# wangjiarui153/AIGV-Assessor

Hardware: AMD Instinct MI355X
Metric: scored clips/sec (8-frame 448x448, InternVL2-8B stage-2 score eval) (higher is better)
Workload: dtype bf16

## Files before the change

### aigv-assessor_amd/build.py

```python
from __future__ import annotations

import os
import subprocess
import sys
from concurrent.futures import ThreadPoolExecutor

HERE = os.path.dirname(os.path.abspath(__file__))
CSRC = os.path.join(HERE, "csrc")
OBJ = os.path.join(HERE, "build")
SOURCES = ["api.hip", "gemm.hip", "gemm256.hip", "gemmco.hip", "attention.hip", "rowops.hip", "head.hip", "head8.hip", "ingest.hip", "slowfast.hip"]
HEADERS = ["common.h", "kernels.h", "attn_lay.h", os.path.join("..", "..", "include", "aigv_amd.h")]
OUT = os.path.join(HERE, "libaigv_amd.so")
FLAGS = ["--offload-arch=gfx950", "-O3", "-std=c++17", "-fPIC", "-Wno-unused-value"]
EXTRA_FLAGS = {"attention.hip": ["-fno-slp-vectorize"]}
DIAG_DEFINES = os.environ.get("AIGV_HIPCC_DEFINES", "").split()


def _mtime(p: str) -> float:
    return os.path.getmtime(p) if os.path.exists(p) else 0.0


def _obj(src: str) -> str:
    return os.path.join(OBJ, src.replace(".hip", ".o"))


def _stale_objects() -> list:
    newest_header = max(_mtime(os.path.join(CSRC, h)) for h in HEADERS)
    me = _mtime(os.path.abspath(__file__))
    return [s for s in SOURCES if _mtime(_obj(s)) < max(_mtime(os.path.join(CSRC, s)), newest_header, me)]


def _stale() -> bool:
    return bool(_stale_objects()) or _mtime(OUT) < max(_mtime(_obj(s)) for s in SOURCES)


def build(force: bool = False, verbose: bool = False, jobs: int = 4) -> str:
    os.makedirs(OBJ, exist_ok=True)
    todo = list(SOURCES) if force else _stale_objects()
    if not todo and not _stale():
        return OUT
    hipcc = os.environ.get("HIPCC", "/opt/rocm/bin/hipcc")
    if not os.path.exists(hipcc):
        hipcc = "hipcc"

    def compile_one(src: str):
        cmd = [hipcc] + FLAGS + DIAG_DEFINES + EXTRA_FLAGS.get(src, []) + ["-c", os.path.join(CSRC, src), "-o", _obj(src)]
        if verbose:
            print(" ".join(cmd), file=sys.stderr)
        return src, subprocess.run(cmd, capture_output=True, text=True)

    with ThreadPoolExecutor(max_workers=max(1, jobs)) as ex:
        for src, r in ex.map(compile_one, todo):
            if r.returncode != 0:
                raise RuntimeError(f"hipcc failed on {src} ({r.returncode}):\n{r.stderr[-4000:]}")
    cmd = [hipcc, "--offload-arch=gfx950", "-shared", "-fPIC", "-o", OUT] + [_obj(s) for s in SOURCES]
    if verbose:
        print(" ".join(cmd), file=sys.stderr)
    r = subprocess.run(cmd, capture_output=True, text=True)
    if r.returncode != 0:
        raise RuntimeError(f"link failed ({r.returncode}):\n{r.stderr[-4000:]}")
    return OUT


if __name__ == "__main__":
    print(build(force="--force" in sys.argv, verbose=True))
```

### aigv-assessor_amd/csrc/api.hip

```cpp
#include <hip/hip_runtime.h>

#include <algorithm>
#include <cmath>
#include <new>
#include <cstdarg>
#include <cstdio>
#include <cstring>
#include <mutex>
#include <string>
#include <unordered_map>
#include <vector>

#include "../../include/aigv_amd.h"
#include "kernels.h"

namespace {

thread_local std::string g_err;

struct DevBuf {
  void* p = nullptr;
  size_t bytes = 0;
};

struct VitLayer {
  const bf16_t *ls1, *ls2, *qkv_w, *qkv_b, *qn, *kn, *proj_w, *proj_b, *fc1_w, *fc1_b, *fc2_w, *fc2_b, *n1w, *n1b, *n2w, *n2b;
};
struct LlmLayer {
  const bf16_t *wqkv, *wo, *w13, *w2, *an, *fn;
};

struct LlmLayerFp8 {
  uint8_t *wqkv = nullptr, *wo = nullptr, *w13 = nullptr, *w2 = nullptr;
  float *s_wqkv = nullptr, *s_wo = nullptr, *s_w13 = nullptr, *s_w2 = nullptr;
};

struct ProfRec {
  int cls;
  hipEvent_t a, b;
  double flops, bytes;
};

struct RowPlan {
  struct Tiny { int row0, stride_rows, count; };
  std::vector<Tiny> tiny;
  int rows = 0, body_halves = 0, tail_halves = 0, tail_rows = 0;
  int32_t* d_tab = nullptr;
  int cap_halves = 0;
};

}

struct aigv_ctx {
  aigv_config cfg{};
  int device = 0;
  std::string err;
  std::unordered_map<std::string, DevBuf> w;
  std::vector<void*> allocs;
  std::vector<void*> ws_allocs;
  bool ws_phase = false;
  bool finalized = false;
  int np = 0, S = 0, Kp = 0, grid = 0, ntok = 0, proj_in = 0, qkv_out = 0, head_dim = 0, vit_head_dim = 0, g = 0;
  std::vector<VitLayer> vit;
  std::vector<LlmLayer> llm;
  const bf16_t *patch_w = nullptr, *patch_b = nullptr, *pos = nullptr, *cls_pos = nullptr;
  const bf16_t *tok_emb = nullptr, *final_norm = nullptr, *lm_head = nullptr, *rope_cos = nullptr, *rope_sin = nullptr;
  const bf16_t *p_ln_w[2] = {nullptr, nullptr}, *p_ln_b[2] = {nullptr, nullptr}, *p_w1[2] = {nullptr, nullptr},
               *p_b1[2] = {nullptr, nullptr}, *p_w2[2] = {nullptr, nullptr}, *p_b2[2] = {nullptr, nullptr};
  ScoreHeadArgs score{};
  bf16_t *v_col = nullptr, *v_x = nullptr, *v_t = nullptr, *v_qkv = nullptr, *v_ao = nullptr, *v_h = nullptr;
  int32_t* v_cu = nullptr;
  bf16_t *p_t = nullptr, *p_mid = nullptr;
  bf16_t *l_h = nullptr, *l_t = nullptr, *l_qkv = nullptr, *l_ao = nullptr, *l_ffn = nullptr, *l_rows = nullptr;
  int32_t *l_pos = nullptr, *l_seq = nullptr, *l_cu = nullptr, *l_rowidx = nullptr, *l_rowidx2 = nullptr, *l_kvlen = nullptr;
  unsigned long long* l_packed = nullptr;
  int32_t* l_neg1 = nullptr;
  bool fp8_llm = false;
  bool llm_lin_dirty = false;
  std::vector<LlmLayerFp8> llm8;
  uint8_t* q8 = nullptr;
  float* q8_scale = nullptr;
  RowPlan rp_vit, rp_llm;
  const RowPlan* cur_rp = nullptr;
  bool trim_last_layer = true;
  int attn_round_scores = AIGV_ATTENTION_NUMERICS_DEFAULT;
  int gemm_mode = -1;
  int t_order = -1, t_variant = -1, t_attn_waves = -1, t_skinny_p = -1, t_body_tile = -1, t_co_kmax = -1;
  int t_tail_slices = -1, t_lead_key = -1, t_decode_fused = -1, t_decode_fp8 = -1, t_skinny_p8 = -1, t_fuse_tails = -1, t_lone_body = -1;
  size_t splitk_floats = 0;
  float* splitk_ws = nullptr;
  float* splitk_ws_vit = nullptr;
  bool on_vit_front = false;
  bf16_t* l_trim = nullptr;
  bf16_t* l_trim_h = nullptr;
  bf16_t* l_score_ws = nullptr;
  bf16_t *kc = nullptr, *vc = nullptr;
  bf16_t *kc_alt = nullptr, *vc_alt = nullptr;
  int32_t* beam_ints = nullptr;
  float* dec_ws = nullptr;
  int32_t *dec_pos = nullptr, *dec_seq = nullptr, *dec_kvlen = nullptr, *dec_slot = nullptr;
  std::vector<int32_t> h_dec;
  std::vector<int32_t> h_pos, h_seq, h_rowidx, h_kvlen;
  int kv_seqs = 0;
  bool kv_valid = false;
  bool prof = false;
  int gemm_cls = AIGV_PROF_GEMM;
  std::vector<ProfRec> recs;
  std::vector<hipEvent_t> ev_pool;
};

namespace {

int fail(aigv_ctx* c, int code, const char* fmt, ...) {
  char buf[512];
  va_list ap;
  va_start(ap, fmt);
  vsnprintf(buf, sizeof buf, fmt, ap);
  va_end(ap);
  if (c) c->err = buf;
  g_err = buf;
  return code;
}

#define HIPCHK(c, call)                                                                              \
  do {                                                                                               \
    hipError_t e_ = (call);                                                                          \
    if (e_ != hipSuccess) return fail(c, AIGV_ERR_HIP, "%s failed: %s (%s:%d)", #call, hipGetErrorString(e_), __FILE__, __LINE__); \
  } while (0)
#define TRY(x)            \
  do {                    \
    int r_ = (x);         \
    if (r_ != 0) return r_; \
  } while (0)

template <typename T>
int dalloc(aigv_ctx* c, T** out, size_t count) {
  void* p = nullptr;
  const size_t bytes = (count ? count : 1) * sizeof(T);
  hipError_t e = hipMalloc(&p, bytes);
  if (e != hipSuccess) return fail(c, AIGV_ERR_ALLOC, "hipMalloc(%zu bytes) failed: %s", bytes, hipGetErrorString(e));
  e = hipMemset(p, 0, bytes);
  if (e != hipSuccess) return fail(c, AIGV_ERR_HIP, "hipMemset failed: %s", hipGetErrorString(e));
  (c->ws_phase ? c->ws_allocs : c->allocs).push_back(p);
  *out = (T*)p;
  return 0;
}

inline uint16_t f32_to_bf16_host(float f) {
  uint32_t u;
  memcpy(&u, &f, 4);
  if ((u & 0x7fffffffu) > 0x7f800000u) return (uint16_t)((u >> 16) | 0x40);
  u += 0x7fffu + ((u >> 16) & 1u);
  return (uint16_t)(u >> 16);
}
inline float bf16_to_f32_host(uint16_t v) {
  uint32_t u = (uint32_t)v << 16;
  float f;
  memcpy(&f, &u, 4);
  return f;
}

int roundup(int x, int m) { return (x + m - 1) / m * m; }

hipEvent_t get_event(aigv_ctx* c) {
  if (!c->ev_pool.empty()) {
    hipEvent_t e = c->ev_pool.back();
    c->ev_pool.pop_back();
    return e;
  }
  hipEvent_t e;
  if (hipEventCreate(&e) != hipSuccess) return nullptr;
  return e;
}
struct ProfScope {
  aigv_ctx* c;
  hipStream_t s;
  ProfRec r{};
  bool on;
  ProfScope(aigv_ctx* c_, int cls, double flops, double bytes, hipStream_t s_) : c(c_), s(s_), on(c_ && c_->prof) {
    if (!on) return;
    r.cls = cls; r.flops = flops; r.bytes = bytes;
    r.a = get_event(c); r.b = get_event(c);
    if (!r.a || !r.b) { on = false; return; }
    hipEventRecord(r.a, s);
  }
  ~ProfScope() {
    if (!on) return;
    hipEventRecord(r.b, s);
    c->recs.push_back(r);
  }
};

struct RowPlanScope {
  aigv_ctx* c;
  RowPlanScope(aigv_ctx* c_, const RowPlan* rp) : c(c_) { c->cur_rp = rp; }
  ~RowPlanScope() { c->cur_rp = nullptr; }
};

struct SplitkVitScope {
  aigv_ctx* c;
  explicit SplitkVitScope(aigv_ctx* c_) : c(c_) { c->on_vit_front = true; }
  ~SplitkVitScope() { c->on_vit_front = false; }
};

struct GemmClassScope {
  aigv_ctx* c;
  int keep;
  GemmClassScope(aigv_ctx* c_, int cls) : c(c_), keep(c_->gemm_cls) { c->gemm_cls = cls; }
  ~GemmClassScope() { c->gemm_cls = keep; }
};

constexpr int CO_KMAX_DEFAULT = 0;
struct Tune {
  int gemm_mode = 0, order_sel = 0, variant_sel = 0, attn_waves = 0, skinny_p = 0, body_tile = 0, co_kmax = CO_KMAX_DEFAULT;
  int tail_slices = 0, lead_key = 0, decode_fused = 1, decode_fp8 = 1, skinny_p8 = 0;
  int fuse_tails = 0;
  int lone_body = 1;
};
Tune g_tune;
int resolved_gemm_mode(const aigv_ctx* c) { return (c && c->gemm_mode >= 0) ? c->gemm_mode : g_tune.gemm_mode; }
Tune tune_of(const aigv_ctx* c) {
  Tune t = g_tune;
  if (c) {
    if (c->gemm_mode >= 0) t.gemm_mode = c->gemm_mode;
    if (c->t_order >= 0) t.order_sel = c->t_order;
    if (c->t_variant >= 0) t.variant_sel = c->t_variant;
    if (c->t_attn_waves >= 0) t.attn_waves = c->t_attn_waves;
    if (c->t_skinny_p >= 0) t.skinny_p = c->t_skinny_p;
    if (c->t_body_tile >= 0) t.body_tile = c->t_body_tile;
    if (c->t_co_kmax >= 0) t.co_kmax = c->t_co_kmax;
    if (c->t_tail_slices >= 0) t.tail_slices = c->t_tail_slices;
    if (c->t_lead_key >= 0) t.lead_key = c->t_lead_key;
    if (c->t_decode_fused >= 0) t.decode_fused = c->t_decode_fused;
    if (c->t_decode_fp8 >= 0) t.decode_fp8 = c->t_decode_fp8;
    if (c->t_skinny_p8 >= 0) t.skinny_p8 = c->t_skinny_p8;
    if (c->t_fuse_tails >= 0) t.fuse_tails = c->t_fuse_tails;
    if (c->t_lone_body >= 0) t.lone_body = c->t_lone_body;
  }
  return t;
}
GemmArgs tuned(const aigv_ctx* c, const GemmArgs& a) {
  GemmArgs b = a;
  const Tune t = tune_of(c);
  b.order_sel = t.order_sel; b.variant_sel = t.variant_sel;
  return b;
}
double g_rate256 = 1.46;
constexpr double KT128 = 0.95, FIX128 = 6.0, LONE128 = 0.70, FIX256 = 9.0, LAUNCH_GAP = 2.0;
double kt256() { return 2.0 * KT128 / g_rate256; }

double t256(long row_tiles, int N, int nk) {
  if (row_tiles <= 0) return 0;
  const long tiles = row_tiles * (N / 256);
  return (double)((tiles + 255) / 256) * (nk * kt256() + FIX256);
}
double t128_blocks(long blocks, double nk_each) {
  const double rt = nk_each * KT128 + FIX128;
  const long full = blocks / 512, part = blocks % 512;
  return full * rt + (part == 0 ? 0.0 : part <= 256 ? LONE128 * rt : rt);
}
double t128(int rows, int N, int nk) { return rows <= 0 ? 0 : t128_blocks((long)((rows + 127) / 128) * (N / 128), nk); }
double t_finalize(long rows, int N, int S) { return (double)rows * N * (4.0 * S + 4.0) / 3.0e6 + 3.0; }

constexpr size_t SPLITK_MAX_FLOATS = (size_t)64 << 20;
constexpr int MAX_DEVICES = 64;
float* g_op_splitk_ws[MAX_DEVICES] = {};
std::mutex g_op_splitk_lock;

int splitk_scratch(aigv_ctx* c, size_t need_floats, float** out) {
  if (need_floats > SPLITK_MAX_FLOATS) return fail(c, AIGV_ERR_ARG, "split-K scratch: %zu floats exceed the planner's cap", need_floats);
  if (c) {
    if (need_floats > c->splitk_floats) return fail(c, AIGV_ERR_STATE, "split-K scratch: %zu floats exceed the context's %zu", need_floats, c->splitk_floats);
    *out = c->on_vit_front ? c->splitk_ws_vit : c->splitk_ws;
    return 0;
  }
  int dev = 0;
  HIPCHK(c, hipGetDevice(&dev));
  if (dev < 0 || dev >= MAX_DEVICES) return fail(c, AIGV_ERR_ARG, "device %d out of range", dev);
  std::lock_guard<std::mutex> g(g_op_splitk_lock);
  if (!g_op_splitk_ws[dev]) HIPCHK(c, hipMalloc((void**)&g_op_splitk_ws[dev], SPLITK_MAX_FLOATS * sizeof(float)));
  *out = g_op_splitk_ws[dev];
  return 0;
}
constexpr int SPLITS[] = {2, 3, 4, 6, 8};

double best_split128(int rows, int N, int nk, int epi, int* S_out) {
  *S_out = 1;
  double best = t128(rows, N, nk);
  if (epi == EPI_PATCH) return best;
  const long tiles = (long)((rows + 127) / 128) * (N / 128);
  for (int S : SPLITS) {
    if (nk % S || nk / S < 4 || (size_t)S * rows * N > SPLITK_MAX_FLOATS) continue;
    const double t = t128_blocks(tiles * S, (double)nk / S) + t_finalize(rows, N, S) + LAUNCH_GAP;
    if (t < best) { best = t; *S_out = S; }
  }
  return best;
}
double best_split256(long row_tiles, int N, int nk, int* S_out) {
  *S_out = 0;
  double best = 1e30;
  for (int S : SPLITS) {
    if (nk % S || nk / S < 4 || (size_t)S * row_tiles * 256 * N > SPLITK_MAX_FLOATS) continue;
    const long blocks = row_tiles * (N / 256) * S;
    const double t = (double)((blocks + 255) / 256) * ((double)nk / S * kt256() + FIX256) + t_finalize(row_tiles * 256, N, S) + LAUNCH_GAP;
    if (t < best) { best = t; *S_out = S; }
  }
  return best;
}

int skinny_epi(int epi) {
  switch (epi) {
    case EPI_STORE: return 0;
    case EPI_GELU: return 3;
    case EPI_LS_RESID: return 6;
    case EPI_RESID: return 1;
    case EPI_SWIGLU: return 2;
  }
  return -1;
}
double t_skinny(int rows, int N, int K) {
  if (rows <= 0) return 0;
  if (rows > 64 || K % 128) return 1e30;
  return (double)N * K * 2.0 / 4.5e6 + 4.0;
}

#define GEMM_PROF(c, a, s) ProfScope ps(c, (c) ? (c)->gemm_cls : AIGV_PROF_GEMM, 2.0 * (a).M * (double)(a).N * (a).K, \
                                       2.0 * ((double)(a).M * (a).K + (double)(a).N * (a).K + (double)(a).M * (a).N), s)

int launch_one(aigv_ctx* c, const GemmArgs& a, int epi, bool use256, hipStream_t s) {
  GEMM_PROF(c, a, s);
  HIPCHK(c, use256 ? aigv_launch_gemm256(tuned(c, a), epi, s) : aigv_launch_gemm(a, epi, s));
  return 0;
}

int launch_co(aigv_ctx* c, const GemmArgs& a, int epi, hipStream_t s) {
  GEMM_PROF(c, a, s);
  HIPCHK(c, aigv_launch_gemmco(tuned(c, a), epi, s));
  return 0;
}
bool use_co(const aigv_ctx* c, const GemmArgs& a, int mode) {
  if (!aigv_gemmco_supported(a)) return false;
  return mode == 4 || ((mode == 0 || mode == 3) && a.K <= tune_of(c).co_kmax);
}

int launch_splitk(aigv_ctx* c, const GemmArgs& a, int epi, int S, bool tile256, hipStream_t s) {
  float* ws = nullptr;
  TRY(splitk_scratch(c, (size_t)S * a.M * a.N, &ws));
  GEMM_PROF(c, a, s);
  HIPCHK(c, aigv_launch_gemm_splitk(tuned(c, a), epi, S, ws, s, tile256));
  return 0;
}

GemmArgs row_slice(const GemmArgs& a, int row0, int rows) {
  GemmArgs b = a;
  b.M = rows;
  b.A = a.A + (size_t)row0 * a.lda;
  b.C = a.C + (size_t)row0 * a.ldc;
  if (a.resid) b.resid = a.resid + (size_t)row0 * a.ldr;
  return b;
}

struct GemmPlan {
  int top_tiles = 0;
  int mid_tiles = 0;
  int mid_slices = 0;
  int last_rows = 0;
  int last_kind = 0;
  int last_slices = 1;
  double est_us = 0;
};

GemmPlan plan_gemm(int M, int N, int K, int epi, int mode) {
  GemmPlan pl;
  const int nk = K / 64, sk = skinny_epi(epi);
  const bool ok256 = (N % 256 == 0);
  if (mode == 1 || !ok256) { pl.last_rows = M; pl.last_kind = 2; pl.est_us = t128(M, N, nk); return pl; }
  pl.top_tiles = -1;
  pl.est_us = t256((M + 255) / 256, N, nk);
  if (mode == 2) return pl;
  if (epi == EPI_PATCH) {
    if (t128(M, N, nk) < pl.est_us) { pl = GemmPlan(); pl.last_rows = M; pl.last_kind = 2; pl.est_us = t128(M, N, nk); }
    return pl;
  }
  const int full_tiles = M / 256;
  for (int R = 0; R <= full_tiles; ++R) {
    for (int Q = 0; Q <= 8 && R + Q <= full_tiles; ++Q) {
      const int rem = M - (R + Q) * 256;
      int S256 = 0, S128 = 1, last = 0;
      double t = t256(R, N, nk);
      if (Q > 0) {
        const double tm = best_split256(Q, N, nk, &S256);
        if (!S256) continue;
        t += tm;
      }
      if (rem > 0) {
        const double tk = best_split128(rem, N, nk, epi, &S128);
        const double ts = sk >= 0 ? t_skinny(rem, N, K) : 1e30;
        last = ts < tk ? 1 : 2;
        if (last == 1) S128 = 1;
        t += ts < tk ? ts : tk;
      }
      t += LAUNCH_GAP * ((R > 0) + (Q > 0) + (rem > 0) - 1);
      if (t < pl.est_us) {
        pl.est_us = t; pl.top_tiles = R; pl.mid_tiles = Q; pl.mid_slices = S256; pl.last_rows = rem; pl.last_kind = last;
        pl.last_slices = S128;
      }
    }
  }
  return pl;
}

int split_columns(int M, int N, int K, int epi, int mode) {
  if (mode != 0 || N % 256 != 128 || N < 384 || epi == EPI_PATCH || epi == EPI_SWIGLU) return 0;
  const int nk = K / 64;
  const double whole = t128(M, N, nk);
  const double split = plan_gemm(M, N - 128, K, epi, mode).est_us + t128(M, 128, nk) + LAUNCH_GAP;
  return split < whole ? 128 : 0;
}

GemmArgs col_slice(const GemmArgs& a, int n0, int n) {
  GemmArgs b = a;
  b.N = n;
  b.W = a.W + (size_t)n0 * a.ldw;
  b.C = a.C + n0;
  if (a.bias) b.bias = a.bias + n0;
  if (a.ls) b.ls = a.ls + n0;
  if (a.resid) b.resid = a.resid + n0;
  return b;
}

int run_gemm(aigv_ctx* c, const GemmArgs& a, int epi, hipStream_t s) {
  if (const char* m = aigv_gemm_check(a, epi)) return fail(c, AIGV_ERR_ARG, "%s (M=%d N=%d K=%d epi=%d)", m, a.M, a.N, a.K, epi);
  if (use_co(c, a, resolved_gemm_mode(c))) return launch_co(c, a, epi, s);
  const int mode = resolved_gemm_mode(c) == 3 || resolved_gemm_mode(c) == 4 ? 0 : resolved_gemm_mode(c);
  if (const int right = split_columns(a.M, a.N, a.K, epi, mode)) {
    TRY(run_gemm(c, col_slice(a, 0, a.N - right), epi, s));
    return launch_one(c, col_slice(a, a.N - right, right), epi, false, s);
  }
  const GemmPlan pl = plan_gemm(a.M, a.N, a.K, epi, mode);
  if (pl.top_tiles < 0) return launch_one(c, a, epi, true, s);
  int row = 0;
  if (pl.top_tiles > 0) {
    TRY(launch_one(c, row_slice(a, 0, pl.top_tiles * 256), epi, true, s));
    row = pl.top_tiles * 256;
  }
  if (pl.mid_tiles > 0) {
    TRY(launch_splitk(c, row_slice(a, row, pl.mid_tiles * 256), epi, pl.mid_slices, true, s));
    row += pl.mid_tiles * 256;
  }
  if (row < a.M) {
    const GemmArgs bot = row_slice(a, row, a.M - row);
    if (pl.last_kind == 1) {
      const int sk = skinny_epi(epi);
      ProfScope ps(c, c ? c->gemm_cls : AIGV_PROF_GEMM, 2.0 * bot.M * (double)a.N * a.K, 2.0 * (double)a.N * a.K, s);
      hipError_t e = aigv_launch_skinny_gemm(bot.A, bot.lda, bot.M, bot.W, bot.ldw, bot.N, bot.K, bot.bias, bot.resid, bot.ldr,
                                            bot.C, bot.ldc, sk, s, bot.ls);
      if (e != hipSuccess) return fail(c, AIGV_ERR_HIP, "skinny remainder (M=%d N=%d K=%d): %s", bot.M, bot.N, bot.K, hipGetErrorString(e));
      return 0;
    }
    if (pl.last_slices > 1) return launch_splitk(c, bot, epi, pl.last_slices, false, s);
    return launch_one(c, bot, epi, false, s);
  }
  return 0;
}

constexpr int TINY_TAIL = 4;

int build_row_plan(aigv_ctx* c, RowPlan& rp, const int32_t* cu, int n_seq, hipStream_t s) {
  rp.tiny.clear();
  std::vector<int32_t> body, tail;
  bool uniform = true;
  for (int b = 1; b < n_seq; ++b) uniform = uniform && (cu[b + 1] - cu[b] == cu[1] - cu[0]);
  rp.tail_rows = 0;
  for (int b = 0; b < n_seq; ++b) {
    const int L = cu[b + 1] - cu[b], nb = L / 256, rem = L % 256, r0 = cu[b] + nb * 256;
    for (int j = 0; j < 2 * nb; ++j) { body.push_back(cu[b] + j * 128); body.push_back(128); }
    if (rem == 0) continue;
    if (rem <= TINY_TAIL) {
      if (!uniform) rp.tiny.push_back({r0, 1, rem});
      else if (b == 0)
        for (int j = 0; j < rem; ++j) rp.tiny.push_back({r0 + j, L, n_seq});
      continue;
    }
    tail.push_back(r0); tail.push_back(std::min(rem, 128));
    if (rem > 128) { tail.push_back(r0 + 128); tail.push_back(rem - 128); }
    rp.tail_rows += rem;
  }
  rp.body_halves = (int)body.size() / 2;
  rp.tail_halves = (int)tail.size() / 2;
  rp.rows = cu[n_seq];
  if (rp.body_halves + rp.tail_halves > rp.cap_halves)
    return fail(c, AIGV_ERR_STATE, "row plan: %d half tiles exceed the table's %d", rp.body_halves + rp.tail_halves, rp.cap_halves);
  body.insert(body.end(), tail.begin(), tail.end());
  if (!body.empty()) HIPCHK(c, aigv_launch_write_ints(body.data(), (int)body.size(), rp.d_tab, s));
  return 0;
}

int tail_slices(int N, int K, int forced) {
  const int tn = N / 256, nk = K / 64;
  int best = 1;
  for (int S : {2, 4, 8})
    if (nk % S == 0 && nk / S >= 8 && 2 * tn * S <= 256) best = S;
  if (forced == 1 || (forced > 1 && nk % forced == 0 && nk / forced >= 4)) best = forced;
  return best;
}

int launch_tab(aigv_ctx* c, const GemmArgs& a, int epi, const int32_t* tab, int halves, int rows, int S, hipStream_t s) {
  if (halves <= 0) return 0;
  GemmArgs b = tuned(c, a);
  b.row_tab = tab; b.tab_halves = halves;
  GemmArgs pf = a; pf.M = rows;
  GEMM_PROF(c, pf, s);
  if (S <= 1) {
    HIPCHK(c, aigv_launch_gemm256(b, epi, s));
    return 0;
  }
  float* ws = nullptr;
  TRY(splitk_scratch(c, (size_t)S * ((halves + 1) / 2) * 256 * a.N, &ws));
  HIPCHK(c, aigv_launch_gemm_splitk(b, epi, S, ws, s, true));
  return 0;
}

int run_tiny_tails(aigv_ctx* c, const GemmArgs& a, int epi, const RowPlan& rp, hipStream_t s);

int run_gemm_rows(aigv_ctx* c, const GemmArgs& a, int epi, const RowPlan& rp, hipStream_t s) {
  if (const char* m = aigv_gemm_check(a, epi)) return fail(c, AIGV_ERR_ARG, "%s (M=%d N=%d K=%d epi=%d)", m, a.M, a.N, a.K, epi);
  if (a.M != rp.rows) return fail(c, AIGV_ERR_STATE, "row plan covers %d rows, the GEMM has %d", rp.rows, a.M);
  const int mode = resolved_gemm_mode(c);
  if (mode == 3) return run_gemm(c, a, epi, s);
  if (mode == 4) return use_co(c, a, mode) ? launch_co(c, a, epi, s) : launch_one(c, a, epi, false, s);
  if (use_co(c, a, mode)) {
    if (rp.body_halves + rp.tail_halves > 0) {
      GemmArgs b = a;
      b.row_tab = rp.d_tab; b.tab_halves = rp.body_halves + rp.tail_halves;
      GemmArgs pf = a; pf.M = rp.body_halves * 128 + rp.tail_rows;
      GEMM_PROF(c, pf, s);
      HIPCHK(c, aigv_launch_gemmco(tuned(c, b), epi, s));
    }
    return run_tiny_tails(c, a, epi, rp, s);
  }
  if (mode == 1 || a.N < 256) return launch_one(c, a, epi, false, s);
  if (mode == 2 && a.N % 256 == 0) return launch_one(c, a, epi, true, s);
  if (a.N % 256) {
    if (epi == EPI_SWIGLU) return launch_one(c, a, epi, false, s);
    TRY(run_gemm_rows(c, col_slice(a, 0, a.N - 128), epi, rp, s));
    return launch_one(c, col_slice(a, a.N - 128, 128), epi, false, s);
  }
  const int S = tail_slices(a.N, a.K, tune_of(c).tail_slices);
  const bool body128 = rp.body_halves > 0 && tune_of(c).body_tile == 2;
  const bool tails_apart = rp.tail_halves > 0 && S > 1;
  const long body_tiles = (long)(rp.body_halves / 2) * (a.N / 256);
  const int lone_knob = tune_of(c).lone_body;
  const bool lone = !body128 && lone_knob != 1 && rp.body_halves > 0 && a.N % 128 == 0 &&
                    (lone_knob == 2 || (body_tiles <= 128 && (!tails_apart || a.K / 64 >= 128) && (lone_knob != 3 || tails_apart) && (lone_knob != 4 || !tails_apart)));
  if (lone) {
    GemmArgs b = tuned(c, a);
    b.row_tab = rp.d_tab; b.tab_halves = tails_apart ? rp.body_halves : rp.body_halves + rp.tail_halves;
    b.variant_sel = 7;
    GemmArgs pf = a; pf.M = rp.body_halves * 128 + (tails_apart ? 0 : rp.tail_rows);
    GEMM_PROF(c, pf, s);
    HIPCHK(c, aigv_launch_gemmco(b, epi, s));
  } else if (body128) {
    {
      GemmArgs b = a;
      b.row_tab = rp.d_tab; b.tab_halves = rp.body_halves;
      GemmArgs pf = a; pf.M = rp.body_halves * 128;
      GEMM_PROF(c, pf, s);
      HIPCHK(c, aigv_launch_gemm(b, epi, s));
    }
    if (rp.tail_halves > 0 && !tails_apart) TRY(launch_tab(c, a, epi, rp.d_tab + 2 * rp.body_halves, rp.tail_halves, rp.tail_rows, 1, s));
  } else if (!tails_apart) {
    TRY(launch_tab(c, a, epi, rp.d_tab, rp.body_halves + rp.tail_halves, rp.body_halves * 128 + rp.tail_rows, 1, s));
  } else {
    const int tn = a.N / 256;
    const long body_wg = (long)(rp.body_halves / 2) * tn, slice_wg = (long)((rp.tail_halves + 1) / 2) * tn * S;
    const size_t need = (size_t)S * ((rp.tail_halves + 1) / 2) * 256 * a.N;
    const int fuse_knob = tune_of(c).fuse_tails;
    const bool by_fill = body_wg % 256 != 0 && body_wg % 256 + slice_wg <= 320;
    if (!lone && rp.body_halves > 0 && (rp.body_halves & 1) == 0 && need <= (c ? c->splitk_floats : SPLITK_MAX_FLOATS) && fuse_knob != 1 && (by_fill || fuse_knob == 2)) {
      float* ws = nullptr;
      TRY(splitk_scratch(c, need, &ws));
      GemmArgs b = tuned(c, a);
      b.row_tab = rp.d_tab; b.tab_halves = rp.body_halves; b.fuse_tail_halves = rp.tail_halves; b.part = ws; b.k_slices = S;
      GemmArgs pf = a; pf.M = rp.body_halves * 128 + rp.tail_halves * 128;
      GEMM_PROF(c, pf, s);
      HIPCHK(c, aigv_launch_gemm256_fused(b, epi, s));
      GemmArgs f = a;
      f.row_tab = rp.d_tab + 2 * rp.body_halves; f.tab_halves = rp.tail_halves;
      HIPCHK(c, aigv_launch_gemm_finalize(f, epi, S, ws, s));
      return run_tiny_tails(c, a, epi, rp, s);
    }
    if (!lone) TRY(launch_tab(c, a, epi, rp.d_tab, rp.body_halves, rp.body_halves * 128, 1, s));
  }
  if (tails_apart) {
    const size_t per_pair = (size_t)S * 256 * a.N;
    const size_t cap = c ? c->splitk_floats : SPLITK_MAX_FLOATS;
    const int max_halves = (int)std::min<size_t>(cap / per_pair, 4096) * 2;
    if (max_halves < 2) return fail(c, AIGV_ERR_STATE, "split-K scratch too small for one tail tile (N=%d, %d slices)", a.N, S);
    for (int h0 = 0; h0 < rp.tail_halves; h0 += max_halves) {
      const int nh = std::min(max_halves, rp.tail_halves - h0);
      TRY(launch_tab(c, a, epi, rp.d_tab + 2 * (rp.body_halves + h0), nh, nh * 128, S, s));
    }
  }
  return run_tiny_tails(c, a, epi, rp, s);
}

int run_tiny_tails(aigv_ctx* c, const GemmArgs& a, int epi, const RowPlan& rp, hipStream_t s) {
  const int sk = skinny_epi(epi);
  for (const RowPlan::Tiny& t : rp.tiny) {
    if (sk < 0 || a.K % 128) return fail(c, AIGV_ERR_STATE, "no skinny form for epilogue %d / K=%d (tiny sequence tails)", epi, a.K);
    const size_t ldx = (size_t)t.stride_rows * a.lda, ldo = (size_t)t.stride_rows * a.ldc, ldr = (size_t)t.stride_rows * a.ldr;
    if (ldx > 0x7fffffffu || ldo > 0x7fffffffu || ldr > 0x7fffffffu) return fail(c, AIGV_ERR_STATE, "tiny-tail row stride overflows");
    for (int i0 = 0; i0 < t.count; i0 += 64) {
      const int R = std::min(64, t.count - i0);
      const size_t r0 = (size_t)t.row0 + (size_t)i0 * t.stride_rows;
      ProfScope ps(c, c ? c->gemm_cls : AIGV_PROF_GEMM, 2.0 * R * (double)a.N * a.K, 2.0 * (double)a.N * a.K, s);
      hipError_t e = aigv_launch_skinny_gemm(a.A + r0 * a.lda, (int)ldx, R, a.W, a.ldw, a.N, a.K, a.bias, a.resid ? a.resid + r0 * a.ldr : nullptr,
                                            (int)ldr, a.C + r0 * a.ldc, (int)ldo, sk, s, a.ls, 0);
      if (e != hipSuccess) return fail(c, AIGV_ERR_HIP, "skinny tiny tails (R=%d N=%d K=%d): %s", R, a.N, a.K, hipGetErrorString(e));
    }
  }
  return 0;
}

int run_gemm_full(aigv_ctx* c, const GemmArgs& a, int epi, hipStream_t s) {
  if (const char* m = aigv_gemm_check(a, epi)) return fail(c, AIGV_ERR_ARG, "%s (M=%d N=%d K=%d epi=%d)", m, a.M, a.N, a.K, epi);
  const int mode = resolved_gemm_mode(c);
  if (use_co(c, a, mode)) return launch_co(c, a, epi, s);
  if (mode == 1 || a.N < 256 || (a.N % 256 && epi == EPI_SWIGLU)) return launch_one(c, a, epi, false, s);
  if (a.N % 256) {
    TRY(launch_one(c, col_slice(a, 0, a.N - 128), epi, true, s));
    return launch_one(c, col_slice(a, a.N - 128, 128), epi, false, s);
  }
  return launch_one(c, a, epi, true, s);
}

int run_llm_gemm(aigv_ctx* c, const GemmArgs& a, int epi, hipStream_t s) {
  return c->cur_rp ? run_gemm_rows(c, a, epi, *c->cur_rp, s) : run_gemm(c, a, epi, s);
}

GemmArgs gemm_args(const bf16_t* A, int lda, const bf16_t* W, int ldw, bf16_t* C, int ldc, int M, int N, int K) {
  GemmArgs a{};
  a.A = A; a.lda = lda; a.W = W; a.ldw = ldw; a.C = C; a.ldc = ldc; a.M = M; a.N = N; a.K = K;
  return a;
}

int run_gemm_fp8(aigv_ctx* c, const bf16_t* A, int lda, int K, const uint8_t* W8, const float* w_scale, bf16_t* C, int ldc, int T, int N,
                 int epi, const bf16_t* resid, int ldr, hipStream_t s) {
  hipError_t e = hipSuccess;
  if (A) {
    e = aigv_launch_quant_fp8_rows(A, lda, T, K, c->q8, K, c->q8_scale, s);
    if (e != hipSuccess) return fail(c, AIGV_ERR_HIP, "fp8 activation quantisation (T=%d K=%d): %s", T, K, hipGetErrorString(e));
  }
  GemmArgs a = tuned(c, GemmArgs{});
  a.A = (const bf16_t*)c->q8; a.lda = K; a.W = (const bf16_t*)W8; a.ldw = K; a.C = C; a.ldc = ldc; a.M = T; a.N = N; a.K = K;
  a.row_scale = c->q8_scale; a.col_scale = w_scale; a.resid = resid; a.ldr = ldr;
  ProfScope ps(c, AIGV_PROF_GEMM_FP8, 2.0 * T * (double)N * K, (double)T * K + (double)N * K + 2.0 * T * (epi == EPI_SWIGLU ? N / 2 : N), s);
  e = aigv_launch_gemm256_fp8(a, epi, s);
  if (e != hipSuccess) return fail(c, e == hipErrorInvalidValue ? AIGV_ERR_ARG : AIGV_ERR_HIP, "fp8 gemm (M=%d N=%d K=%d epi=%d): %s", T, N, K, epi, hipGetErrorString(e));
  return 0;
}


int run_skinny(aigv_ctx* c, const bf16_t* x, int ldx, int R, const bf16_t* W, int ldw, int N, int K, const bf16_t* bias,
               const bf16_t* resid, int ldr, bf16_t* out, int ldo, int epi, hipStream_t s, int p = 1) {
  ProfScope ps(c, AIGV_PROF_SKINNY, 2.0 * R * (double)N * K, 2.0 * (double)N * K, s);
  hipError_t e = aigv_launch_skinny_gemm(x, ldx, R, W, ldw, N, K, bias, resid, ldr, out, ldo, epi, s, nullptr, p);
  if (e != hipSuccess) return fail(c, e == hipErrorInvalidValue ? AIGV_ERR_ARG : AIGV_ERR_HIP,
                                   "skinny gemm (R=%d N=%d K=%d epi=%d): %s", R, N, K, epi, hipGetErrorString(e));
  return 0;
}

int need(aigv_ctx* c, const std::string& name, size_t elems, const bf16_t** out) {
  auto it = c->w.find(name);
  if (it == c->w.end()) return fail(c, AIGV_ERR_STATE, "weight '%s' was never loaded", name.c_str());
  if (it->second.bytes != elems * 2)
    return fail(c, AIGV_ERR_STATE, "weight '%s' has %zu elements, expected %zu", name.c_str(), it->second.bytes / 2, elems);
  *out = (const bf16_t*)it->second.p;
  return 0;
}

}


void aigv_set_error(const char* msg) { g_err = msg ? msg : ""; }

extern "C" {

int aigv_abi_version(void) { return AIGV_ABI_VERSION; }
int aigv_sizeof_config(void) { return (int)sizeof(aigv_config); }

const char* aigv_last_error(const aigv_ctx* ctx) { return ctx ? ctx->err.c_str() : g_err.c_str(); }

void aigv_clear_hip_error(void) { (void)hipGetLastError(); }

static int alloc_workspaces(aigv_ctx* c) {
  const aigv_config& k = c->cfg;
  hipError_t e = hipSuccess;
  int rc = 0;
  c->ws_phase = true;
  c->kc = c->vc = nullptr;
  c->kc_alt = c->vc_alt = nullptr; c->beam_ints = nullptr;
  c->dec_ws = nullptr; c->dec_pos = c->dec_seq = c->dec_kvlen = c->dec_slot = nullptr;
  const size_t vr = (size_t)k.vit_chunk * c->S;
  const size_t pr = (size_t)k.vit_chunk * c->ntok;
  const size_t T = (size_t)k.max_tokens;
  do {
    if ((rc = dalloc(c, &c->v_col, (size_t)k.vit_chunk * c->np * c->Kp))) break;
    if ((rc = dalloc(c, &c->v_x, vr * k.vit_hidden))) break;
    if ((rc = dalloc(c, &c->v_t, vr * k.vit_hidden))) break;
    if ((rc = dalloc(c, &c->v_qkv, vr * 3 * k.vit_hidden))) break;
    if ((rc = dalloc(c, &c->v_ao, vr * k.vit_hidden))) break;
    if ((rc = dalloc(c, &c->v_h, vr * k.vit_inter))) break;
    if ((rc = dalloc(c, &c->v_cu, (size_t)k.vit_chunk + 1))) break;
    if ((rc = dalloc(c, &c->p_t, pr * c->proj_in))) break;
    if ((rc = dalloc(c, &c->p_mid, pr * k.llm_hidden))) break;
    if ((rc = dalloc(c, &c->l_h, T * k.llm_hidden))) break;
    if ((rc = dalloc(c, &c->l_t, T * k.llm_hidden))) break;
    if ((rc = dalloc(c, &c->l_qkv, T * c->qkv_out))) break;
    if ((rc = dalloc(c, &c->l_ao, T * k.llm_hidden))) break;
    if ((rc = dalloc(c, &c->l_ffn, T * k.llm_inter))) break;
    if ((rc = dalloc(c, &c->l_rows, (size_t)(k.max_out_rows + k.max_seqs + 64) * k.llm_hidden))) break;
    if ((rc = dalloc(c, &c->l_pos, T))) break;
    if ((rc = dalloc(c, &c->l_seq, T))) break;
    if ((rc = dalloc(c, &c->l_cu, (size_t)k.max_seqs + 1))) break;
// ... 739 lines not shown
}

int aigv_kv_fork(aigv_ctx* c, int copies, void* stream) {
  if (!c) return fail(c, AIGV_ERR_ARG, "aigv_kv_fork: null context");
  if (!c->kv_valid) return fail(c, AIGV_ERR_STATE, "aigv_kv_fork: no KV state (run aigv_llm_prefill with keep_kv)");
  const aigv_config& k = c->cfg;
  const int B = c->kv_seqs;
  if (copies < 1 || (long)B * copies > k.max_seqs) return fail(c, AIGV_ERR_ARG, "aigv_kv_fork: %d x %d sequences exceed max_seqs %d", B, copies, k.max_seqs);
  if (copies == 1) return 0;
  HIPCHK(c, hipSetDevice(c->device));
  hipStream_t s = (hipStream_t)stream;
  const size_t slot = (size_t)k.llm_kv_heads * k.kv_capacity * c->head_dim;
  const size_t kv_layer = (size_t)k.max_seqs * slot;
  for (int li = 0; li < k.llm_layers; ++li)
    for (int cpy = 1; cpy < copies; ++cpy) {
      HIPCHK(c, hipMemcpyAsync(c->kc + li * kv_layer + (size_t)cpy * B * slot, c->kc + li * kv_layer, (size_t)B * slot * sizeof(bf16_t), hipMemcpyDeviceToDevice, s));
      HIPCHK(c, hipMemcpyAsync(c->vc + li * kv_layer + (size_t)cpy * B * slot, c->vc + li * kv_layer, (size_t)B * slot * sizeof(bf16_t), hipMemcpyDeviceToDevice, s));
    }
  const int N = B * copies;
  c->h_kvlen.resize(N);
  c->h_dec.resize((size_t)4 * N);
  for (int i = 0; i < N; ++i) {
    const int len = c->h_kvlen[i % B];
    c->h_kvlen[i] = len;
    c->h_dec[i] = len; c->h_dec[N + i] = i; c->h_dec[2 * N + i] = len + 1; c->h_dec[3 * N + i] = -1;
  }
  HIPCHK(c, aigv_launch_write_ints(c->h_dec.data(), N, c->dec_pos, s));
  HIPCHK(c, aigv_launch_write_ints(c->h_dec.data() + N, N, c->dec_seq, s));
  HIPCHK(c, aigv_launch_write_ints(c->h_dec.data() + 2 * N, N, c->dec_kvlen, s));
  HIPCHK(c, aigv_launch_write_ints(c->h_dec.data() + 3 * N, N, c->dec_slot, s));
  c->kv_seqs = N;
  return 0;
}

int aigv_kv_reorder(aigv_ctx* c, const int32_t* parent, const int32_t* len, int n, void* stream) {
  if (!c || !parent || !len) return fail(c, AIGV_ERR_ARG, "aigv_kv_reorder: null argument");
  if (!c->kv_valid) return fail(c, AIGV_ERR_STATE, "aigv_kv_reorder: no KV state (run aigv_llm_prefill with keep_kv)");
  const aigv_config& k = c->cfg;
  if (n != c->kv_seqs) return fail(c, AIGV_ERR_ARG, "aigv_kv_reorder: %d sequences, the cache holds %d", n, c->kv_seqs);
  int max_len = 0;
  for (int i = 0; i < n; ++i) {
    if (parent[i] < 0 || parent[i] >= n) return fail(c, AIGV_ERR_ARG, "aigv_kv_reorder: parent[%d] = %d outside 0..%d", i, parent[i], n - 1);
    if (len[i] <= 0 || len[i] > k.kv_capacity) return fail(c, AIGV_ERR_ARG, "aigv_kv_reorder: len[%d] = %d outside 1..%d", i, len[i], k.kv_capacity);
    max_len = std::max(max_len, len[i]);
  }
  HIPCHK(c, hipSetDevice(c->device));
  hipStream_t s = (hipStream_t)stream;
  if (!c->kc_alt || !c->vc_alt || !c->beam_ints) {
    const size_t per = (size_t)k.llm_layers * k.max_seqs * k.llm_kv_heads * k.kv_capacity * c->head_dim;
    void *a = nullptr, *b = nullptr, *i = nullptr;
    const hipError_t e1 = hipMalloc(&a, per * sizeof(bf16_t));
    const hipError_t e2 = e1 == hipSuccess ? hipMalloc(&b, per * sizeof(bf16_t)) : e1;
    const hipError_t e3 = e2 == hipSuccess ? hipMalloc(&i, (size_t)2 * k.max_seqs * sizeof(int32_t)) : e2;
    if (e3 != hipSuccess) {
      if (a) hipFree(a);
      if (b) hipFree(b);
      if (i) hipFree(i);
      c->kc_alt = c->vc_alt = nullptr; c->beam_ints = nullptr;
      return fail(c, AIGV_ERR_ALLOC, "aigv_kv_reorder: second KV cache (2 x %zu bytes): %s", per * sizeof(bf16_t), hipGetErrorString(e3));
    }
    c->kc_alt = (bf16_t*)a; c->vc_alt = (bf16_t*)b; c->beam_ints = (int32_t*)i;
    c->ws_allocs.push_back(a); c->ws_allocs.push_back(b); c->ws_allocs.push_back(i);
  }
  HIPCHK(c, aigv_launch_write_ints(parent, n, c->beam_ints, s));
  HIPCHK(c, aigv_launch_write_ints(len, n, c->beam_ints + k.max_seqs, s));
  const size_t kv_layer = (size_t)k.max_seqs * k.llm_kv_heads * k.kv_capacity * c->head_dim;
  hipError_t e = aigv_launch_kv_reorder(c->kc, c->vc, c->kc_alt, c->vc_alt, c->beam_ints, c->beam_ints + k.max_seqs, n, k.llm_layers, k.llm_kv_heads,
                                        k.kv_capacity, c->head_dim, kv_layer, max_len, s);
  if (e != hipSuccess) return fail(c, AIGV_ERR_HIP, "aigv_kv_reorder (n=%d): %s", n, hipGetErrorString(e));
  std::swap(c->kc, c->kc_alt);
  std::swap(c->vc, c->vc_alt);
  return 0;
}

int aigv_set_precision(aigv_ctx* c, int mode) {
  if (!c) return fail(c, AIGV_ERR_ARG, "aigv_set_precision: null context");
  if (mode != AIGV_PRECISION_BF16 && mode != AIGV_PRECISION_FP8_LLM) return fail(c, AIGV_ERR_ARG, "aigv_set_precision: unknown mode %d", mode);
  if (mode == AIGV_PRECISION_BF16) { c->fp8_llm = false; return 0; }
  if (c->llm.empty()) return fail(c, AIGV_ERR_STATE, "aigv_set_precision: call aigv_finalize_weights first");
  const aigv_config& k = c->cfg;
  const int H = k.llm_hidden, I = k.llm_inter, Q = c->qkv_out;
  if (H % 256 || Q % 256 || (2 * I) % 256 || H % 128 || I % 128)
    return fail(c, AIGV_ERR_ARG, "aigv_set_precision: the fp8 kernel needs output widths in multiples of 256 and depths in multiples of 128 (H=%d I=%d qkv=%d)", H, I, Q);
  HIPCHK(c, hipSetDevice(c->device));
  if (c->llm8.empty()) {
    std::vector<LlmLayerFp8> q(k.llm_layers);
    TRY(dalloc(c, &c->q8, (size_t)k.max_tokens * (size_t)std::max(H, I)));
    TRY(dalloc(c, &c->q8_scale, (size_t)k.max_tokens));
    for (int li = 0; li < k.llm_layers; ++li) {
      const LlmLayer& L = c->llm[li];
      struct { const bf16_t* w; int n, kk; uint8_t** q; float** sc; } items[4] = {
          {L.wqkv, Q, H, &q[li].wqkv, &q[li].s_wqkv}, {L.wo, H, H, &q[li].wo, &q[li].s_wo},
          {L.w13, 2 * I, H, &q[li].w13, &q[li].s_w13}, {L.w2, H, I, &q[li].w2, &q[li].s_w2}};
      for (auto& it : items) {
        TRY(dalloc(c, it.q, (size_t)it.n * it.kk));
        TRY(dalloc(c, it.sc, (size_t)it.n));
        hipError_t e = aigv_launch_quant_fp8_rows(it.w, it.kk, it.n, it.kk, *it.q, it.kk, *it.sc, nullptr);
        if (e != hipSuccess) return fail(c, AIGV_ERR_HIP, "weight quantisation failed: %s", hipGetErrorString(e));
      }
    }
    HIPCHK(c, hipDeviceSynchronize());
    c->llm8 = std::move(q);
  }
  c->fp8_llm = true;
  return 0;
}

int aigv_set_row_trimming(aigv_ctx* c, int on) {
  if (!c) return fail(c, AIGV_ERR_ARG, "aigv_set_row_trimming: null context");
  c->trim_last_layer = on != 0;
  return 0;
}

int aigv_ctx_tune(aigv_ctx* c, int knob, int value) {
  if (!c) return fail(c, AIGV_ERR_ARG, "aigv_ctx_tune: null context");
  switch (knob) {
    case AIGV_TUNE_GEMM_MODE: return aigv_set_gemm_mode(c, value);
    case AIGV_TUNE_GEMM256_ORDER:
      if (value < -1 || value > 15) break;
      c->t_order = value; return 0;
    case AIGV_TUNE_GEMM256_VARIANT:
      if (value < -1 || value > 7) break;
      c->t_variant = value; return 0;
    case AIGV_TUNE_ATTN_WAVES:
      if (value != -1 && value != 0 && value != 4 && value != 8) break;
      c->t_attn_waves = value; return 0;
    case AIGV_TUNE_SKINNY_P:
      if (value != -1 && value != 0 && value != 1 && value != 2 && value != 4 && !(value >= 1000 && value < 1000 + 4096)) break;
      c->t_skinny_p = value; return 0;
    case AIGV_TUNE_BODY_TILE:
      if (value < -1 || value > 2) break;
      c->t_body_tile = value; return 0;
    case AIGV_TUNE_CO_KMAX:
      if (value < -1 || value > 65536 || (value > 0 && value % 64)) break;
      c->t_co_kmax = value; return 0;
    case AIGV_TUNE_TAIL_SLICES:
      if (value < -1 || value > 16) break;
      c->t_tail_slices = value; return 0;
    case AIGV_TUNE_ATTN_LEAD_KEY:
      if (value < -1 || value > 1) break;
      c->t_lead_key = value; return 0;
    case AIGV_TUNE_DECODE_FUSED:
      if (value < -1 || value > 1) break;
      c->t_decode_fused = value; return 0;
    case AIGV_TUNE_DECODE_FP8:
      if (value < -1 || value > 1) break;
      c->t_decode_fp8 = value; return 0;
    case AIGV_TUNE_FUSE_TAILS:
      if (value < -1 || value > 2) break;
      c->t_fuse_tails = value; return 0;
    case AIGV_TUNE_LONE_BODY:
      if (value < -1 || value > 4) break;
      c->t_lone_body = value; return 0;
    case AIGV_TUNE_SKINNY_P8:
      if (value != -1 && value != 0 && value != 1 && value != 2 && value != 4) break;
      c->t_skinny_p8 = value; return 0;
    default: return fail(c, AIGV_ERR_ARG, "aigv_ctx_tune: unknown knob %d", knob);
  }
  return fail(c, AIGV_ERR_ARG, "aigv_ctx_tune: value %d out of range for knob %d", value, knob);
}

int aigv_get_attention_numerics(const aigv_ctx* c) { return c ? c->attn_round_scores : AIGV_ATTENTION_NUMERICS_DEFAULT; }

int aigv_set_attention_numerics(aigv_ctx* c, int mode) {
  if (!c) return fail(c, AIGV_ERR_ARG, "aigv_set_attention_numerics: null context");
  if (mode != 0 && mode != 1) return fail(c, AIGV_ERR_ARG, "aigv_set_attention_numerics: 0 (fp32 scores) or 1 (the reference's bf16 score matrix)");
  c->attn_round_scores = mode;
  return 0;
}

int aigv_set_gemm_mode(aigv_ctx* c, int mode) {
  if (!c) return fail(c, AIGV_ERR_ARG, "aigv_set_gemm_mode: null context");
  if (mode < -1 || mode > 4) return fail(c, AIGV_ERR_ARG, "aigv_set_gemm_mode: mode must be -1 (process default), 0 (row plans), 1 (128 tile), 2 (256 tile), 3 (batch-level dispatch) or 4 (co-resident 256x128 tile)");
  c->gemm_mode = mode;
  return 0;
}

static int pick_form(int max_p, int K) {
  int best = 1;
  for (int p = 2; p <= max_p; p *= 2) {
    if (K % (128 * p) || K / (4 * p) < 256 || (K > 8192 && p > 2)) break;
    best = p;
  }
  return best;
}

static void decode_forms(aigv_ctx* c, int B, int* pq, int* po, int* p13, int* p2) {
  const aigv_config& k = c->cfg;
  const int max_p = B <= 4 ? 4 : B <= 8 ? 2 : 1;
  if (resolved_gemm_mode(c) == 1) {
    *pq = *po = *p13 = *p2 = 1;
    return;
  }
  *pq = *po = *p13 = pick_form(max_p, k.llm_hidden);
  *p2 = pick_form(max_p, k.llm_inter);
  if (const int sp = tune_of(c).skinny_p) {
    if (sp < 1000) *pq = *po = *p13 = *p2 = std::min(sp, max_p);
    else {
      int* out[4] = {pq, po, p13, p2};
      for (int i = 0; i < 4; ++i) {
        const int v = ((sp - 1000) >> (3 * i)) & 7;
        if ((v == 1 || v == 2 || v == 4) && v <= max_p) *out[i] = v;
      }
    }
  }
}

int aigv_decode_step(aigv_ctx* c, const int64_t* ids, int64_t* next, void* stream) {
  if (!c || !ids || !next) return fail(c, AIGV_ERR_ARG, "aigv_decode_step: null argument");
  if (!c->kv_valid) return fail(c, AIGV_ERR_STATE, "aigv_decode_step: no KV state (run aigv_llm_prefill with keep_kv)");
  const aigv_config& k = c->cfg;
  const int B = c->kv_seqs, H = k.llm_hidden, I = k.llm_inter, D = c->head_dim, g = c->g, nkv = k.llm_kv_heads;
  if (B > 64) return fail(c, AIGV_ERR_ARG, "decode supports at most 64 clips per step");
  for (int b = 0; b < B; ++b)
    if (c->h_kvlen[b] + 1 > k.kv_capacity || c->h_kvlen[b] + 1 > k.max_positions)
      return fail(c, AIGV_ERR_STATE, "clip %d: KV cache / RoPE table exhausted at %d tokens", b, c->h_kvlen[b]);
  HIPCHK(c, hipSetDevice(c->device));
  hipStream_t s = (hipStream_t)stream;
  int max_vis = 0;
  for (int b = 0; b < B; ++b) max_vis = std::max(max_vis, c->h_kvlen[b] + 1);
  HIPCHK(c, aigv_launch_embed(ids, c->dec_slot, c->tok_emb, nullptr, nullptr, 0, c->l_h, B, H, s));
  const size_t kv_layer = (size_t)k.max_seqs * nkv * k.kv_capacity * D;
  const Tune tn_ = tune_of(c);
  const bool fused = tn_.decode_fused != 0 && B <= 4 && aigv_skinny_norm_fusable(H);
  int pq, po, p13, p2;
  decode_forms(c, B, &pq, &po, &p13, &p2);
  const bool f8 = tn_.decode_fp8 != 0 && c->fp8_llm && B <= 4 && aigv_skinny_fp8_supported(H, true) && aigv_skinny_fp8_supported(I, false) && D == 128;
  int q8[4] = {4, 2, 4, 2};
  {
    if (const int v = tn_.skinny_p8)
      for (int i = 0; i < 4; ++i) q8[i] = v;
    if (I / (4 * q8[3]) < 256 || I % (512 * q8[3])) q8[3] = 1;
  }
  for (int li = 0; li < k.llm_layers; ++li) {
    const LlmLayer& L = c->llm[li];
    if (f8) {
      const LlmLayerFp8& Q = c->llm8[li];
      const bool post8 = li != k.llm_layers - 1;
      const AigvRopeKv rk{c->dec_pos, c->dec_seq, c->rope_cos, c->rope_sin, c->kc + li * kv_layer, c->vc + li * kv_layer, g, nkv, k.kv_capacity};
      {
        ProfScope ps(c, AIGV_PROF_SKINNY, 2.0 * B * (double)c->qkv_out * H, (double)c->qkv_out * H, s);
        HIPCHK(c, aigv_launch_skinny_fp8(c->l_h, H, B, Q.wqkv, H, Q.s_wqkv, c->qkv_out, H, nullptr, 0, c->l_qkv, c->qkv_out, 7, &rk, L.an, k.rms_eps, q8[0], s));
      }
      HIPCHK(c, aigv_launch_attention_decode(c->l_qkv, c->qkv_out, (g + 2) * D, c->kc + li * kv_layer, c->vc + li * kv_layer,
                                             c->dec_kvlen, k.kv_capacity, c->l_ao, H, B, nkv, g, D, sqrtf((float)D), max_vis,
                                             c->dec_ws, s));
      if (post8) {
        ProfScope ps(c, AIGV_PROF_SKINNY, 2.0 * B * ((double)H * H + 3.0 * H * I), (double)H * H + 3.0 * H * I, s);
        HIPCHK(c, aigv_launch_skinny_fp8(c->l_ao, H, B, Q.wo, H, Q.s_wo, H, H, c->l_h, H, c->l_h, H, 1, nullptr, nullptr, 0.f, q8[1], s));
        HIPCHK(c, aigv_launch_skinny_fp8(c->l_h, H, B, Q.w13, H, Q.s_w13, 2 * I, H, nullptr, 0, c->l_ffn, I, 2, nullptr, L.fn, k.rms_eps, q8[2], s));
        HIPCHK(c, aigv_launch_skinny_fp8(c->l_ffn, I, B, Q.w2, I, Q.s_w2, H, I, c->l_h, H, c->l_h, H, 1, nullptr, nullptr, 0.f, q8[3], s));
      } else {
        TRY(run_skinny(c, c->l_ao, H, B, L.wo, H, H, H, nullptr, c->l_h, H, c->l_h, H, 1, s, po));
        if (fused) {
          ProfScope ps(c, AIGV_PROF_SKINNY, 2.0 * B * 2.0 * I * H, 2.0 * 2.0 * I * H, s);
          HIPCHK(c, aigv_launch_skinny_swiglu_normed(c->l_h, H, B, L.w13, H, 2 * I, H, c->l_ffn, I, L.fn, k.rms_eps, s, p13));
        } else {
          HIPCHK(c, aigv_launch_rmsnorm(c->l_h, H, L.fn, c->l_t, H, B, H, k.rms_eps, nullptr, s));
          TRY(run_skinny(c, c->l_t, H, B, L.w13, H, 2 * I, H, nullptr, nullptr, 0, c->l_ffn, I, 2, s, p13));
        }
        TRY(run_skinny(c, c->l_ffn, I, B, L.w2, I, H, I, nullptr, c->l_h, H, c->l_h, H, 1, s, p2));
      }
      continue;
    }
    if (!fused) HIPCHK(c, aigv_launch_rmsnorm(c->l_h, H, L.an, c->l_t, H, B, H, k.rms_eps, nullptr, s));
    {
      ProfScope ps(c, AIGV_PROF_SKINNY, 2.0 * B * (double)c->qkv_out * H, 2.0 * (double)c->qkv_out * H, s);
      HIPCHK(c, aigv_launch_skinny_rope_kv(fused ? c->l_h : c->l_t, H, B, L.wqkv, H, c->qkv_out, H, c->l_qkv, c->qkv_out, c->dec_pos, c->dec_seq, c->rope_cos,
                                           c->rope_sin, c->kc + li * kv_layer, c->vc + li * kv_layer, g, nkv, k.kv_capacity, D, s,
                                           fused ? L.an : nullptr, k.rms_eps, pq));
    }
    HIPCHK(c, aigv_launch_attention_decode(c->l_qkv, c->qkv_out, (g + 2) * D, c->kc + li * kv_layer, c->vc + li * kv_layer,
                                           c->dec_kvlen, k.kv_capacity, c->l_ao, H, B, nkv, g, D, sqrtf((float)D), max_vis,
                                           c->dec_ws, s));
    TRY(run_skinny(c, c->l_ao, H, B, L.wo, H, H, H, nullptr, c->l_h, H, c->l_h, H, 1, s, po));
    if (fused) {
      ProfScope ps(c, AIGV_PROF_SKINNY, 2.0 * B * 2.0 * I * H, 2.0 * 2.0 * I * H, s);
      HIPCHK(c, aigv_launch_skinny_swiglu_normed(c->l_h, H, B, L.w13, H, 2 * I, H, c->l_ffn, I, L.fn, k.rms_eps, s, p13));
    } else {
      HIPCHK(c, aigv_launch_rmsnorm(c->l_h, H, L.fn, c->l_t, H, B, H, k.rms_eps, nullptr, s));
      TRY(run_skinny(c, c->l_t, H, B, L.w13, H, 2 * I, H, nullptr, nullptr, 0, c->l_ffn, I, 2, s, p13));
    }
    TRY(run_skinny(c, c->l_ffn, I, B, L.w2, I, H, I, nullptr, c->l_h, H, c->l_h, H, 1, s, p2));
  }
  HIPCHK(c, aigv_launch_rmsnorm(c->l_h, H, c->final_norm, c->l_rows, H, B, H, k.rms_eps, nullptr, s));
  HIPCHK(c, aigv_launch_lm_head_argmax(c->l_rows, B, H, c->lm_head, k.vocab, c->l_packed, next, nullptr, s));
  HIPCHK(c, aigv_launch_advance(c->dec_pos, c->dec_kvlen, B, s));
  for (int b = 0; b < B; ++b) c->h_kvlen[b] += 1;
  return 0;
}

int aigv_out_row_logits(aigv_ctx* c, int first_row, int n_rows, void* logits_bf16, int ldo, void* stream) {
  if (!c || !logits_bf16) return fail(c, AIGV_ERR_ARG, "aigv_out_row_logits: null argument");
  if (!c->finalized) return fail(c, AIGV_ERR_STATE, "aigv_out_row_logits: call aigv_finalize_weights first");
  const aigv_config& k = c->cfg;
  const int cap = k.max_out_rows + k.max_seqs + 64;
  if (first_row < 0 || n_rows <= 0 || first_row + n_rows > cap) return fail(c, AIGV_ERR_ARG, "aigv_out_row_logits: rows %d..%d outside 0..%d", first_row, first_row + n_rows - 1, cap - 1);
  HIPCHK(c, hipSetDevice(c->device));
  hipStream_t s = (hipStream_t)stream;
  for (int r0 = 0; r0 < n_rows; r0 += 64) {
    const int rr = std::min(64, n_rows - r0);
    ProfScope ps(c, AIGV_PROF_SKINNY, 2.0 * rr * (double)k.vocab * k.llm_hidden, 2.0 * (double)k.vocab * k.llm_hidden, s);
    hipError_t e = aigv_launch_lm_head_logits(c->l_rows + (size_t)(first_row + r0) * k.llm_hidden, rr, k.llm_hidden, c->lm_head, k.vocab,
                                              (bf16_t*)logits_bf16 + (size_t)r0 * ldo, ldo, s);
    if (e != hipSuccess) return fail(c, e == hipErrorInvalidValue ? AIGV_ERR_ARG : AIGV_ERR_HIP, "lm-head logits (rows=%d ldo=%d): %s", rr, ldo, hipGetErrorString(e));
  }
// ... 97 lines not shown

int aigv_op_skinny_gemm(const void* x, int ldx, int R, const void* W_, int ldw, int N, int K, const void* bias,
                        const void* resid, int ldr, void* out, int ldo, int epi, void* stream) {
  return run_skinny(nullptr, (const bf16_t*)x, ldx, R, (const bf16_t*)W_, ldw, N, K, (const bf16_t*)bias,
                    (const bf16_t*)resid, ldr, (bf16_t*)out, ldo, epi, (hipStream_t)stream, g_tune.skinny_p ? g_tune.skinny_p : 1);
}

int aigv_op_skinny_gemm_fp8(const void* x, int ldx, int R, const void* W_e4m3, int ldw, const float* w_scale, int N, int K, const void* resid,
                            int ldr, void* out, int ldo, int epi, const void* norm_w, float eps, int p, void* stream) {
  if (epi != 1 && epi != 2) return fail(nullptr, AIGV_ERR_ARG, "aigv_op_skinny_gemm_fp8: epi must be 1 (residual) or 2 (swiglu)");
  hipError_t e = aigv_launch_skinny_fp8((const bf16_t*)x, ldx, R, (const uint8_t*)W_e4m3, ldw, w_scale, N, K, (const bf16_t*)resid, ldr, (bf16_t*)out, ldo,
                                        epi, nullptr, (const bf16_t*)norm_w, eps, p, (hipStream_t)stream);
  if (e != hipSuccess)
    return fail(nullptr, e == hipErrorInvalidValue ? AIGV_ERR_ARG : AIGV_ERR_HIP, "fp8 skinny gemm (R=%d N=%d K=%d epi=%d p=%d): %s", R, N, K, epi, p, hipGetErrorString(e));
  return 0;
}

int aigv_op_layernorm(const void* x, int ldx, const void* w, const void* b, void* y, int ldy, int rows, int H, float eps,
                      void* stream) {
  HIPCHK(nullptr, aigv_launch_layernorm((const bf16_t*)x, ldx, (const bf16_t*)w, (const bf16_t*)b, (bf16_t*)y, ldy, rows, H,
                                        eps, (hipStream_t)stream));
  return 0;
}

int aigv_op_rmsnorm(const void* x, int ldx, const void* w, void* y, int ldy, int rows, int H, float eps,
                    const int32_t* row_idx, void* stream) {
  HIPCHK(nullptr, aigv_launch_rmsnorm((const bf16_t*)x, ldx, (const bf16_t*)w, (bf16_t*)y, ldy, rows, H, eps, row_idx,
                                      (hipStream_t)stream));
  return 0;
}

int aigv_op_rope(void* qkv, int ld, const int32_t* pos, const void* cos, const void* sin, int tokens, int n_rot, int slots,
                 int n_groups, int head_dim, void* stream) {
  HIPCHK(nullptr, aigv_launch_rope((bf16_t*)qkv, ld, pos, (const bf16_t*)cos, (const bf16_t*)sin, tokens, n_rot, slots,
                                   n_groups, head_dim, (hipStream_t)stream));
  return 0;
}

int aigv_op_attention(const void* q, int ldq, const void* k, int ldk, const void* v, int ldv, void* o, int ldo,
                      const int32_t* cu, int n_seq, int max_len, int n_heads, int n_kv_heads, int q_group_stride,
                      int kv_head_stride, int head_dim, int causal, float post_div, float q_prescale, void* stream) {
  AttnArgs a{};
  a.q = (const bf16_t*)q; a.ldq = ldq; a.k = (const bf16_t*)k; a.ldk = ldk; a.v = (const bf16_t*)v; a.ldv = ldv;
  a.o = (bf16_t*)o; a.ldo = ldo; a.cu = cu; a.n_seq = n_seq; a.max_len = max_len; a.n_heads = n_heads;
  a.n_kv_heads = n_kv_heads; a.q_group_stride = q_group_stride; a.kv_head_stride = kv_head_stride;
  a.causal = causal & 1; a.uniform_len = (causal >> 1) & 1; a.post_div = post_div; a.q_prescale = q_prescale;
  a.round_scores = (causal >> 2) & 1; a.lead_key = (causal >> 3) & 1; a.waves = g_tune.attn_waves;
  if (const char* m = aigv_attn_check(a, head_dim)) return fail(nullptr, AIGV_ERR_ARG, "%s", m);
  HIPCHK(nullptr, aigv_launch_attention(a, head_dim, (hipStream_t)stream));
  return 0;
}

int aigv_op_attention_rope(const void* q, int ldq, const void* k, int ldk, const void* v, int ldv, void* o, int ldo,
                           const int32_t* cu, int n_seq, int max_len, int n_heads, int n_kv_heads, int q_group_stride,
                           int kv_head_stride, int head_dim, int causal, float post_div, float q_prescale, const int32_t* pos,
                           const void* cos, const void* sin, void* stream) {
  AttnArgs a{};
  a.q = (const bf16_t*)q; a.ldq = ldq; a.k = (const bf16_t*)k; a.ldk = ldk; a.v = (const bf16_t*)v; a.ldv = ldv;
  a.o = (bf16_t*)o; a.ldo = ldo; a.cu = cu; a.n_seq = n_seq; a.max_len = max_len; a.n_heads = n_heads;
  a.n_kv_heads = n_kv_heads; a.q_group_stride = q_group_stride; a.kv_head_stride = kv_head_stride;
  a.causal = causal & 1; a.uniform_len = (causal >> 1) & 1; a.post_div = post_div; a.q_prescale = q_prescale;
  a.round_scores = (causal >> 2) & 1; a.lead_key = (causal >> 3) & 1; a.waves = g_tune.attn_waves;
  a.rope_pos = pos; a.rope_cos = (const bf16_t*)cos; a.rope_sin = (const bf16_t*)sin;
  if (const char* m = aigv_attn_check(a, head_dim)) return fail(nullptr, AIGV_ERR_ARG, "%s", m);
  HIPCHK(nullptr, aigv_launch_attention(a, head_dim, (hipStream_t)stream));
  return 0;
}

int aigv_op_pixel_shuffle(const void* vit_out, int grid, int vit_hidden, void* out, int n_frames, void* stream) {
  HIPCHK(nullptr, aigv_launch_pixel_shuffle((const bf16_t*)vit_out, grid, vit_hidden, (bf16_t*)out, n_frames, (hipStream_t)stream));
  return 0;
}

int aigv_op_im2col(const void* frames, int n_frames, int channels, int image_size, int patch, int kp, void* out,
                   void* stream) {
  HIPCHK(nullptr, aigv_launch_im2col((const bf16_t*)frames, n_frames, channels, image_size, patch, kp, (bf16_t*)out,
                                     (hipStream_t)stream));
  return 0;
}

int aigv_op_lm_head_argmax(const void* h, int rows, int hidden, const void* W_, int vocab, void* scratch_u64, int64_t* idx,
                           float* val, void* stream) {
  HIPCHK(nullptr, aigv_launch_lm_head_argmax((const bf16_t*)h, rows, hidden, (const bf16_t*)W_, vocab,
                                             (unsigned long long*)scratch_u64, idx, val, (hipStream_t)stream));
  return 0;
}

int aigv_op_frame_ingest(const void* hwc_u8, int n_frames, int height, int width, const float* mean, const float* stdv,
                         void* out_nchw, void* stream) {
  HIPCHK(nullptr, aigv_launch_frame_ingest((const uint8_t*)hwc_u8, n_frames, height, width, mean, stdv, (bf16_t*)out_nchw,
                                           (hipStream_t)stream));
  return 0;
}

int aigv_op_frame_resize_ingest(const void* hwc_u8, int n_frames, int in_h, int in_w, int out_h, int out_w, const float* mean,
                                const float* stdv, void* tmp_u8, void* out_u8_hwc, void* out_nchw, void* stream) {
  if (!hwc_u8 || !tmp_u8 || (!out_u8_hwc && !out_nchw) || n_frames < 0 || in_h <= 0 || in_w <= 0 || out_h <= 0 || out_w <= 0 ||
      (out_nchw && (!mean || !stdv)))
    return fail(nullptr, AIGV_ERR_ARG, "aigv_op_frame_resize_ingest: bad argument (frames %d, %dx%d -> %dx%d)", n_frames, in_h, in_w, out_h, out_w);
  if (in_h > 16384 || in_w > 16384 || out_h > 16384 || out_w > 16384)
    return fail(nullptr, AIGV_ERR_ARG, "aigv_op_frame_resize_ingest: sizes above 16384 are not supported");
  if (in_w != out_w && in_h != out_h && in_h > out_h && (long)in_h > 100L * in_w)
    return fail(nullptr, AIGV_ERR_ARG, "aigv_op_frame_resize_ingest: %dx%d frames (more than 100 times taller than wide) are not supported: Pillow orders its passes differently there", in_h, in_w);
  HIPCHK(nullptr, aigv_launch_frame_resize_ingest((const uint8_t*)hwc_u8, n_frames, in_h, in_w, out_h, out_w, mean, stdv,
                                                  (uint8_t*)tmp_u8, (uint8_t*)out_u8_hwc, (bf16_t*)out_nchw, (hipStream_t)stream));
  return 0;
}

int aigv_plan_gemm(int M, int N, int K, int epi, int* plan, double* est_us) {
  if (!plan || M <= 0 || N <= 0 || K <= 0 || N % 128 || K % 64 || epi < 0 || epi >= EPI_COUNT)
    return fail(nullptr, AIGV_ERR_ARG, "aigv_plan_gemm: bad problem M=%d N=%d K=%d epi=%d", M, N, K, epi);
  const int pmode = g_tune.gemm_mode == 3 ? 0 : g_tune.gemm_mode;
  const int right = split_columns(M, N, K, epi, pmode);
  const GemmPlan pl = plan_gemm(M, N - right, K, epi, pmode);
  plan[6] = right;
  plan[0] = pl.top_tiles; plan[1] = pl.mid_tiles; plan[2] = pl.mid_slices; plan[3] = pl.last_rows; plan[4] = pl.last_kind;
  plan[5] = pl.last_slices;
  if (est_us) *est_us = pl.est_us + (right ? t128(M, right, K / 64) + LAUNCH_GAP : 0.0);
  return 0;
}

int aigv_tune_skinny(int p) {
  if (p != 0 && p != 1 && p != 2 && p != 4) return fail(nullptr, AIGV_ERR_ARG, "aigv_tune_skinny: 0 (default), 1, 2 or 4, got %d", p);
  g_tune.skinny_p = p;
  return 0;
}

int aigv_tune_attention(int waves) {
  if (waves != 0 && waves != 4 && waves != 8)
    return fail(nullptr, AIGV_ERR_ARG, "aigv_tune_attention: 0 (default), 4 or 8 waves per workgroup, got %d", waves);
  g_tune.attn_waves = waves;
  return 0;
}

int aigv_tune_gemm(int mode, double rate256) {
  g_tune.body_tile = (mode >> 14) & 3;
  g_tune.order_sel = (mode >> 10) & 15;
  mode &= 1023;
  const int vsel = mode >> 4;
  mode &= 15;
  if (mode < 0 || mode > 4 || vsel < 0 || vsel > 7)
    return fail(nullptr, AIGV_ERR_ARG, "aigv_tune_gemm: mode must be 0 (auto), 1 (128 tile), 2 (256 tile), 3 (batch-level dispatch in the scoring pass) or 4 (co-resident 256x128 tile)");
  if (vsel > 0) g_tune.variant_sel = vsel;
  g_tune.gemm_mode = mode;
  if (rate256 > 0) g_rate256 = rate256;
  return 0;
}

int aigv_tune_default(int knob, int value) {
  switch (knob) {
    case AIGV_TUNE_TAIL_SLICES: if (value < 0 || value > 16) break; g_tune.tail_slices = value; return 0;
    case AIGV_TUNE_FUSE_TAILS: if (value < 0 || value > 2) break; g_tune.fuse_tails = value; return 0;
    case AIGV_TUNE_LONE_BODY: if (value < 0 || value > 4) break; g_tune.lone_body = value; return 0;
    case AIGV_TUNE_ATTN_LEAD_KEY: if (value < 0 || value > 1) break; g_tune.lead_key = value; return 0;
    case AIGV_TUNE_CO_KMAX: return aigv_tune_co_gemm(value);
    default: return fail(nullptr, AIGV_ERR_ARG, "aigv_tune_default: knob %d has no process default here (aigv_tune_gemm / _attention / _skinny set the others)", knob);
  }
  return fail(nullptr, AIGV_ERR_ARG, "aigv_tune_default: value %d out of range for knob %d", value, knob);
}

int aigv_tune_co_gemm(int kmax) {
  if (kmax < 0 || kmax > 65536 || kmax % 64) return fail(nullptr, AIGV_ERR_ARG, "aigv_tune_co_gemm: K threshold must be 0 (off) or a multiple of 64");
  g_tune.co_kmax = kmax;
  return 0;
}

int aigv_prof_enable(aigv_ctx* c, int on) {
  if (!c) return fail(c, AIGV_ERR_ARG, "null ctx");
  c->prof = on != 0;
  return 0;
}

int aigv_prof_read(aigv_ctx* c, int cls, int64_t* launches, double* total_ms, double* flops, double* bytes) {
  if (!c || cls < 0 || cls >= AIGV_PROF_COUNT) return fail(c, AIGV_ERR_ARG, "aigv_prof_read: bad argument");
  HIPCHK(c, hipSetDevice(c->device));
  int64_t n = 0;
  double ms = 0, fl = 0, by = 0;
  std::vector<ProfRec> keep;
  for (auto& r : c->recs) {
    if (r.cls != cls) { keep.push_back(r); continue; }
    HIPCHK(c, hipEventSynchronize(r.b));
    float t = 0;
    HIPCHK(c, hipEventElapsedTime(&t, r.a, r.b));
    ms += t; fl += r.flops; by += r.bytes; ++n;
    c->ev_pool.push_back(r.a);
    c->ev_pool.push_back(r.b);
  }
  c->recs.swap(keep);
  if (launches) *launches = n;
  if (total_ms) *total_ms = ms;
  if (flops) *flops = fl;
  if (bytes) *bytes = by;
  return 0;
}

}
```

### aigv-assessor_amd/csrc/gemm256.hip

```cpp
#include <cstdlib>
#include <type_traits>

#include "common.h"
#include "kernels.h"

namespace {

constexpr int TM = 256, TN = 256, TK = 64;
constexpr int UNIT = 128 * 128;
constexpr int BUF = 4 * UNIT;
constexpr int STAGE_ROWP = 144;
constexpr int STAGE_BYTES = 16 * STAGE_ROWP;
constexpr int LDS_BYTES = 2 * BUF + 8 * STAGE_BYTES;
constexpr int GROUP_M256 = 4;
inline int row_tiles(const GemmArgs& a) { return a.row_tab ? (a.tab_halves + 1) / 2 : (a.M + TM - 1) / TM; }
}
static inline int tile_order(const GemmArgs& a, bool big_w, int nbm) { return a.order_sel > 0 ? a.order_sel - 1 : (big_w && nbm >= 32 ? 4 : 0); }
namespace {

#define RAW_BARRIER() asm volatile("s_barrier" ::: "memory")

#ifdef AIGV_GEMM_STAMP
constexpr int GSTAMP_REPL = 1024;
__device__ unsigned long long g_gemm_stamp[8][2][GSTAMP_REPL][8];
#define GSTAMP(var) const unsigned long long var = __builtin_readcyclecounter()
#else
#define GSTAMP(var)
#endif

__device__ __forceinline__ void wait_vm(int n) {
  if (n >= 8) asm volatile("s_waitcnt vmcnt(8)" ::: "memory");
  else if (n == 6) asm volatile("s_waitcnt vmcnt(6)" ::: "memory");
  else if (n == 4) asm volatile("s_waitcnt vmcnt(4)" ::: "memory");
  else if (n == 2) asm volatile("s_waitcnt vmcnt(2)" ::: "memory");
  else asm volatile("s_waitcnt vmcnt(0)" ::: "memory");
}

__device__ __forceinline__ void store_row_segment(bf16_t* dst, const u16x8& val, int policy) {
#ifdef AIGV_STORE_POLICY_AB
  if (policy == 5) { asm volatile("global_store_dwordx4 %0, %1, off nt" : : "v"(dst), "v"(val) : "memory"); return; }
  if (policy == 6) { asm volatile("global_store_dwordx4 %0, %1, off sc1" : : "v"(dst), "v"(val) : "memory"); return; }
  if (policy == 7) { asm volatile("global_store_dwordx4 %0, %1, off sc1 nt" : : "v"(dst), "v"(val) : "memory"); return; }
#endif
  (void)policy;
  *(u16x8*)dst = val;
}

template <int EPI, int VAR, bool FP8 = false, bool FUSE = false>
__global__ __launch_bounds__(512, 2) void gemm256_kernel(const GemmArgs p) {
  static_assert(!FP8 || ((VAR & 4) != 0 && EPI != EPI_PATCH), "the fp8 form uses the LDS-staged epilogue (or writes split-K slabs)");
  static_assert(!FUSE || (!FP8 && EPI != EPI_PARTIAL && EPI != EPI_PATCH), "the fused form: bf16, a body epilogue");
  extern __shared__ __attribute__((aligned(16))) char smem[];
  const int tid = threadIdx.x, lane = tid & 63;
  const int wave = __builtin_amdgcn_readfirstlane(tid >> 6);
  const int g = wave >> 2, wc = wave & 3;
  GSTAMP(gs_begin);

  const int nbm = p.row_tab ? (p.tab_halves + 1) / 2 : (p.M + TM - 1) / TM, nbn = p.N / TN;
  const int n_body = nbm * nbn;
  const bool is_slice = FUSE && (int)blockIdx.x >= n_body;
  const int nwg = is_slice ? ((p.fuse_tail_halves + 1) / 2) * nbn * p.k_slices : n_body;
  int wg;
  {
    const int bid = is_slice ? (int)blockIdx.x - n_body : (int)blockIdx.x, xcd = bid & 7, q = nwg >> 3, r = nwg & 7;
    wg = (xcd < r ? xcd * (q + 1) : r * (q + 1) + (xcd - r) * q) + (bid >> 3);
  }
  const bool partial = (EPI == EPI_PARTIAL) || is_slice;
  int slice_idx = (EPI == EPI_PARTIAL) ? (int)blockIdx.y : 0;
  int tm, tn;
  if (is_slice) {
    slice_idx = wg % p.k_slices;
    const int tile = wg / p.k_slices;
    tn = tile % nbn; tm = tile / nbn;
  } else if (p.order == 0) {
    const int per_group = GROUP_M256 * nbn;
    const int grp = wg / per_group, first_m = grp * GROUP_M256;
    const int gsz = min(nbm - first_m, GROUP_M256);
    const int in_g = wg - grp * per_group;
    tm = first_m + in_g % gsz; tn = in_g / gsz;
  } else {
    const int gn = p.order;
    const int per_group = gn * nbm;
    const int grp = wg / per_group, first_n = grp * gn;
    const int gsz = min(nbn - first_n, gn);
    const int in_g = wg - grp * per_group;
    tn = first_n + in_g % gsz; tm = in_g / gsz;
  }
  const int n0 = tn * TN;
  int hb, hv;
  if (p.row_tab) {
    const int h = 2 * tm + g;
    hb = 0; hv = 0;
    if (is_slice) {
      if (h < p.fuse_tail_halves) { hb = p.row_tab[2 * (p.tab_halves + h)]; hv = p.row_tab[2 * (p.tab_halves + h) + 1]; }
    } else if (h < p.tab_halves) { hb = p.row_tab[2 * h]; hv = p.row_tab[2 * h + 1]; }
  } else {
    hb = tm * TM + g * 128; hv = min(p.M - hb, 128);
    if (hv <= 0) { hb = p.M - 1; hv = 0; }
  }
  hb = __builtin_amdgcn_readfirstlane(hb);
  hv = __builtin_amdgcn_readfirstlane(hv);
  const int hend = hb + hv;
  auto relc = [&](int r) { return max(min(r, hv - 1), 0); };

  const int lr = lane >> 3, lc = (lane & 7) ^ lr;
  const int nk = partial ? p.K / TK / p.k_slices : p.K / TK;
  const size_t kbase = partial ? (size_t)slice_idx * nk * TK : 0;
  const char* tileA = (const char*)(p.A + (size_t)hb * p.lda + kbase);
  const char* tileW = (const char*)(p.W + (size_t)n0 * p.ldw + kbase);
  unsigned off[4][2];
#pragma unroll
  for (int i = 0; i < 2; ++i) {
    const int r = wave * 16 + i * 8 + lr;
    const int ra0 = r & 63, rb0 = (r >> 5) * 64 + (r & 31);
    off[0][i] = (unsigned)relc(ra0) * (unsigned)p.lda * 2u + lc * 16;
    off[1][i] = (unsigned)relc(ra0 + 64) * (unsigned)p.lda * 2u + lc * 16;
    off[2][i] = (unsigned)rb0 * (unsigned)p.ldw * 2u + lc * 16;
    off[3][i] = (unsigned)(rb0 + 32) * (unsigned)p.ldw * 2u + lc * 16;
  }
  const int n_units = 4 * nk;
  const unsigned lds0 = (unsigned)(size_t)(LDS_AS char*)smem + wave * 2048;
  auto dma = [&](int tile, int unit) {
    const char* base = (unit < 2 ? tileA : tileW) + (size_t)tile * (TK * 2);
    const unsigned dst = lds0 + (tile & 1) * BUF + unit * UNIT;
    glds16_saddr(base, off[unit][0], dst);
    glds16_saddr(base, off[unit][1], dst + 1024);
  };
  auto issue = [&](int tile, int o) {
    if (tile >= nk) return;
    dma(tile, (o == 0) ? 0 : (o == 1) ? 2 : (o == 2) ? 3 : 1);
  };

  constexpr bool RESID_PF = ((VAR & 4) != 0) && (EPI == EPI_RESID || EPI == EPI_LS_RESID) && !FP8;
  const char* rtile = RESID_PF ? (const char*)(p.resid + (size_t)hb * p.ldr + n0 + wc * 64) : nullptr;
  auto resid_dma = [&](int mh, int i0, int cnt) {
    const int buf = (mh == 0) ? ((nk - 1) & 1) ^ 1 : ((nk - 1) & 1);
    const unsigned dst = (unsigned)(size_t)(LDS_AS char*)smem + buf * BUF + wave * 8192;
#pragma unroll
    for (int i = i0; i < i0 + cnt; ++i) {
      const int r = i * 8 + lr;
      const int row = relc(mh * 64 + r);
      glds16_saddr(rtile, (unsigned)row * (unsigned)p.ldr * 2u + (unsigned)(((lane & 7) ^ (r & 7)) * 16), dst + i * 1024);
    }
  };

  const int fr = lane & 15, fq = lane >> 4, sw = fr & 7;
  int offA[2], offB[2];
#pragma unroll
  for (int kh = 0; kh < 2; ++kh) {
    const int phys = (FP8 ? (2 * fq + kh) : (kh * 4 + fq)) ^ sw;
    offA[kh] = (g * 64 + fr) * 128 + phys * 16;
    offB[kh] = (wc * 32 + fr) * 128 + phys * 16;
  }

  f32x4 acc[2][4][2][2];
#pragma unroll
  for (int a = 0; a < 2; ++a)
#pragma unroll
    for (int b = 0; b < 4; ++b)
#pragma unroll
      for (int c = 0; c < 2; ++c)
#pragma unroll
        for (int d = 0; d < 2; ++d) acc[a][b][c][d] = f32x4{0.f, 0.f, 0.f, 0.f};
  bf16x8 fa[4][2], fb0[2][2][2], fb1[2][2];
  constexpr bool BAL = (VAR & 1) != 0;
  constexpr bool PRIO = (VAR & 2) == 0;

  auto read_b0 = [&](const char* sb, auto SET) {
#pragma unroll
    for (int nt = 0; nt < 2; ++nt)
#pragma unroll
      for (int kh = 0; kh < 2; ++kh) fb0[decltype(SET)::value][nt][kh] = *(const bf16x8*)(sb + 2 * UNIT + offB[kh] + nt * 2048);
  };
  auto read_b1 = [&](const char* sb) {
#pragma unroll
    for (int nt = 0; nt < 2; ++nt)
#pragma unroll
      for (int kh = 0; kh < 2; ++kh) fb1[nt][kh] = *(const bf16x8*)(sb + 3 * UNIT + offB[kh] + nt * 2048);
  };
  auto read_a = [&](const char* sb, int unit) {
#pragma unroll
    for (int mt = 0; mt < 4; ++mt)
#pragma unroll
      for (int kh = 0; kh < 2; ++kh) fa[mt][kh] = *(const bf16x8*)(sb + unit * UNIT + offA[kh] + mt * 2048);
  };
  typedef int v8i_t __attribute__((ext_vector_type(8)));
  typedef int v4i_t __attribute__((ext_vector_type(4)));
  auto cat = [](bf16x8 lo, bf16x8 hi) {
    const v4i_t l = __builtin_bit_cast(v4i_t, lo), h = __builtin_bit_cast(v4i_t, hi);
    return v8i_t{l[0], l[1], l[2], l[3], h[0], h[1], h[2], h[3]};
  };
  auto mfma16 = [&](auto J, auto SET) {
    constexpr int j = decltype(J)::value, st = decltype(SET)::value;
    if constexpr (FP8) {
#pragma unroll
      for (int mt = 0; mt < 4; ++mt)
#pragma unroll
        for (int nt = 0; nt < 2; ++nt) {
          const v8i_t fav = cat(fa[mt][0], fa[mt][1]);
          if constexpr (j == 0) acc[0][mt][0][nt] = __builtin_amdgcn_mfma_scale_f32_16x16x128_f8f6f4(cat(fb0[st][nt][0], fb0[st][nt][1]), fav, acc[0][mt][0][nt], 0, 0, 0, 127, 0, 127);
          if constexpr (j == 1) acc[0][mt][1][nt] = __builtin_amdgcn_mfma_scale_f32_16x16x128_f8f6f4(cat(fb1[nt][0], fb1[nt][1]), fav, acc[0][mt][1][nt], 0, 0, 0, 127, 0, 127);
          if constexpr (j == 2) acc[1][mt][1][nt] = __builtin_amdgcn_mfma_scale_f32_16x16x128_f8f6f4(cat(fb1[nt][0], fb1[nt][1]), fav, acc[1][mt][1][nt], 0, 0, 0, 127, 0, 127);
          if constexpr (j == 3) acc[1][mt][0][nt] = __builtin_amdgcn_mfma_scale_f32_16x16x128_f8f6f4(cat(fb0[st][nt][0], fb0[st][nt][1]), fav, acc[1][mt][0][nt], 0, 0, 0, 127, 0, 127);
        }
      return;
// ... 342 lines not shown
            if constexpr (EPI == EPI_LS_RESID) {
              const u16x4 s = *(const u16x4*)(p.ls + n);
#pragma unroll
              for (int e = 0; e < 4; ++e) v[e] = rbf(v[e] * bf2f(s[e]));
            }
            if constexpr (EPI == EPI_LS_RESID || EPI == EPI_RESID) {
              const u16x4 r = *(const u16x4*)(p.resid + (size_t)m * p.ldr + n);
#pragma unroll
              for (int e = 0; e < 4; ++e) v[e] = rbf(bf2f(r[e]) + v[e]);
            }
            if constexpr (EPI == EPI_PATCH) {
              const u16x4 ps = *(const u16x4*)(posrow + n);
#pragma unroll
              for (int e = 0; e < 4; ++e) v[e] = rbf(v[e] + bf2f(ps[e]));
            }
            u16x4 o;
#pragma unroll
            for (int e = 0; e < 4; ++e) o[e] = f2bf(v[e]);
            *(u16x4*)(p.C + orow * p.ldc + n) = o;
          }
      }
    }
  GSTAMP_FINISH();
}

template <int EPI, int VAR>
hipError_t launch256(const GemmArgs& a, hipStream_t s) {
  static LdsAttrOnce lds_attr;
  if (hipError_t e = lds_attr.ensure((const void*)gemm256_kernel<EPI, VAR>, LDS_BYTES); e != hipSuccess) return e;
  const int nbm = row_tiles(a), nbn = a.N / TN;
  GemmArgs b = a;
  b.order = tile_order(a, (size_t)a.N * (size_t)a.K >= ((size_t)32 << 20), nbm);
  hipLaunchKernelGGL((gemm256_kernel<EPI, VAR>), dim3(nbm * nbn), dim3(512), LDS_BYTES, s, b);
  return hipGetLastError();
}

template <int VAR>
hipError_t launch256v(const GemmArgs& a, int epi, hipStream_t s) {
  switch (epi) {
    case EPI_STORE: return launch256<EPI_STORE, VAR>(a, s);
    case EPI_GELU: return launch256<EPI_GELU, VAR>(a, s);
    case EPI_LS_RESID: return launch256<EPI_LS_RESID, VAR>(a, s);
    case EPI_RESID: return launch256<EPI_RESID, VAR>(a, s);
    case EPI_SWIGLU: return launch256<EPI_SWIGLU, VAR>(a, s);
    case EPI_PATCH: return launch256<EPI_PATCH, VAR>(a, s);
  }
  return hipErrorInvalidValue;
}

}

#ifdef AIGV_GEMM_STAMP
extern "C" int aigv_debug_gemm_stamps(unsigned long long* out , int reset) {
  static unsigned long long host[8][2][GSTAMP_REPL][8];
  if (hipDeviceSynchronize() != hipSuccess) return -2;
  if (out) {
    if (hipMemcpyFromSymbol(host, HIP_SYMBOL(g_gemm_stamp), sizeof host) != hipSuccess) return -2;
    for (int e = 0; e < 8; ++e)
      for (int c = 0; c < 2; ++c)
        for (int i = 0; i < 8; ++i) {
          unsigned long long t = 0;
          for (int r = 0; r < GSTAMP_REPL; ++r) t += host[e][c][r][i];
          out[(e * 2 + c) * 8 + i] = t;
        }
  }
  if (reset) {
    for (auto& a : host) for (auto& b : a) for (auto& c : b) for (auto& d : c) d = 0;
    if (hipMemcpyToSymbol(HIP_SYMBOL(g_gemm_stamp), host, sizeof host) != hipSuccess) return -2;
  }
  return 0;
}
#endif


bool aigv_gemm256_supported(const GemmArgs& a) { return a.N % TN == 0 && a.K % TK == 0 && a.M >= 1 && (!a.row_tab || a.tab_halves >= 1); }

template <int EPI>
hipError_t launch256_fp8(const GemmArgs& b, hipStream_t s) {
  static LdsAttrOnce lds_attr;
  if (hipError_t e = lds_attr.ensure((const void*)gemm256_kernel<EPI, 7, true>, LDS_BYTES); e != hipSuccess) return e;
  const int nbm = row_tiles(b), nbn = b.N / TN;
  GemmArgs c = b;
  c.order = tile_order(b, (size_t)b.N * (size_t)b.K * 2 >= ((size_t)64 << 20), nbm);
  hipLaunchKernelGGL((gemm256_kernel<EPI, 7, true>), dim3(nbm * nbn), dim3(512), LDS_BYTES, s, c);
  return hipGetLastError();
}

hipError_t aigv_launch_gemm256_fp8(const GemmArgs& a, int epi, hipStream_t s) {
  if (a.M < 1 || a.N % TN || a.K % 128 || (a.lda % 16) || (a.ldw % 16) || !a.row_scale || !a.col_scale || !a.A || !a.W || !a.C)
    return hipErrorInvalidValue;
  if ((epi == EPI_RESID || epi == EPI_LS_RESID) && (!a.resid || a.ldr % 8)) return hipErrorInvalidValue;
  if (epi == EPI_LS_RESID && !a.ls) return hipErrorInvalidValue;
  if (epi == EPI_SWIGLU && a.bias) return hipErrorInvalidValue;
  GemmArgs b = a;
  b.K = a.K / 2; b.lda = a.lda / 2; b.ldw = a.ldw / 2;
  switch (epi) {
    case EPI_STORE: return launch256_fp8<EPI_STORE>(b, s);
    case EPI_GELU: return launch256_fp8<EPI_GELU>(b, s);
    case EPI_LS_RESID: return launch256_fp8<EPI_LS_RESID>(b, s);
    case EPI_RESID: return launch256_fp8<EPI_RESID>(b, s);
    case EPI_SWIGLU: return launch256_fp8<EPI_SWIGLU>(b, s);
    default: return hipErrorInvalidValue;
  }
}

hipError_t aigv_launch_gemm256_fp8_partial(const GemmArgs& a, hipStream_t s) {
  if (a.M < 1 || a.N % TN || a.K % 128 || (a.lda % 16) || (a.ldw % 16) || !a.row_scale || !a.col_scale || !a.A || !a.W || !a.part || a.k_slices < 1 ||
      (a.K / 128) % a.k_slices)
    return hipErrorInvalidValue;
  static LdsAttrOnce lds_attr;
  if (hipError_t e = lds_attr.ensure((const void*)gemm256_kernel<EPI_PARTIAL, 7, true>, LDS_BYTES); e != hipSuccess) return e;
  GemmArgs b = a;
  b.K = a.K / 2; b.lda = a.lda / 2; b.ldw = a.ldw / 2;
  const int nbm = row_tiles(a), nbn = a.N / TN;
  hipLaunchKernelGGL((gemm256_kernel<EPI_PARTIAL, 7, true>), dim3(nbm * nbn, a.k_slices), dim3(512), LDS_BYTES, s, b);
  return hipGetLastError();
}

hipError_t aigv_launch_gemm256_partial(const GemmArgs& a, hipStream_t s) {
  if (!aigv_gemm256_supported(a) || a.k_slices < 1 || (a.K / TK) % a.k_slices || !a.part) return hipErrorInvalidValue;
  static LdsAttrOnce lds_attr;
  if (hipError_t e = lds_attr.ensure((const void*)gemm256_kernel<EPI_PARTIAL, 7>, LDS_BYTES); e != hipSuccess) return e;
  const int nbm = row_tiles(a), nbn = a.N / TN;
  hipLaunchKernelGGL((gemm256_kernel<EPI_PARTIAL, 7>), dim3(nbm * nbn, a.k_slices), dim3(512), LDS_BYTES, s, a);
  return hipGetLastError();
}

template <int EPI>
static hipError_t launch256_fused(const GemmArgs& a, hipStream_t s) {
  static LdsAttrOnce lds_attr;
  if (hipError_t e = lds_attr.ensure((const void*)gemm256_kernel<EPI, 7, false, true>, LDS_BYTES); e != hipSuccess) return e;
  const int nbm = (a.tab_halves + 1) / 2, nbn = a.N / TN;
  GemmArgs b = a;
  b.order = tile_order(a, (size_t)a.N * (size_t)a.K >= ((size_t)32 << 20), nbm);
  b.fuse_body_wg = nbm * nbn;
  const int grid = nbm * nbn + ((a.fuse_tail_halves + 1) / 2) * nbn * a.k_slices;
  hipLaunchKernelGGL((gemm256_kernel<EPI, 7, false, true>), dim3(grid), dim3(512), LDS_BYTES, s, b);
  return hipGetLastError();
}

hipError_t aigv_launch_gemm256_fused(const GemmArgs& a, int epi, hipStream_t s) {
  if (!aigv_gemm256_supported(a) || !a.row_tab || (a.tab_halves & 1) || a.fuse_tail_halves < 1 || a.k_slices < 2 || (a.K / TK) % a.k_slices || !a.part)
    return hipErrorInvalidValue;
  switch (epi) {
    case EPI_STORE: return launch256_fused<EPI_STORE>(a, s);
    case EPI_GELU: return launch256_fused<EPI_GELU>(a, s);
    case EPI_LS_RESID: return launch256_fused<EPI_LS_RESID>(a, s);
    case EPI_RESID: return launch256_fused<EPI_RESID>(a, s);
    case EPI_SWIGLU: return launch256_fused<EPI_SWIGLU>(a, s);
  }
  return hipErrorInvalidValue;
}

hipError_t aigv_launch_gemm256(const GemmArgs& a, int epi, hipStream_t s) {
  switch (a.variant_sel > 0 ? a.variant_sel - 1 : 1) {
    case 0: return launch256v<0>(a, epi, s);
    case 3: return launch256v<3>(a, epi, s);
    default: return launch256v<7>(a, epi, s);
  }
}
```

### aigv-assessor_amd/csrc/head.hip

```cpp
#include <cstdlib>
#include <type_traits>

#include "common.h"
#include "kernels.h"

namespace {

#ifndef SKINNY_DEPTH2
#define SKINNY_DEPTH2 8
#endif
enum { SK_STORE = 0, SK_RESID = 1, SK_SWIGLU = 2, SK_GELU = 3, SK_ARGMAX = 4, SK_RELU = 5, SK_LS_RESID = 6, SK_ROPE_KV = 7 };

struct RopeKvArgs {
  const int32_t* pos; const int32_t* seq;
  const bf16_t* cos; const bf16_t* sin;
  bf16_t* kc; bf16_t* vc;
  int g, n_kv, cap;
};

struct NormArgs { const bf16_t* w; float eps; };

__device__ __forceinline__ unsigned int ord_f32(float f) {
  const unsigned int u = __float_as_uint(f);
  return (u & 0x80000000u) ? ~u : (u | 0x80000000u);
}

template <bool NT>
__device__ __forceinline__ bf16x8 wload(const bf16_t* p) {
  if constexpr (NT) return __builtin_nontemporal_load((const bf16x8*)p);
  else return *(const bf16x8*)p;
}

template <int RT, int EPI, int NWV = 4, bool NT = false, int NC = 0, int P = 1>
__global__ __launch_bounds__(NWV * 64) void skinny_kernel(const bf16_t* __restrict__ x, int ldx, int R,
                                                     const bf16_t* __restrict__ W, int ldw, int N, int K,
                                                     const bf16_t* __restrict__ bias, const bf16_t* __restrict__ resid,
                                                     int ldr, bf16_t* __restrict__ out, int ldo,
                                                     unsigned long long* __restrict__ packed,
                                                     const bf16_t* __restrict__ ls, const RopeKvArgs rk = RopeKvArgs{},
                                                     const NormArgs na = NormArgs{}) {
  constexpr bool NORM = NC > 0;
  static_assert(!NORM || (RT == 1 && NWV == 4), "the fused norm is the decode form: one row tile, 256 threads (rmsnorm_kernel's reduction)");
  extern __shared__ __attribute__((aligned(16))) bf16_t xs[];
  constexpr int NS = (EPI == SK_SWIGLU || EPI == SK_ROPE_KV) ? 2 : (EPI == SK_ARGMAX && RT >= 2) ? 4 : 1;
  static_assert(P == 1 || ((P == 2 || P == 4) && RT == 1 && EPI != SK_ARGMAX), "sub-slab forms: one row tile, 8 or 4 rows per slab");
  constexpr int RS = 16 / P;
  __shared__ float part[NWV - 1][NS][RT][4][64];
  const int lane = threadIdx.x & 63, wave = threadIdx.x >> 6;
  const int fr = lane & 15, fq = lane >> 4;
  const int sr = fr % RS, sp = fr / RS;
  const int n0 = EPI == SK_ROPE_KV ? (int)(blockIdx.x / (64 / RS)) * 128 + (int)(blockIdx.x % (64 / RS)) * RS
                 : EPI == SK_SWIGLU ? (int)(blockIdx.x / P) * 32 + (int)(blockIdx.x % P) * RS
                                    : blockIdx.x * RS * NS;
  constexpr int SLAB_STEP = EPI == SK_ROPE_KV ? 64 : 16;
  const int kper = K / (NWV * P), kbeg = (wave * P + sp) * kper;

  const bf16_t* wrow[NS];
#pragma unroll
  for (int s = 0; s < NS; ++s) wrow[s] = W + (size_t)min(n0 + s * SLAB_STEP + sr, N - 1) * ldw + kbeg + fq * 8;
  const bf16_t* xrow[RT];
#pragma unroll
  for (int t = 0; t < RT; ++t) xrow[t] = x + (size_t)min(t * 16 + sr, R - 1) * ldx + kbeg + fq * 8;

  f32x4 acc[NS][RT];
#pragma unroll
  for (int s = 0; s < NS; ++s)
#pragma unroll
    for (int t = 0; t < RT; ++t) acc[s][t] = f32x4{0.f, 0.f, 0.f, 0.f};

  constexpr int DEPTH = RT == 1 ? (NS == 1 ? 16 : SKINNY_DEPTH2) : (RT == 2 && NS == 1) ? 8 : 4;
  int k = 0;
  const int xs_off = min(sr, R - 1) * K + kbeg + fq * 8;
  if constexpr (NORM) {
    u16x8 xr[4][NC], gw[NC];
#pragma unroll
    for (int r = 0; r < 4; ++r)
#pragma unroll
      for (int c = 0; c < NC; ++c) xr[r][c] = *(const u16x8*)(x + (size_t)min(r, R - 1) * ldx + ((threadIdx.x + c * 256) << 3));
#pragma unroll
    for (int c = 0; c < NC; ++c) gw[c] = *(const u16x8*)(na.w + ((threadIdx.x + c * 256) << 3));
    bf16x8 wf[DEPTH][NS];
#pragma unroll
    for (int u = 0; u < DEPTH; ++u)
#pragma unroll
      for (int s = 0; s < NS; ++s) wf[u][s] = wload<NT>(wrow[s] + 32 * u);
    {
      __shared__ float red[4];
#pragma unroll
      for (int r = 0; r < 4; ++r) {
        if (r == 0 || r < R) {
          float sq = 0.f;
#pragma unroll
          for (int c = 0; c < NC; ++c)
#pragma unroll
            for (int e = 0; e < 8; ++e) { const float v = bf2f(xr[r][c][e]); sq += v * v; }
          const float rstd = rsqrtf(block_sum_256(sq, red) / (float)K + na.eps);
#pragma unroll
          for (int c = 0; c < NC; ++c) {
            u16x8 o;
#pragma unroll
            for (int e = 0; e < 8; ++e) o[e] = f2bf(bf2f(gw[c][e]) * rbf(bf2f(xr[r][c][e]) * rstd));
            *(u16x8*)(xs + (size_t)r * K + ((threadIdx.x + c * 256) << 3)) = o;
          }
        }
      }
      __syncthreads();
    }
#pragma unroll
    for (int u = 0; u < DEPTH; ++u) {
      const bf16x8 xf = *(const bf16x8*)(xs + xs_off + 32 * u);
#pragma unroll
      for (int s = 0; s < NS; ++s) acc[s][0] = __builtin_amdgcn_mfma_f32_16x16x32_bf16(wf[u][s], xf, acc[s][0], 0, 0, 0);
    }
    k = 32 * DEPTH;
  }
  auto run = [&](auto dtag) {
    constexpr int DD = decltype(dtag)::value;
    for (; k + 32 * DD <= kper; k += 32 * DD) {
      bf16x8 wf[DD][NS], xf[DD][RT];
#pragma unroll
      for (int u = 0; u < DD; ++u) {
#pragma unroll
        for (int s = 0; s < NS; ++s) wf[u][s] = wload<NT>(wrow[s] + k + 32 * u);
#pragma unroll
        for (int t = 0; t < RT; ++t) {
          if constexpr (NORM) xf[u][t] = *(const bf16x8*)(xs + xs_off + k + 32 * u);
          else xf[u][t] = *(const bf16x8*)(xrow[t] + k + 32 * u);
        }
      }
#pragma unroll
      for (int u = 0; u < DD; ++u)
#pragma unroll
        for (int s = 0; s < NS; ++s)
#pragma unroll
          for (int t = 0; t < RT; ++t)
            acc[s][t] = __builtin_amdgcn_mfma_f32_16x16x32_bf16(wf[u][s], xf[u][t], acc[s][t], 0, 0, 0);
    }
  };
  run(std::integral_constant<int, DEPTH>{});
  if constexpr (DEPTH > 8) run(std::integral_constant<int, 8>{});
  if constexpr (DEPTH > 4) run(std::integral_constant<int, 4>{});
  run(std::integral_constant<int, 1>{});

  if (wave > 0) {
#pragma unroll
    for (int s = 0; s < NS; ++s)
#pragma unroll
      for (int t = 0; t < RT; ++t)
#pragma unroll
        for (int e = 0; e < 4; ++e) part[wave - 1][s][t][e][lane] = acc[s][t][e];
  }
  __syncthreads();
  if (wave != 0) return;
#pragma unroll
  for (int s = 0; s < NS; ++s)
#pragma unroll
    for (int t = 0; t < RT; ++t)
#pragma unroll
      for (int e = 0; e < 4; ++e) {
        if constexpr (NWV == 4) {
          acc[s][t][e] += (part[0][s][t][e][lane] + part[1][s][t][e][lane]) + part[2][s][t][e][lane];
        } else {
          float sum = 0.f;
#pragma unroll
          for (int w = 0; w < NWV - 1; ++w) sum += part[w][s][t][e][lane];
          acc[s][t][e] += sum;
        }
      }

  if constexpr (P == 2) {
#pragma unroll
    for (int s = 0; s < NS; ++s)
#pragma unroll
      for (int e = 0; e < 4; ++e) acc[s][0][e] += __shfl(acc[s][0][e], (lane + 40) & 63, 64);
  } else if constexpr (P == 4) {
#pragma unroll
    for (int s = 0; s < NS; ++s)
#pragma unroll
      for (int e = 0; e < 4; ++e) {
        const float v = acc[s][0][e];
        acc[s][0][e] = ((v + __shfl(v, (lane + 20) & 63, 64)) + __shfl(v, (lane + 40) & 63, 64)) + __shfl(v, (lane + 60) & 63, 64);
      }
  }
  const bool own = P == 1 || (fr < RS && fq < RS / 4);

#pragma unroll
  for (int t = 0; t < RT; ++t) {
    const int r = own ? t * 16 + fr : R;
    if constexpr (EPI == SK_ARGMAX) {
      unsigned long long best = 0ull;
#pragma unroll
      for (int sl = 0; sl < NS; ++sl)
#pragma unroll
        for (int e = 0; e < 4; ++e) {
          const int n = n0 + sl * 16 + 4 * fq + e;
          if (n < N) {
            const unsigned long long key = ((unsigned long long)ord_f32(rbf(acc[sl][t][e])) << 32) | (0xFFFFFFFFu - (unsigned)n);
            best = key > best ? key : best;
          }
        }
      unsigned long long o = __shfl_xor(best, 16, 64); best = o > best ? o : best;
      o = __shfl_xor(best, 32, 64); best = o > best ? o : best;
      if (fq == 0 && r < R) atomicMax(packed + r, best);
    } else if constexpr (EPI == SK_ROPE_KV) {
      if (r < R) {
        const int hs = blockIdx.x / (64 / RS), d = (int)(blockIdx.x % (64 / RS)) * RS + 4 * fq;
        const int slot = hs % (rk.g + 2), gi = hs / (rk.g + 2);
        const int p = rk.pos[r];
        u16x4 olo, ohi;
        if (slot <= rk.g) {
          const u16x4 co = *(const u16x4*)(rk.cos + (size_t)p * 64 + d), si = *(const u16x4*)(rk.sin + (size_t)p * 64 + d);
#pragma unroll
          for (int e = 0; e < 4; ++e) {
            const float x1 = rbf(acc[0][t][e]), x2 = rbf(acc[1][t][e]), cc = bf2f(co[e]), ss = bf2f(si[e]);
            olo[e] = f2bf(rbf(x1 * cc) + rbf(-x2 * ss));
            ohi[e] = f2bf(rbf(x2 * cc) + rbf(x1 * ss));
          }
        } else {
#pragma unroll
          for (int e = 0; e < 4; ++e) { olo[e] = f2bf(acc[0][t][e]); ohi[e] = f2bf(acc[1][t][e]); }
        }
        bf16_t* dst = slot < rk.g ? out + (size_t)r * ldo + (size_t)hs * 128 + d
                                  : (slot == rk.g ? rk.kc : rk.vc) + (((size_t)rk.seq[r] * rk.n_kv + gi) * rk.cap + p) * 128 + d;
        *(u16x4*)dst = olo;
        *(u16x4*)(dst + 64) = ohi;
      }
    } else if constexpr (EPI == SK_SWIGLU) {
      if (r < R) {
        const int n = (int)(blockIdx.x / P) * 16 + (int)(blockIdx.x % P) * RS + 4 * fq;
        u16x4 o;
#pragma unroll
        for (int e = 0; e < 4; ++e) {
          const float g = rbf(acc[0][t][e]), u = rbf(acc[1][t][e]);
          o[e] = f2bf(rbf(silu_f(g)) * u);
        }
        *(u16x4*)(out + (size_t)r * ldo + n) = o;
      }
    } else {
      const int n = n0 + 4 * fq;
      if (r < R && n < N) {
        float v[4];
#pragma unroll
        for (int e = 0; e < 4; ++e) v[e] = acc[0][t][e] + (bias ? bf2f(bias[n + e]) : 0.f);
#pragma unroll
        for (int e = 0; e < 4; ++e) v[e] = rbf(v[e]);
        if constexpr (EPI == SK_GELU) {
#pragma unroll
          for (int e = 0; e < 4; ++e) v[e] = rbf(gelu_fast(v[e]));
        }
        if constexpr (EPI == SK_RELU) {
#pragma unroll
          for (int e = 0; e < 4; ++e) v[e] = fmaxf(v[e], 0.f);
        }
        if constexpr (EPI == SK_LS_RESID) {
#pragma unroll
          for (int e = 0; e < 4; ++e) v[e] = rbf(v[e] * bf2f(ls[n + e]));
        }
        if constexpr (EPI == SK_RESID || EPI == SK_LS_RESID) {
          const u16x4 rr = *(const u16x4*)(resid + (size_t)r * ldr + n);
#pragma unroll
          for (int e = 0; e < 4; ++e) v[e] = rbf(bf2f(rr[e]) + v[e]);
        }
        u16x4 o;
#pragma unroll
        for (int e = 0; e < 4; ++e) o[e] = f2bf(v[e]);
        *(u16x4*)(out + (size_t)r * ldo + n) = o;
      }
    }
  }
}

__global__ void unpack_argmax_kernel(const unsigned long long* __restrict__ packed, int64_t* __restrict__ idx,
                                     float* __restrict__ val, int R) {
  const int r = blockIdx.x * blockDim.x + threadIdx.x;
  if (r >= R) return;
  const unsigned long long p = packed[r];
  idx[r] = (int64_t)(0xFFFFFFFFu - (unsigned)(p & 0xFFFFFFFFull));
  if (val) {
    unsigned int u = (unsigned)(p >> 32);
    u = (u & 0x80000000u) ? (u & 0x7FFFFFFFu) : ~u;
    val[r] = __uint_as_float(u);
  }
}

__global__ __launch_bounds__(256) void score_guard_kernel(const bf16_t* __restrict__ x, int ldx, int B, int H,
                                                          bf16_t* __restrict__ out) {
  __shared__ int any_nan;
  if (threadIdx.x == 0) any_nan = 0;
  __syncthreads();
  int nan_here = 0;
  for (int i = threadIdx.x; i < B * H; i += 256) {
    const float v = bf2f(x[(size_t)(i / H) * ldx + (i % H)]);
    nan_here |= (v != v);
  }
  if (nan_here) atomicOr(&any_nan, 1);
  __syncthreads();
  const bool fix = any_nan != 0;
  for (int i = threadIdx.x; i < B * H; i += 256) {
    float v = bf2f(x[(size_t)(i / H) * ldx + (i % H)]);
    if (fix) {
      if (v != v) v = 0.f;
      else if (isinf(v)) v = v > 0 ? 1e9f : -1e9f;
    }
    out[i] = f2bf(v);
  }
}

__global__ __launch_bounds__(256) void score_tail_kernel(const ScoreHeadArgs a, int first_layer) {
  __shared__ float buf[2][1024];
  const int b = blockIdx.x, lane = threadIdx.x & 63, wave = threadIdx.x >> 6;
  const int d0 = a.dims[first_layer];
  for (int i = threadIdx.x; i < d0; i += 256) buf[0][i] = bf2f(a.x[(size_t)b * a.ldx + i]);
  __syncthreads();
  int cur = 0;
  for (int L = first_layer; L < a.n_layers; ++L) {
    const int din = a.dims[L], dout = a.dims[L + 1];
    const bf16_t* w = a.w[L];
    const bf16_t* bb = a.b[L];
    for (int o = wave; o < dout; o += 4) {
      float s = 0.f;
      for (int i = lane; i < din; i += 64) s += bf2f(w[(size_t)o * din + i]) * buf[cur][i];
      s = wave_sum(s);
      if (lane == 0) buf[cur ^ 1][o] = fmaxf(rbf(s + bf2f(bb[o])), 0.f);
    }
    __syncthreads();
    cur ^= 1;
  }
  if (threadIdx.x == 0) a.score[b] = buf[cur][0];
}

template <int EPI>
hipError_t launch_skinny(const bf16_t* x, int ldx, int R, const bf16_t* W, int ldw, int N, int K, const bf16_t* bias,
                         const bf16_t* resid, int ldr, bf16_t* out, int ldo, unsigned long long* packed,
                         hipStream_t s, const bf16_t* ls = nullptr, int p = 1) {
  const int rt = (R + 15) / 16;
  if (p > 1) {
    const int rs = 16 / p;
    if ((p != 2 && p != 4) || R > rs || K % (128 * p) || N % (EPI == SK_SWIGLU ? 32 : rs)) return hipErrorInvalidValue;
    if constexpr (EPI == SK_STORE || EPI == SK_RESID || EPI == SK_SWIGLU) {
      const int blocks = EPI == SK_SWIGLU ? N / 32 * p : N / rs;
      if (p == 2) hipLaunchKernelGGL((skinny_kernel<1, EPI, 4, false, 0, 2>), dim3(blocks), dim3(256), 0, s, x, ldx, R, W, ldw, N, K, bias, resid, ldr, out, ldo, packed, ls);
      else hipLaunchKernelGGL((skinny_kernel<1, EPI, 4, false, 0, 4>), dim3(blocks), dim3(256), 0, s, x, ldx, R, W, ldw, N, K, bias, resid, ldr, out, ldo, packed, ls);
      return hipGetLastError();
    } else {
      return hipErrorInvalidValue;
    }
  }
  const int ns = (EPI == SK_SWIGLU) ? 2 : (EPI == SK_ARGMAX && rt >= 2) ? 4 : 1;
  const int blocks = (N + 16 * ns - 1) / (16 * ns);
#define GO(RT) hipLaunchKernelGGL((skinny_kernel<RT, EPI>), dim3(blocks), dim3(256), 0, s, x, ldx, R, W, ldw, N, K, bias, resid, ldr, out, ldo, packed, ls)
  if constexpr (EPI == SK_STORE || EPI == SK_RESID) {
    constexpr int max8 = 256;
    if (rt == 1 && K % 256 == 0 && blocks <= max8 && p != 0) {
      hipLaunchKernelGGL((skinny_kernel<1, EPI, 8>), dim3(blocks), dim3(512), 0, s, x, ldx, R, W, ldw, N, K, bias, resid, ldr, out, ldo, packed, ls);
      return hipGetLastError();
    }
  }
  switch (rt) {
    case 1: GO(1); break;
    case 2: GO(2); break;
    case 3: GO(3); break;
    case 4: GO(4); break;
    default: return hipErrorInvalidValue;
  }
#undef GO
  return hipGetLastError();
}

}

bool aigv_skinny_norm_fusable(int K) { return K == 4096 || K == 6144; }

hipError_t aigv_launch_skinny_rope_kv(const bf16_t* x, int ldx, int R, const bf16_t* W, int ldw, int N, int K, bf16_t* qkv, int ldo,
                                      const int32_t* pos, const int32_t* seq, const bf16_t* cos, const bf16_t* sin, bf16_t* kc, bf16_t* vc,
                                      int g, int n_kv, int cap, int head_dim, hipStream_t s, const bf16_t* norm_w, float norm_eps, int p) {
  if (R <= 0) return hipSuccess;
  if (R > 64 || K % 128 || (ldx % 8) || (ldw % 8) || (ldo % 4) || head_dim != 128 || N != n_kv * (g + 2) * 128 || !pos || !seq || !cos ||
      !sin || !kc || !vc)
    return hipErrorInvalidValue;
  RopeKvArgs rk{pos, seq, cos, sin, kc, vc, g, n_kv, cap};
  const int rt = (R + 15) / 16, blocks = N / 32 * p;
  if ((p != 1 && p != 2 && p != 4) || R > (p == 1 ? 64 : 16 / p) || K % (128 * p)) return hipErrorInvalidValue;
  if (norm_w) {
    if (R > 4 || !aigv_skinny_norm_fusable(K)) return hipErrorInvalidValue;
#define GO(NC, PP) hipLaunchKernelGGL((skinny_kernel<1, SK_ROPE_KV, 4, false, NC, PP>), dim3(blocks), dim3(256), (size_t)R * K * sizeof(bf16_t), s, x, ldx, R, W, ldw, N, K, \
                                      nullptr, nullptr, 0, qkv, ldo, nullptr, nullptr, rk, NormArgs{norm_w, norm_eps})
    if (K == 4096) { if (p == 1) GO(2, 1); else if (p == 2) GO(2, 2); else GO(2, 4); }
    else { if (p == 1) GO(3, 1); else if (p == 2) GO(3, 2); else GO(3, 4); }
#undef GO
    return hipGetLastError();
  }
  if (p != 1) {
    if (p == 2) hipLaunchKernelGGL((skinny_kernel<1, SK_ROPE_KV, 4, false, 0, 2>), dim3(blocks), dim3(256), 0, s, x, ldx, R, W, ldw, N, K, nullptr, nullptr, 0, qkv, ldo, nullptr, nullptr, rk);
    else hipLaunchKernelGGL((skinny_kernel<1, SK_ROPE_KV, 4, false, 0, 4>), dim3(blocks), dim3(256), 0, s, x, ldx, R, W, ldw, N, K, nullptr, nullptr, 0, qkv, ldo, nullptr, nullptr, rk);
    return hipGetLastError();
  }
#define GO(RT) hipLaunchKernelGGL((skinny_kernel<RT, SK_ROPE_KV, 4, false>), dim3(blocks), dim3(256), 0, s, x, ldx, R, W, ldw, N, K, nullptr, nullptr, 0, qkv, ldo, nullptr, nullptr, rk)
  switch (rt) {
    case 1: GO(1); break;
    case 2: GO(2); break;
    case 3: GO(3); break;
    case 4: GO(4); break;
    default: return hipErrorInvalidValue;
  }
#undef GO
  return hipGetLastError();
}

hipError_t aigv_launch_skinny_swiglu_normed(const bf16_t* x, int ldx, int R, const bf16_t* W, int ldw, int N, int K, bf16_t* out, int ldo,
                                            const bf16_t* norm_w, float norm_eps, hipStream_t s, int p) {
  if (R <= 0) return hipSuccess;
  if (R > 4 || !aigv_skinny_norm_fusable(K) || (ldx % 8) || (ldw % 8) || (ldo % 4) || (N % 32) || !norm_w || (p != 1 && p != 2 && p != 4)) return hipErrorInvalidValue;
#define GO(NC, PP) hipLaunchKernelGGL((skinny_kernel<1, SK_SWIGLU, 4, false, NC, PP>), dim3(N / 32 * p), dim3(256), (size_t)R * K * sizeof(bf16_t), s, x, ldx, R, W, ldw, N, K, \
                                      nullptr, nullptr, 0, out, ldo, nullptr, nullptr, RopeKvArgs{}, NormArgs{norm_w, norm_eps})
  if (K == 4096) { if (p == 1) GO(2, 1); else if (p == 2) GO(2, 2); else GO(2, 4); }
  else { if (p == 1) GO(3, 1); else if (p == 2) GO(3, 2); else GO(3, 4); }
#undef GO
  return hipGetLastError();
}

hipError_t aigv_launch_skinny_gemm(const bf16_t* x, int ldx, int R, const bf16_t* W, int ldw, int N, int K,
                                   const bf16_t* bias, const bf16_t* resid, int ldr, bf16_t* out, int ldo, int epi,
// ... 72 lines not shown
```

### aigv-assessor_amd/csrc/kernels.h

```cpp
#pragma once
#include <hip/hip_runtime.h>
#include <stdint.h>

typedef uint16_t bf16_t;

enum GemmEpilogue {
  EPI_STORE = 0,
  EPI_GELU = 1,
  EPI_LS_RESID = 2,
  EPI_RESID = 3,
  EPI_SWIGLU = 4,
  EPI_PATCH = 5,
  EPI_COUNT = 6,
  EPI_PARTIAL = 6
};

struct GemmArgs {
  const bf16_t* A; int lda;
  const bf16_t* W; int ldw;
  bf16_t* C; int ldc;
  const bf16_t* bias;
  const bf16_t* ls;
  const bf16_t* resid; int ldr;
  const bf16_t* pos;
  int M, N, K;
  int np;
  float* part;
  int k_slices;
  const float* row_scale;
  const float* col_scale;
  const int32_t* row_tab; int tab_halves;
  int fuse_tail_halves, fuse_body_wg;
  int order_sel, variant_sel;
  int order;
};

const char* aigv_gemm_check(const GemmArgs& a, int epi);
hipError_t aigv_launch_gemm(const GemmArgs& a, int epi, hipStream_t s);
hipError_t aigv_launch_gemm_splitk(const GemmArgs& a, int epi, int k_slices, float* ws, hipStream_t s, bool tile256 = false);
hipError_t aigv_launch_gemm256_partial(const GemmArgs& a, hipStream_t s);
hipError_t aigv_launch_gemm256_fp8(const GemmArgs& a, int epi, hipStream_t s);
hipError_t aigv_launch_gemm256_fp8_partial(const GemmArgs& a, hipStream_t s);
hipError_t aigv_launch_gemm_splitk_fp8(const GemmArgs& a, int epi, int k_slices, float* ws, hipStream_t s);
hipError_t aigv_launch_rmsnorm_quant_fp8(const bf16_t* x, int ldx, const bf16_t* w, uint8_t* q, int ldq, float* scale, int rows, int H, float eps,
                                         hipStream_t s);
hipError_t aigv_launch_quant_fp8_rows(const bf16_t* x, int ldx, int rows, int K, uint8_t* q, int ldq, float* scale, hipStream_t s);
bool aigv_gemm256_supported(const GemmArgs& a);
hipError_t aigv_launch_gemm256_fused(const GemmArgs& a, int epi, hipStream_t s);
hipError_t aigv_launch_gemm_finalize(const GemmArgs& a, int epi, int k_slices, const float* ws, hipStream_t s);
hipError_t aigv_launch_gemm256(const GemmArgs& a, int epi, hipStream_t s);
bool aigv_gemmco_supported(const GemmArgs& a);
hipError_t aigv_launch_gemmco(const GemmArgs& a, int epi, hipStream_t s);

struct AttnArgs {
  const bf16_t* q; int ldq;
  const bf16_t* k; int ldk;
  const bf16_t* v; int ldv;
  bf16_t* o; int ldo;
  const int32_t* cu;
  int n_seq, max_len;
  int n_heads, n_kv_heads;
  int q_group_stride, kv_head_stride;
  int kv_len_offset;
  const int32_t* kv_off;
  size_t kv_seq_stride;
  int causal;
  float post_div;
  int round_scores;
  float q_prescale;
  const int32_t* rope_pos; const bf16_t* rope_cos; const bf16_t* rope_sin;
  int rope_pos_is_row;
  int q_tail;
  int uniform_len;
  int waves;
  int lead_key;
  int q_begin;
};
const char* aigv_attn_check(const AttnArgs& a, int head_dim);
hipError_t aigv_launch_attention(const AttnArgs& a, int head_dim, hipStream_t s);
size_t aigv_attention_decode_ws_floats(int n_seq, int n_kv, int g, int cap);
hipError_t aigv_launch_attention_decode(const bf16_t* q, int ldq, int q_group_stride, const bf16_t* kc,
                                        const bf16_t* vc, const int32_t* kv_lens, int cap, bf16_t* o, int ldo,
                                        int n_seq, int n_kv, int g, int head_dim, float post_div, int max_kv_len,
                                        float* ws, hipStream_t s);

hipError_t aigv_launch_layernorm(const bf16_t* x, int ldx, const bf16_t* w, const bf16_t* b, bf16_t* y, int ldy,
                                 int rows, int H, float eps, hipStream_t s);
hipError_t aigv_launch_rmsnorm(const bf16_t* x, int ldx, const bf16_t* w, bf16_t* y, int ldy, int rows, int H,
                               float eps, const int32_t* row_idx, hipStream_t s);
hipError_t aigv_launch_pixel_shuffle(const bf16_t* vit, int grid, int Hv, bf16_t* out, int frames, hipStream_t s);
hipError_t aigv_launch_im2col(const bf16_t* frames, int F, int C, int S, int P, int Kp, bf16_t* out, hipStream_t s);
hipError_t aigv_launch_gather_rows(const bf16_t* src, int ld, const int32_t* idx, int n, bf16_t* dst, int H, hipStream_t s);
hipError_t aigv_launch_scatter_rows(const bf16_t* src, const int32_t* idx, int n, bf16_t* dst, int ld, int H, hipStream_t s);
hipError_t aigv_launch_cls_rows(const bf16_t* cls_pos, bf16_t* x, int F, int tokens_per_frame, int H, hipStream_t s);
hipError_t aigv_launch_rope(bf16_t* qkv, int ld, const int32_t* pos, const bf16_t* cos, const bf16_t* sin,
                            int tokens, int n_rot, int slots, int n_groups, int D, hipStream_t s, int first_rot = 0);
hipError_t aigv_launch_embed(const int64_t* ids, const int32_t* slot, const bf16_t* emb, const bf16_t* vis,
                             const bf16_t* motion, int n_vis, bf16_t* out, int tokens, int H, hipStream_t s);
hipError_t aigv_launch_skinny_gemm(const bf16_t* x, int ldx, int R, const bf16_t* W, int ldw, int N, int K,
                                   const bf16_t* bias, const bf16_t* resid, int ldr, bf16_t* out, int ldo, int epi,
                                   hipStream_t s, const bf16_t* ls = nullptr, int p = 1);
struct AigvRopeKv {
  const int32_t* pos; const int32_t* seq;
  const bf16_t* cos; const bf16_t* sin;
  bf16_t* kc; bf16_t* vc;
  int g, n_kv, cap;
};
bool aigv_skinny_fp8_supported(int K, bool with_norm);
hipError_t aigv_launch_skinny_fp8(const bf16_t* x, int ldx, int R, const uint8_t* W8, int ldw, const float* w_scale, int N, int K, const bf16_t* resid,
                                  int ldr, bf16_t* out, int ldo, int epi, const AigvRopeKv* rk, const bf16_t* norm_w, float eps, int p, hipStream_t s);
bool aigv_skinny_norm_fusable(int K);
hipError_t aigv_launch_skinny_swiglu_normed(const bf16_t* x, int ldx, int R, const bf16_t* W, int ldw, int N, int K, bf16_t* out, int ldo,
                                            const bf16_t* norm_w, float norm_eps, hipStream_t s, int p = 1);
hipError_t aigv_launch_skinny_rope_kv(const bf16_t* x, int ldx, int R, const bf16_t* W, int ldw, int N, int K, bf16_t* qkv, int ldo,
                                      const int32_t* pos, const int32_t* seq, const bf16_t* cos, const bf16_t* sin, bf16_t* kc, bf16_t* vc,
                                      int g, int n_kv, int cap, int head_dim, hipStream_t s, const bf16_t* norm_w = nullptr, float norm_eps = 0.f, int p = 1);
hipError_t aigv_launch_lm_head_argmax(const bf16_t* h, int R, int H, const bf16_t* W, int V,
                                      unsigned long long* packed, int64_t* out_idx, float* out_val, hipStream_t s);
hipError_t aigv_launch_lm_head_logits(const bf16_t* h, int R, int H, const bf16_t* W, int V, bf16_t* out, int ldo, hipStream_t s);
struct ScoreHeadArgs {
  const bf16_t* x; int ldx; int B;
  int n_layers; int dims[9];
  const bf16_t* w[8]; const bf16_t* b[8];
  float* score;
};
hipError_t aigv_launch_score_head(const ScoreHeadArgs& a, bf16_t* scratch, hipStream_t s);
hipError_t aigv_launch_rope_kv_store(bf16_t* qkv, int ld, const int32_t* seq_of_tok, const int32_t* pos, const bf16_t* cos,
                                     const bf16_t* sin, bf16_t* kc, bf16_t* vc, int tokens, int n_groups, int g, int D, int cap,
                                     hipStream_t s);
hipError_t aigv_launch_kv_store(const bf16_t* qkv, int ld, const int32_t* seq_of_tok, const int32_t* pos,
                                bf16_t* kc, bf16_t* vc, int tokens, int n_groups, int g, int D, int cap,
                                hipStream_t s);
hipError_t aigv_launch_frame_ingest(const uint8_t* hwc, int n_frames, int H, int W, const float* mean, const float* stdv,
                                    bf16_t* out, hipStream_t s);
hipError_t aigv_launch_frame_resize_ingest(const uint8_t* hwc, int n_frames, int in_h, int in_w, int out_h, int out_w,
                                           const float* mean, const float* stdv, uint8_t* tmp_u8, uint8_t* out_u8, bf16_t* out_nchw,
                                           hipStream_t s);
void aigv_set_error(const char* msg);
hipError_t aigv_launch_advance(int32_t* a, int32_t* b, int n, hipStream_t s);
hipError_t aigv_launch_decode_eos(int64_t* tok, int32_t* state, int n, const int64_t* eos_host, int n_eos, int64_t pad, hipStream_t s);
#define AIGV_SMALL_INTS 256
struct SmallInts { int32_t v[AIGV_SMALL_INTS]; };
hipError_t aigv_launch_seqpos(const int32_t* cu_host, int n_seq, int32_t* pos, int32_t* seq, int32_t* cu_dev, int tokens,
                              hipStream_t s, const int32_t* pos_offset_host = nullptr);
hipError_t aigv_launch_write_ints(const int32_t* host, int n, int32_t* dst, hipStream_t s);
hipError_t aigv_launch_kv_reorder(const bf16_t* sk, const bf16_t* sv, bf16_t* dk, bf16_t* dv, const int32_t* parent, const int32_t* lens, int n,
                                  int layers, int nkv, int cap, int D, size_t kv_layer, int max_len, hipStream_t s);
```

### aigv-assessor_amd/modeling.py

```python
from __future__ import annotations

import ctypes as C
import os
from typing import Dict, List, Optional

import torch
import torch.nn as nn
import torch.nn.functional as F

from . import native, synth
from .config import InternVLChatConfig
from .conversation import get_conv_template


def rope_tables(head_dim: int, theta: float, n_pos: int, max_pos: int = 32768, scaling: Optional[dict] = None,
                seq_len: Optional[int] = None):
    base = float(theta)
    if scaling is not None and scaling.get("type") == "dynamic" and seq_len is not None and seq_len > max_pos:
        f = float(scaling["factor"])
        base = base * ((f * seq_len / max_pos) - (f - 1)) ** (head_dim / (head_dim - 2))
    inv_freq = 1.0 / (base ** (torch.arange(0, head_dim, 2).float() / head_dim))
    t = torch.arange(n_pos).to(inv_freq.dtype)
    if scaling is not None and scaling.get("type") == "linear":
        t = t / float(scaling["factor"])
# ... 1105 lines not shown
        return x

    @torch.no_grad()
    def generate(self, pixel_values: Optional[torch.Tensor] = None, input_ids: Optional[torch.Tensor] = None,
                 attention_mask: Optional[torch.Tensor] = None, visual_features: Optional[torch.Tensor] = None,
                 generation_config=None, output_hidden_states=None, return_dict=None, **generate_kwargs) -> torch.Tensor:
        assert self.img_context_token_id is not None
        max_new, eos, pad, sampler, procs, beams = self._gen_args(generation_config, generate_kwargs)
        pad = self.config.llm_config.pad_token_id if pad is None else pad
        dev = self.device
        input_ids = input_ids.to(dev)
        ids_packed, cu, _ = self._pack(input_ids, attention_mask.to(dev) if attention_mask is not None else None)
        slot = torch.full_like(ids_packed, -1, dtype=torch.int32)
        vis, n_vis = None, 0
        if pixel_values is not None or visual_features is not None:
            vit = visual_features if visual_features is not None else self.extract_feature(pixel_values)
            vis = vit.reshape(-1, vit.shape[-1]).to(dev).contiguous()
            n_vis = vis.shape[0]
            sel = ids_packed == self.img_context_token_id
            assert int(sel.sum()) != 0
            if int(sel.sum()) != n_vis:
                raise ValueError(f"visual token count mismatch: {int(sel.sum())} slots vs {n_vis} tokens")
            slot[sel] = torch.arange(n_vis, device=dev, dtype=torch.int32)
        return self._greedy(ids_packed, slot, cu, vis, n_vis, max_new, eos, pad, sampler=sampler, processors=procs, beams=beams)

    @torch.no_grad()
    def generate2(self, input_embeds: torch.Tensor, attention_mask: Optional[torch.Tensor] = None, visual_features=None,
                  generation_config=None, output_hidden_states=None, return_dict=None, **generate_kwargs) -> torch.Tensor:
        max_new, eos, pad, sampler, procs, beams = self._gen_args(generation_config, generate_kwargs)
        pad = self.config.llm_config.pad_token_id if pad is None else pad
        dev = self.device
        b, n, _ = input_embeds.shape
        mask = torch.ones((b, n), dtype=torch.bool, device=dev) if attention_mask is None else attention_mask.to(dev).bool()
        emb = input_embeds.to(dev)[mask].to(torch.bfloat16).contiguous()
        lens = mask.sum(1).tolist()
        cu = [0]
        for x in lens:
            cu.append(cu[-1] + int(x))
        T = emb.shape[0]
        ids = torch.zeros(T, dtype=torch.long, device=dev)
        slot = torch.arange(T, dtype=torch.int32, device=dev)
        return self._greedy(ids, slot, cu, emb, T, max_new, eos, pad, sampler=sampler, processors=procs, beams=beams)

    @torch.no_grad()
    def generate_stage2(self, pixel_values, input_ids, attention_mask=None, image_flags=None, motion_feature=None,
                        generation_config=None, **generate_kwargs) -> torch.LongTensor:
        if self.img_context_token_id is None:
            raise AssertionError("img_context_token_id must be set (stage2_eval.py:810)")
        max_new, eos, pad, sampler, procs, beams = self._gen_args(generation_config, generate_kwargs)
        pad = self.config.llm_config.pad_token_id if pad is None else pad
        B = input_ids.shape[0]
        plan = self._plan(input_ids, attention_mask, None, image_flags, pixel_values.shape[0], drop_dead_tail=False)
        motion_feature = self._motion_feature(pixel_values, B, motion_feature)
        self._native(n_frames=pixel_values.shape[0], n_tokens=plan["cu"][-1], n_clips=B)
        vit_embeds, motion = self._visual_inputs(pixel_values, None, motion_feature, plan)
        return self._greedy(plan["ids_packed"], plan["slot"], plan["cu"], vit_embeds, plan["n_vis"], max_new, eos, pad, motion=motion, sampler=sampler, processors=procs, beams=beams)

    def chat2(self, tokenizer, pixel_values, input_ids, generation_config, attention_mask, history=None,
              return_history=False, image_flags=None, IMG_START_TOKEN="<img>", IMG_END_TOKEN="</img>",
              IMG_CONTEXT_TOKEN="<IMG_CONTEXT>", verbose=False, motion_feature=None):
        self.img_context_token_id = tokenizer.convert_tokens_to_ids(IMG_CONTEXT_TOKEN)
        template = get_conv_template(self.template)
        generation_config["eos_token_id"] = tokenizer.convert_tokens_to_ids(template.sep)
        out = self.generate_stage2(pixel_values, input_ids, attention_mask, image_flags, motion_feature, **generation_config)
        response = tokenizer.batch_decode(out, skip_special_tokens=True)[0].split(template.sep)[0].strip()
        return (response, history) if return_history else response

    def chat(self, tokenizer, pixel_values, question, generation_config, history=None, return_history=False,
             num_patches_list=None, IMG_START_TOKEN="<img>", IMG_END_TOKEN="</img>", IMG_CONTEXT_TOKEN="<IMG_CONTEXT>",
             verbose=False):
        if history is None and pixel_values is not None and "<image>" not in question:
            question = "<image>\n" + question
        if num_patches_list is None:
            num_patches_list = [pixel_values.shape[0]] if pixel_values is not None else []
        assert pixel_values is None or len(pixel_values) == sum(num_patches_list)
        self.img_context_token_id = tokenizer.convert_tokens_to_ids(IMG_CONTEXT_TOKEN)
        template = get_conv_template(self.template)
        template.system_message = self.system_message
        eos_token_id = tokenizer.convert_tokens_to_ids(template.sep)
        history = [] if history is None else history
        for old_q, old_a in history:
            template.append_message(template.roles[0], old_q)
            template.append_message(template.roles[1], old_a)
        template.append_message(template.roles[0], question)
        template.append_message(template.roles[1], None)
        query = template.get_prompt()
        for num_patches in num_patches_list:
            image_tokens = IMG_START_TOKEN + IMG_CONTEXT_TOKEN * self.num_image_token * num_patches + IMG_END_TOKEN
            query = query.replace("<image>", image_tokens, 1)
        model_inputs = tokenizer(query, return_tensors="pt")
        generation_config["eos_token_id"] = eos_token_id
        out = self.generate(pixel_values=pixel_values, input_ids=model_inputs["input_ids"],
                            attention_mask=model_inputs["attention_mask"], **generation_config)
        response = tokenizer.batch_decode(out, skip_special_tokens=True)[0].split(template.sep)[0].strip()
        history.append((question, response))
        if return_history:
            return response, history
        if verbose:
            print(query.replace(IMG_CONTEXT_TOKEN, "").replace(f"{IMG_START_TOKEN}{IMG_END_TOKEN}", "<image>"), response)
        return response

    def batch_chat(self, tokenizer, pixel_values, questions, generation_config, num_patches_list=None, history=None,
                   return_history=False, IMG_START_TOKEN="<img>", IMG_END_TOKEN="</img>",
                   IMG_CONTEXT_TOKEN="<IMG_CONTEXT>", verbose=False, image_counts=None):
        if history is not None or return_history:
            raise NotImplementedError("Now multi-turn chat is not supported in batch_chat.")
        if image_counts is not None:
            num_patches_list = image_counts
        self.img_context_token_id = tokenizer.convert_tokens_to_ids(IMG_CONTEXT_TOKEN)
        queries = []
        template = None
        for idx, num_patches in enumerate(num_patches_list):
            question = questions[idx]
            if pixel_values is not None and "<image>" not in question:
                question = "<image>\n" + question
            template = get_conv_template(self.template)
            template.system_message = self.system_message
            template.append_message(template.roles[0], question)
            template.append_message(template.roles[1], None)
            query = template.get_prompt()
            image_tokens = IMG_START_TOKEN + IMG_CONTEXT_TOKEN * self.num_image_token * num_patches + IMG_END_TOKEN
            queries.append(query.replace("<image>", image_tokens, 1))
        tokenizer.padding_side = "left"
        model_inputs = tokenizer(queries, return_tensors="pt", padding=True)
        generation_config["eos_token_id"] = tokenizer.convert_tokens_to_ids(template.sep)
        out = self.generate(pixel_values=pixel_values, input_ids=model_inputs["input_ids"],
                            attention_mask=model_inputs["attention_mask"], **generation_config)
        responses = tokenizer.batch_decode(out, skip_special_tokens=True)
        return [r.split(template.sep)[0].strip() for r in responses]

    def set_precision(self, mode: str = "bf16"):
        self._drop_graphs()
        if mode not in ("bf16", "fp8"):
            raise ValueError("precision must be 'bf16' or 'fp8'")
        self._precision = mode
        if self._ctx is not None and not self._dirty:
            native.check(native.load().aigv_set_precision(self._ctx, 1 if mode == "fp8" else 0), self._ctx)

    def set_attention_numerics(self, mode: str = "fp32"):
        self._drop_graphs()
        if mode not in ("reference", "fp32"):
            raise ValueError("attention numerics must be 'reference' or 'fp32'")
        self._attn_numerics = 1 if mode == "reference" else 0
        lib, ctx = self._native()
        native.check(lib.aigv_set_attention_numerics(ctx, self._attn_numerics), ctx)

    def set_gemm_mode(self, mode: int = -1):
        self._drop_graphs()
        self._gemm_mode = int(mode)
        lib, ctx = self._native()
        native.check(lib.aigv_set_gemm_mode(ctx, int(mode)), ctx)

    TUNE_KNOBS = {"gemm_mode": 0, "gemm256_order": 1, "gemm256_variant": 2, "attn_waves": 3, "skinny_p": 4, "body_tile": 5, "co_kmax": 6,
                  "tail_slices": 7, "attn_lead_key": 8, "decode_fused": 9, "decode_fp8": 10, "skinny_p8": 11, "fuse_tails": 12, "lone_body": 13}

    def tune(self, knob: str, value: int = -1):
        self._drop_graphs()
        lib, ctx = self._native()
        native.check(lib.aigv_ctx_tune(ctx, self.TUNE_KNOBS[knob], int(value)), ctx)

    def capture_forward(self, **forward_kwargs):
        pv = forward_kwargs.get("pixel_values")
        if torch.is_tensor(pv) and forward_kwargs.get("motion_feature") is None and forward_kwargs.get("input_ids") is not None:
            self._prepare_motion_branch(pv, int(forward_kwargs["input_ids"].shape[0]))
        torch.cuda.synchronize(self.device)
        graph = torch.cuda.CUDAGraph()
        self._capture_keep = []
        try:
            with native.capturing(), torch.cuda.graph(graph, capture_error_mode="relaxed"):
                outputs = self.forward(**forward_kwargs)
            keep = self._capture_keep
        finally:
            self._capture_keep = None

        def replay(_graph=graph, _keep=keep):
            _graph.replay()
            return outputs
        return replay, outputs

    def set_row_trimming(self, on: bool = True):
        self._drop_graphs()
        self._row_trim = bool(on)
        lib, ctx = self._native()
        native.check(lib.aigv_set_row_trimming(ctx, int(on)), ctx)
        self.drop_dead_tail = bool(on)

    def prof_enable(self, on: bool = True):
        self._drop_graphs()
        self._prof_on = bool(on)
        lib, ctx = self._native()
        native.check(lib.aigv_prof_enable(ctx, int(on)), ctx)

    def prof_read(self) -> Dict[str, Dict[str, float]]:
        lib, ctx = self._native()
        out = {}
        for cls, name in enumerate(("gemm_llm", "attn_vit", "attn_llm", "skinny", "gemm_fp8", "gemm_vit")):
            n, ms, fl, by = C.c_int64(), C.c_double(), C.c_double(), C.c_double()
            native.check(lib.aigv_prof_read(ctx, cls, C.byref(n), C.byref(ms), C.byref(fl), C.byref(by)), ctx)
            out[name] = dict(launches=n.value, ms=ms.value, flops=fl.value, bytes=by.value)
        out["gemm"] = {k: out["gemm_llm"][k] + out["gemm_vit"][k] for k in out["gemm_llm"]}
        return out
```

### include/aigv_amd.h

```cpp
#ifndef AIGV_AMD_H
#define AIGV_AMD_H

#include <stdint.h>

#ifdef __cplusplus
extern "C" {
#endif

#define AIGV_ABI_VERSION 1

typedef struct aigv_ctx aigv_ctx;

enum aigv_status {
  AIGV_OK = 0,
  AIGV_ERR_ARG = -1,
  AIGV_ERR_HIP = -2,
  AIGV_ERR_STATE = -3,
  AIGV_ERR_ALLOC = -4
};

enum aigv_dtype { AIGV_BF16 = 0, AIGV_F32 = 1 };

typedef struct aigv_config {
  int32_t vit_hidden, vit_inter, vit_heads, vit_layers;
  int32_t image_size, patch_size, num_channels;
  int32_t vit_norm_rms;
  int32_t vit_qk_norm;
  int32_t vit_qkv_bias;
  float vit_eps;
  int32_t select_layer;
  int32_t shuffle;
  int32_t llm_hidden, llm_inter, llm_heads, llm_kv_heads, llm_layers, vocab;
  float rms_eps;
  int32_t max_positions;
  int32_t motion_dim;
  int32_t n_score_layers;
  int32_t score_dims[8];
  int32_t max_frames;
  int32_t vit_chunk;
  int32_t max_tokens;
  int32_t max_seqs;
  int32_t max_out_rows;
  int32_t kv_capacity;
} aigv_config;

int aigv_abi_version(void);
int aigv_sizeof_config(void);
int aigv_ctx_create(int device, const aigv_config* cfg, aigv_ctx** out);
void aigv_ctx_destroy(aigv_ctx* ctx);
int aigv_ctx_resize(aigv_ctx* ctx, const aigv_config* cfg);
const char* aigv_last_error(const aigv_ctx* ctx);
void aigv_clear_hip_error(void);

int aigv_load_weight(aigv_ctx* ctx, const char* name, const void* data, const int64_t* shape, int ndim,
                     int dtype, int on_device);
int aigv_finalize_weights(aigv_ctx* ctx);

int aigv_vit_forward(aigv_ctx* ctx, const void* frames, int n_frames, void* out_tokens, void* stream);
int aigv_project(aigv_ctx* ctx, const void* tokens, int rows, void* out, void* stream);
int aigv_motion_project(aigv_ctx* ctx, const void* motion_feature, int n_clips, void* out, void* stream);

int aigv_llm_prefill(aigv_ctx* ctx, const int64_t* ids, const int32_t* slot, const int32_t* cu_seqlens, int n_clips,
                     const void* vis, int n_vis, const void* motion, const int32_t* score_rows, float* score,
                     const int32_t* logit_rows, int n_logit_rows, int64_t* argmax, int keep_kv, void* stream);
int aigv_llm_extend(aigv_ctx* ctx, const int64_t* ids, const int32_t* cu, int n_clips, const int32_t* score_rows, float* score,
                    const int32_t* logit_rows, int n_logit_rows, int64_t* argmax, int commit, void* stream);

int aigv_kv_fork(aigv_ctx* ctx, int copies, void* stream);
int aigv_kv_reorder(aigv_ctx* ctx, const int32_t* parent, const int32_t* len, int n, void* stream);

enum aigv_precision { AIGV_PRECISION_BF16 = 0, AIGV_PRECISION_FP8_LLM = 1 };
int aigv_set_precision(aigv_ctx* ctx, int mode);
int aigv_set_row_trimming(aigv_ctx* ctx, int on);
#define AIGV_ATTENTION_NUMERICS_DEFAULT 0
int aigv_set_attention_numerics(aigv_ctx* ctx, int mode);
int aigv_get_attention_numerics(const aigv_ctx* ctx);
int aigv_set_gemm_mode(aigv_ctx* ctx, int mode);

int aigv_decode_step(aigv_ctx* ctx, const int64_t* ids, int64_t* next, void* stream);
int aigv_out_row_logits(aigv_ctx* ctx, int first_row, int n_rows, void* logits_bf16, int ldo, void* stream);
int aigv_out_row_hidden(aigv_ctx* ctx, int first_row, int n_rows, void* hidden_bf16, int ldo, void* stream);
int aigv_decode_eos(aigv_ctx* ctx, int64_t* tokens, int32_t* state, const int64_t* eos_ids, int n_eos, int64_t pad_id, void* stream);

int aigv_op_gemm(const void* A, int lda, const void* W, int ldw, void* C, int ldc, const void* bias, const void* ls,
                 const void* resid, int ldr, const void* pos, int np, int M, int N, int K, int epi, void* stream);
int aigv_op_gemm_rows(const void* A, int lda, const void* W, int ldw, void* C, int ldc, const void* bias, const void* ls,
                      const void* resid, int ldr, const int32_t* cu_host, int n_seq, int N, int K, int epi, void* stream);
int aigv_op_gemm_splitk(const void* A, int lda, const void* W, int ldw, void* C, int ldc, const void* bias, const void* ls,
                        const void* resid, int ldr, int M, int N, int K, int epi, int k_slices, void* ws_f32, void* stream);
int aigv_op_gemm_splitk256(const void* A, int lda, const void* W, int ldw, void* C, int ldc, const void* bias, const void* ls,
                           const void* resid, int ldr, int M, int N, int K, int epi, int k_slices, void* ws_f32, void* stream);
int aigv_op_quant_fp8_rows(const void* x_bf16, int ldx, int rows, int K, void* q_e4m3, int ldq, float* row_scale, void* stream);
int aigv_op_gemm_fp8(const void* A_e4m3, int lda, const void* W_e4m3, int ldw, void* C, int ldc, const float* row_scale,
                     const float* col_scale, const void* bias, const void* ls, const void* resid, int ldr, int M, int N, int K, int epi,
                     int k_slices, void* ws_f32, void* stream);
int aigv_op_skinny_gemm(const void* x, int ldx, int R, const void* W, int ldw, int N, int K, const void* bias,
                        const void* resid, int ldr, void* out, int ldo, int epi, void* stream);
int aigv_op_skinny_gemm_fp8(const void* x, int ldx, int R, const void* W_e4m3, int ldw, const float* w_scale, int N, int K, const void* resid,
                            int ldr, void* out, int ldo, int epi, const void* norm_w, float eps, int p, void* stream);
int aigv_op_layernorm(const void* x, int ldx, const void* w, const void* b, void* y, int ldy, int rows, int H,
                      float eps, void* stream);
int aigv_op_rmsnorm(const void* x, int ldx, const void* w, void* y, int ldy, int rows, int H, float eps,
                    const int32_t* row_idx, void* stream);
int aigv_op_rope(void* qkv, int ld, const int32_t* pos, const void* cos, const void* sin, int tokens, int n_rot,
                 int slots, int n_groups, int head_dim, void* stream);
int aigv_op_attention(const void* q, int ldq, const void* k, int ldk, const void* v, int ldv, void* o, int ldo,
                      const int32_t* cu, int n_seq, int max_len, int n_heads, int n_kv_heads, int q_group_stride,
                      int kv_head_stride, int head_dim, int causal, float post_div, float q_prescale, void* stream);
int aigv_op_attention_rope(const void* q, int ldq, const void* k, int ldk, const void* v, int ldv, void* o, int ldo,
                           const int32_t* cu, int n_seq, int max_len, int n_heads, int n_kv_heads, int q_group_stride,
                           int kv_head_stride, int head_dim, int causal, float post_div, float q_prescale, const int32_t* pos,
                           const void* cos, const void* sin, void* stream);
int aigv_op_pixel_shuffle(const void* vit_out, int grid, int vit_hidden, void* out, int n_frames, void* stream);
int aigv_op_im2col(const void* frames, int n_frames, int channels, int image_size, int patch, int kp, void* out,
                   void* stream);
int aigv_op_lm_head_argmax(const void* h, int rows, int hidden, const void* W, int vocab, void* scratch_u64,
                           int64_t* idx, float* val, void* stream);

int aigv_op_frame_ingest(const void* hwc_u8, int n_frames, int height, int width, const float* mean, const float* stdv,
                         void* out_nchw, void* stream);

int aigv_op_frame_resize_ingest(const void* hwc_u8, int n_frames, int in_h, int in_w, int out_h, int out_w, const float* mean,
                                const float* stdv, void* tmp_u8, void* out_u8_hwc, void* out_nchw, void* stream);

enum aigv_tune_knob {
  AIGV_TUNE_GEMM_MODE = 0,
  AIGV_TUNE_GEMM256_ORDER = 1,
  AIGV_TUNE_GEMM256_VARIANT = 2,
  AIGV_TUNE_ATTN_WAVES = 3,
  AIGV_TUNE_SKINNY_P = 4,
  AIGV_TUNE_BODY_TILE = 5,
  AIGV_TUNE_CO_KMAX = 6,
  AIGV_TUNE_TAIL_SLICES = 7,
  AIGV_TUNE_ATTN_LEAD_KEY = 8,
  AIGV_TUNE_DECODE_FUSED = 9,
  AIGV_TUNE_DECODE_FP8 = 10,
  AIGV_TUNE_SKINNY_P8 = 11,
  AIGV_TUNE_FUSE_TAILS = 12,
  AIGV_TUNE_LONE_BODY = 13
};
int aigv_ctx_tune(aigv_ctx* ctx, int knob, int value);
int aigv_tune_gemm(int mode, double rate256);
int aigv_tune_co_gemm(int kmax);
int aigv_tune_default(int knob, int value);
int aigv_plan_gemm(int M, int N, int K, int epi, int* plan, double* est_us);
int aigv_tune_attention(int waves);
int aigv_tune_skinny(int p);

enum aigv_prof_class { AIGV_PROF_GEMM = 0, AIGV_PROF_ATTN_VIT = 1, AIGV_PROF_ATTN_LLM = 2, AIGV_PROF_SKINNY = 3,
                       AIGV_PROF_GEMM_FP8 = 4, AIGV_PROF_GEMM_VIT = 5, AIGV_PROF_COUNT = 6 };
int aigv_prof_enable(aigv_ctx* ctx, int on);
int aigv_prof_read(aigv_ctx* ctx, int cls, int64_t* launches, double* total_ms, double* flops, double* bytes);

typedef struct aigv_slowfast aigv_slowfast;
int aigv_slowfast_create(int device, int max_clips, int frames_per_clip, int height, int width, aigv_slowfast** out);
void aigv_slowfast_destroy(aigv_slowfast* sf);
int aigv_slowfast_load_weight(aigv_slowfast* sf, const char* name, const void* host_data, const int64_t* shape, int ndim, int dtype);
int aigv_slowfast_finalize(aigv_slowfast* sf);
int aigv_slowfast_forward(aigv_slowfast* sf, const void* frames_nchw_bf16, int clips, void* feature_bf16, void* stream);
double aigv_slowfast_flops_per_clip(const aigv_slowfast* sf);
int aigv_op_conv3d(const void* x, int ld_in, int Cin, int B, const int* dims, const void* w_packed, int Kp, const float* bias, int Cout,
                   const void* res, int ld_res, void* out, int ld_out, int c_off, int relu, void* stream);

#ifdef __cplusplus
}
#endif
#endif
```

Baseline: 34.18.

## Fold tiny-tail skinny GEMM rows into the gemm256 launch as extra blocks

```diff
diff --git a/aigv-assessor_amd/build.py b/aigv-assessor_amd/build.py
--- a/aigv-assessor_amd/build.py
+++ b/aigv-assessor_amd/build.py
@@ -9,7 +9,7 @@
 CSRC = os.path.join(HERE, "csrc")
 OBJ = os.path.join(HERE, "build")
 SOURCES = ["api.hip", "gemm.hip", "gemm256.hip", "gemmco.hip", "attention.hip", "rowops.hip", "head.hip", "head8.hip", "ingest.hip", "slowfast.hip"]
-HEADERS = ["common.h", "kernels.h", "attn_lay.h", os.path.join("..", "..", "include", "aigv_amd.h")]
+HEADERS = ["common.h", "kernels.h", "attn_lay.h", "skinny.h", os.path.join("..", "..", "include", "aigv_amd.h")]
 OUT = os.path.join(HERE, "libaigv_amd.so")
 FLAGS = ["--offload-arch=gfx950", "-O3", "-std=c++17", "-fPIC", "-Wno-unused-value"]
 EXTRA_FLAGS = {"attention.hip": ["-fno-slp-vectorize"]}
diff --git a/aigv-assessor_amd/csrc/api.hip b/aigv-assessor_amd/csrc/api.hip
--- a/aigv-assessor_amd/csrc/api.hip
+++ b/aigv-assessor_amd/csrc/api.hip
@@ -86,7 +86,7 @@
   int attn_round_scores = AIGV_ATTENTION_NUMERICS_DEFAULT;
   int gemm_mode = -1;
   int t_order = -1, t_variant = -1, t_attn_waves = -1, t_skinny_p = -1, t_body_tile = -1, t_co_kmax = -1;
-  int t_tail_slices = -1, t_lead_key = -1, t_decode_fused = -1, t_decode_fp8 = -1, t_skinny_p8 = -1, t_fuse_tails = -1, t_lone_body = -1;
+  int t_tail_slices = -1, t_lead_key = -1, t_decode_fused = -1, t_decode_fp8 = -1, t_skinny_p8 = -1, t_fuse_tails = -1, t_lone_body = -1, t_fuse_tiny = -1;
   size_t splitk_floats = 0;
   float* splitk_ws = nullptr;
   float* splitk_ws_vit = nullptr;
@@ -215,6 +215,7 @@
   int gemm_mode = 0, order_sel = 0, variant_sel = 0, attn_waves = 0, skinny_p = 0, body_tile = 0, co_kmax = CO_KMAX_DEFAULT;
   int tail_slices = 0, lead_key = 0, decode_fused = 1, decode_fp8 = 1, skinny_p8 = 0;
   int fuse_tails = 0;
+  int fuse_tiny = 0;
   int lone_body = 1;
 };
 Tune g_tune;
@@ -236,6 +237,7 @@
     if (c->t_skinny_p8 >= 0) t.skinny_p8 = c->t_skinny_p8;
     if (c->t_fuse_tails >= 0) t.fuse_tails = c->t_fuse_tails;
     if (c->t_lone_body >= 0) t.lone_body = c->t_lone_body;
+    if (c->t_fuse_tiny >= 0) t.fuse_tiny = c->t_fuse_tiny;
   }
   return t;
 }
@@ -523,6 +525,24 @@
 
 int run_tiny_tails(aigv_ctx* c, const GemmArgs& a, int epi, const RowPlan& rp, hipStream_t s);
 
+bool tiny_jobs(const RowPlan& rp, GemmArgs& b) {
+  b.tiny_jobs = 0;
+  for (const RowPlan::Tiny& t : rp.tiny)
+    for (int i0 = 0; i0 < t.count; i0 += 64) {
+      if (b.tiny_jobs == AIGV_TINY_JOBS) { b.tiny_jobs = 0; return false; }
+      const long long r0 = (long long)t.row0 + (long long)i0 * t.stride_rows;
+      if (r0 > 0x7fffffffLL) { b.tiny_jobs = 0; return false; }
+      b.tiny_row0[b.tiny_jobs] = (int)r0; b.tiny_stride[b.tiny_jobs] = t.stride_rows; b.tiny_rows[b.tiny_jobs] = std::min(64, t.count - i0);
+      ++b.tiny_jobs;
+    }
+  return b.tiny_jobs > 0;
+}
+int tiny_row_count(const RowPlan& rp) {
+  int n = 0;
+  for (const RowPlan::Tiny& t : rp.tiny) n += t.count;
+  return n;
+}
+
 int run_gemm_rows(aigv_ctx* c, const GemmArgs& a, int epi, const RowPlan& rp, hipStream_t s) {
   if (const char* m = aigv_gemm_check(a, epi)) return fail(c, AIGV_ERR_ARG, "%s (M=%d N=%d K=%d epi=%d)", m, a.M, a.N, a.K, epi);
   if (a.M != rp.rows) return fail(c, AIGV_ERR_STATE, "row plan covers %d rows, the GEMM has %d", rp.rows, a.M);
@@ -570,7 +590,16 @@
     }
     if (rp.tail_halves > 0 && !tails_apart) TRY(launch_tab(c, a, epi, rp.d_tab + 2 * rp.body_halves, rp.tail_halves, rp.tail_rows, 1, s));
   } else if (!tails_apart) {
-    TRY(launch_tab(c, a, epi, rp.d_tab, rp.body_halves + rp.tail_halves, rp.body_halves * 128 + rp.tail_rows, 1, s));
+    const int halves = rp.body_halves + rp.tail_halves;
+    GemmArgs b = tuned(c, a);
+    b.row_tab = rp.d_tab; b.tab_halves = halves;
+    if (halves > 0 && tune_of(c).fuse_tiny == 0 && tiny_jobs(rp, b) && aigv_gemm256_tiny_supported(b, epi)) {
+      GemmArgs pf = a; pf.M = rp.body_halves * 128 + rp.tail_rows + tiny_row_count(rp);
+      GEMM_PROF(c, pf, s);
+      HIPCHK(c, aigv_launch_gemm256(b, epi, s));
+      return 0;
+    }
+    TRY(launch_tab(c, a, epi, rp.d_tab, halves, rp.body_halves * 128 + rp.tail_rows, 1, s));
   } else {
     const int tn = a.N / 256;
     const long body_wg = (long)(rp.body_halves / 2) * tn, slice_wg = (long)((rp.tail_halves + 1) / 2) * tn * S;
@@ -1616,6 +1645,9 @@
     case AIGV_TUNE_LONE_BODY:
       if (value < -1 || value > 4) break;
       c->t_lone_body = value; return 0;
+    case AIGV_TUNE_FUSE_TINY:
+      if (value < -1 || value > 1) break;
+      c->t_fuse_tiny = value; return 0;
     case AIGV_TUNE_SKINNY_P8:
       if (value != -1 && value != 0 && value != 1 && value != 2 && value != 4) break;
       c->t_skinny_p8 = value; return 0;
@@ -2019,6 +2051,7 @@
     case AIGV_TUNE_TAIL_SLICES: if (value < 0 || value > 16) break; g_tune.tail_slices = value; return 0;
     case AIGV_TUNE_FUSE_TAILS: if (value < 0 || value > 2) break; g_tune.fuse_tails = value; return 0;
     case AIGV_TUNE_LONE_BODY: if (value < 0 || value > 4) break; g_tune.lone_body = value; return 0;
+    case AIGV_TUNE_FUSE_TINY: if (value < 0 || value > 1) break; g_tune.fuse_tiny = value; return 0;
     case AIGV_TUNE_ATTN_LEAD_KEY: if (value < 0 || value > 1) break; g_tune.lead_key = value; return 0;
     case AIGV_TUNE_CO_KMAX: return aigv_tune_co_gemm(value);
     default: return fail(nullptr, AIGV_ERR_ARG, "aigv_tune_default: knob %d has no process default here (aigv_tune_gemm / _attention / _skinny set the others)", knob);
diff --git a/aigv-assessor_amd/csrc/gemm256.hip b/aigv-assessor_amd/csrc/gemm256.hip
--- a/aigv-assessor_amd/csrc/gemm256.hip
+++ b/aigv-assessor_amd/csrc/gemm256.hip
@@ -3,6 +3,7 @@
 
 #include "common.h"
 #include "kernels.h"
+#include "skinny.h"
 
 namespace {
 
@@ -46,11 +47,52 @@
   *(u16x8*)dst = val;
 }
 
-template <int EPI, int VAR, bool FP8 = false, bool FUSE = false>
+template <int EPI>
+__device__ __forceinline__ void tiny_tail_block(const GemmArgs& p, int b, char* smem) {
+  constexpr int SK = EPI == EPI_STORE ? SK_STORE : EPI == EPI_GELU ? SK_GELU : EPI == EPI_LS_RESID ? SK_LS_RESID : SK_RESID;
+  if (threadIdx.x >= 256) {
+    __syncthreads();
+    return;
+  }
+  const int per_job = (p.N + 15) / 16;
+  int j = 0;
+#pragma unroll
+  for (int i = 1; i < AIGV_TINY_JOBS; ++i) j += (i < p.tiny_jobs && b >= i * per_job) ? 1 : 0;
+  int row0 = p.tiny_row0[0], st = p.tiny_stride[0], R = p.tiny_rows[0];
+#pragma unroll
+  for (int i = 1; i < AIGV_TINY_JOBS; ++i)
+    if (j == i) { row0 = p.tiny_row0[i]; st = p.tiny_stride[i]; R = p.tiny_rows[i]; }
+  const int blk = b - j * per_job, tid = threadIdx.x;
+  float* part = (float*)smem;
+  const size_t r0 = (size_t)row0;
+  const bf16_t* x = p.A + r0 * p.lda;
+  const bf16_t* resid = p.resid ? p.resid + r0 * p.ldr : nullptr;
+  bf16_t* out = p.C + r0 * p.ldc;
+  const int ldx = st * p.lda, ldr = st * p.ldr, ldo = st * p.ldc;
+#define TINY_GO(RT) skinny_body<RT, SK>(blk, tid, part, nullptr, x, ldx, R, p.W, p.ldw, p.N, p.K, p.bias, resid, ldr, out, ldo, nullptr, p.ls, RopeKvArgs{}, NormArgs{})
+  switch ((R + 15) >> 4) {
+    case 1: TINY_GO(1); break;
+    case 2: TINY_GO(2); break;
+    case 3: TINY_GO(3); break;
+    default: TINY_GO(4); break;
+  }
+#undef TINY_GO
+}
+
+template <int EPI, int VAR, bool FP8 = false, bool FUSE = false, bool TINY = false>
 __global__ __launch_bounds__(512, 2) void gemm256_kernel(const GemmArgs p) {
   static_assert(!FP8 || ((VAR & 4) != 0 && EPI != EPI_PATCH), "the fp8 form uses the LDS-staged epilogue (or writes split-K slabs)");
   static_assert(!FUSE || (!FP8 && EPI != EPI_PARTIAL && EPI != EPI_PATCH), "the fused form: bf16, a body epilogue");
+  static_assert(!TINY || (!FP8 && !FUSE && (EPI == EPI_STORE || EPI == EPI_GELU || EPI == EPI_LS_RESID || EPI == EPI_RESID)),
+                "tiny tails: bf16, an epilogue the skinny kernel has");
   extern __shared__ __attribute__((aligned(16))) char smem[];
+  if constexpr (TINY) {
+    const int n_tiles = (p.row_tab ? (p.tab_halves + 1) / 2 : (p.M + TM - 1) / TM) * (p.N / TN);
+    if ((int)blockIdx.x >= n_tiles) {
+      tiny_tail_block<EPI>(p, (int)blockIdx.x - n_tiles, smem);
+      return;
+    }
+  }
   const int tid = threadIdx.x, lane = tid & 63;
   const int wave = __builtin_amdgcn_readfirstlane(tid >> 6);
   const int g = wave >> 2, wc = wave & 3;
@@ -699,7 +741,45 @@
   return hipErrorInvalidValue;
 }
 
+template <int EPI>
+static hipError_t launch256_tiny(const GemmArgs& a, hipStream_t s) {
+  static LdsAttrOnce lds_attr;
+  if (hipError_t e = lds_attr.ensure((const void*)gemm256_kernel<EPI, 7, false, false, true>, LDS_BYTES); e != hipSuccess) return e;
+  const int nbm = row_tiles(a), nbn = a.N / TN;
+  GemmArgs b = a;
+  b.order = tile_order(a, (size_t)a.N * (size_t)a.K >= ((size_t)32 << 20), nbm);
+  const int grid = nbm * nbn + a.tiny_jobs * ((a.N + 15) / 16);
+  hipLaunchKernelGGL((gemm256_kernel<EPI, 7, false, false, true>), dim3(grid), dim3(512), LDS_BYTES, s, b);
+  return hipGetLastError();
+}
+
+bool aigv_gemm256_tiny_supported(const GemmArgs& a, int epi) {
+  if (epi != EPI_STORE && epi != EPI_GELU && epi != EPI_LS_RESID && epi != EPI_RESID) return false;
+  const int v = a.variant_sel > 0 ? a.variant_sel - 1 : 1;
+  if (v == 0 || v == 3) return false;
+  if (!aigv_gemm256_supported(a) || a.K % 128 || a.lda % 8 || a.ldw % 8 || a.ldc % 4) return false;
+  if ((epi == EPI_LS_RESID || epi == EPI_RESID) && !a.resid) return false;
+  if (epi == EPI_LS_RESID && !a.ls) return false;
+  if (a.tiny_jobs < 1 || a.tiny_jobs > AIGV_TINY_JOBS) return false;
+  for (int j = 0; j < a.tiny_jobs; ++j) {
+    const long long st = a.tiny_stride[j];
+    if (a.tiny_rows[j] < 1 || a.tiny_rows[j] > 64 || a.tiny_row0[j] < 0 || st < 1) return false;
+    if (st * a.lda > 0x7fffffffLL || st * a.ldc > 0x7fffffffLL || st * a.ldr > 0x7fffffffLL) return false;
+  }
+  return true;
+}
+
 hipError_t aigv_launch_gemm256(const GemmArgs& a, int epi, hipStream_t s) {
+  if (a.tiny_jobs > 0) {
+    if (!aigv_gemm256_tiny_supported(a, epi)) return hipErrorInvalidValue;
+    switch (epi) {
+      case EPI_STORE: return launch256_tiny<EPI_STORE>(a, s);
+      case EPI_GELU: return launch256_tiny<EPI_GELU>(a, s);
+      case EPI_LS_RESID: return launch256_tiny<EPI_LS_RESID>(a, s);
+      case EPI_RESID: return launch256_tiny<EPI_RESID>(a, s);
+    }
+    return hipErrorInvalidValue;
+  }
   switch (a.variant_sel > 0 ? a.variant_sel - 1 : 1) {
     case 0: return launch256v<0>(a, epi, s);
     case 3: return launch256v<3>(a, epi, s);
diff --git a/aigv-assessor_amd/csrc/head.hip b/aigv-assessor_amd/csrc/head.hip
--- a/aigv-assessor_amd/csrc/head.hip
+++ b/aigv-assessor_amd/csrc/head.hip
@@ -4,32 +4,9 @@
 #include "common.h"
 #include "kernels.h"
 
+#include "skinny.h"
+
 namespace {
-
-#ifndef SKINNY_DEPTH2
-#define SKINNY_DEPTH2 8
-#endif
-enum { SK_STORE = 0, SK_RESID = 1, SK_SWIGLU = 2, SK_GELU = 3, SK_ARGMAX = 4, SK_RELU = 5, SK_LS_RESID = 6, SK_ROPE_KV = 7 };
-
-struct RopeKvArgs {
-  const int32_t* pos; const int32_t* seq;
-  const bf16_t* cos; const bf16_t* sin;
-  bf16_t* kc; bf16_t* vc;
-  int g, n_kv, cap;
-};
-
-struct NormArgs { const bf16_t* w; float eps; };
-
-__device__ __forceinline__ unsigned int ord_f32(float f) {
-  const unsigned int u = __float_as_uint(f);
-  return (u & 0x80000000u) ? ~u : (u | 0x80000000u);
-}
-
-template <bool NT>
-__device__ __forceinline__ bf16x8 wload(const bf16_t* p) {
-  if constexpr (NT) return __builtin_nontemporal_load((const bf16x8*)p);
-  else return *(const bf16x8*)p;
-}
 
 template <int RT, int EPI, int NWV = 4, bool NT = false, int NC = 0, int P = 1>
 __global__ __launch_bounds__(NWV * 64) void skinny_kernel(const bf16_t* __restrict__ x, int ldx, int R,
@@ -39,235 +16,9 @@
                                                      unsigned long long* __restrict__ packed,
                                                      const bf16_t* __restrict__ ls, const RopeKvArgs rk = RopeKvArgs{},
                                                      const NormArgs na = NormArgs{}) {
-  constexpr bool NORM = NC > 0;
-  static_assert(!NORM || (RT == 1 && NWV == 4), "the fused norm is the decode form: one row tile, 256 threads (rmsnorm_kernel's reduction)");
   extern __shared__ __attribute__((aligned(16))) bf16_t xs[];
-  constexpr int NS = (EPI == SK_SWIGLU || EPI == SK_ROPE_KV) ? 2 : (EPI == SK_ARGMAX && RT >= 2) ? 4 : 1;
-  static_assert(P == 1 || ((P == 2 || P == 4) && RT == 1 && EPI != SK_ARGMAX), "sub-slab forms: one row tile, 8 or 4 rows per slab");
-  constexpr int RS = 16 / P;
-  __shared__ float part[NWV - 1][NS][RT][4][64];
-  const int lane = threadIdx.x & 63, wave = threadIdx.x >> 6;
-  const int fr = lane & 15, fq = lane >> 4;
-  const int sr = fr % RS, sp = fr / RS;
-  const int n0 = EPI == SK_ROPE_KV ? (int)(blockIdx.x / (64 / RS)) * 128 + (int)(blockIdx.x % (64 / RS)) * RS
-                 : EPI == SK_SWIGLU ? (int)(blockIdx.x / P) * 32 + (int)(blockIdx.x % P) * RS
-                                    : blockIdx.x * RS * NS;
-  constexpr int SLAB_STEP = EPI == SK_ROPE_KV ? 64 : 16;
-  const int kper = K / (NWV * P), kbeg = (wave * P + sp) * kper;
-
-  const bf16_t* wrow[NS];
-#pragma unroll
-  for (int s = 0; s < NS; ++s) wrow[s] = W + (size_t)min(n0 + s * SLAB_STEP + sr, N - 1) * ldw + kbeg + fq * 8;
-  const bf16_t* xrow[RT];
-#pragma unroll
-  for (int t = 0; t < RT; ++t) xrow[t] = x + (size_t)min(t * 16 + sr, R - 1) * ldx + kbeg + fq * 8;
-
-  f32x4 acc[NS][RT];
-#pragma unroll
-  for (int s = 0; s < NS; ++s)
-#pragma unroll
-    for (int t = 0; t < RT; ++t) acc[s][t] = f32x4{0.f, 0.f, 0.f, 0.f};
-
-  constexpr int DEPTH = RT == 1 ? (NS == 1 ? 16 : SKINNY_DEPTH2) : (RT == 2 && NS == 1) ? 8 : 4;
-  int k = 0;
-  const int xs_off = min(sr, R - 1) * K + kbeg + fq * 8;
-  if constexpr (NORM) {
-    u16x8 xr[4][NC], gw[NC];
-#pragma unroll
-    for (int r = 0; r < 4; ++r)
-#pragma unroll
-      for (int c = 0; c < NC; ++c) xr[r][c] = *(const u16x8*)(x + (size_t)min(r, R - 1) * ldx + ((threadIdx.x + c * 256) << 3));
-#pragma unroll
-    for (int c = 0; c < NC; ++c) gw[c] = *(const u16x8*)(na.w + ((threadIdx.x + c * 256) << 3));
-    bf16x8 wf[DEPTH][NS];
-#pragma unroll
-    for (int u = 0; u < DEPTH; ++u)
-#pragma unroll
-      for (int s = 0; s < NS; ++s) wf[u][s] = wload<NT>(wrow[s] + 32 * u);
-    {
-      __shared__ float red[4];
-#pragma unroll
-      for (int r = 0; r < 4; ++r) {
-        if (r == 0 || r < R) {
-          float sq = 0.f;
-#pragma unroll
-          for (int c = 0; c < NC; ++c)
-#pragma unroll
-            for (int e = 0; e < 8; ++e) { const float v = bf2f(xr[r][c][e]); sq += v * v; }
-          const float rstd = rsqrtf(block_sum_256(sq, red) / (float)K + na.eps);
-#pragma unroll
-          for (int c = 0; c < NC; ++c) {
-            u16x8 o;
-#pragma unroll
-            for (int e = 0; e < 8; ++e) o[e] = f2bf(bf2f(gw[c][e]) * rbf(bf2f(xr[r][c][e]) * rstd));
-            *(u16x8*)(xs + (size_t)r * K + ((threadIdx.x + c * 256) << 3)) = o;
-          }
-        }
-      }
-      __syncthreads();
-    }
-#pragma unroll
-    for (int u = 0; u < DEPTH; ++u) {
-      const bf16x8 xf = *(const bf16x8*)(xs + xs_off + 32 * u);
-#pragma unroll
-      for (int s = 0; s < NS; ++s) acc[s][0] = __builtin_amdgcn_mfma_f32_16x16x32_bf16(wf[u][s], xf, acc[s][0], 0, 0, 0);
-    }
-    k = 32 * DEPTH;
-  }
-  auto run = [&](auto dtag) {
-    constexpr int DD = decltype(dtag)::value;
-    for (; k + 32 * DD <= kper; k += 32 * DD) {
-      bf16x8 wf[DD][NS], xf[DD][RT];
-#pragma unroll
-      for (int u = 0; u < DD; ++u) {
-#pragma unroll
-        for (int s = 0; s < NS; ++s) wf[u][s] = wload<NT>(wrow[s] + k + 32 * u);
-#pragma unroll
-        for (int t = 0; t < RT; ++t) {
-          if constexpr (NORM) xf[u][t] = *(const bf16x8*)(xs + xs_off + k + 32 * u);
-          else xf[u][t] = *(const bf16x8*)(xrow[t] + k + 32 * u);
-        }
-      }
-#pragma unroll
-      for (int u = 0; u < DD; ++u)
-#pragma unroll
-        for (int s = 0; s < NS; ++s)
-#pragma unroll
-          for (int t = 0; t < RT; ++t)
-            acc[s][t] = __builtin_amdgcn_mfma_f32_16x16x32_bf16(wf[u][s], xf[u][t], acc[s][t], 0, 0, 0);
-    }
-  };
-  run(std::integral_constant<int, DEPTH>{});
-  if constexpr (DEPTH > 8) run(std::integral_constant<int, 8>{});
-  if constexpr (DEPTH > 4) run(std::integral_constant<int, 4>{});
-  run(std::integral_constant<int, 1>{});
-
-  if (wave > 0) {
-#pragma unroll
-    for (int s = 0; s < NS; ++s)
-#pragma unroll
-      for (int t = 0; t < RT; ++t)
-#pragma unroll
-        for (int e = 0; e < 4; ++e) part[wave - 1][s][t][e][lane] = acc[s][t][e];
-  }
-  __syncthreads();
-  if (wave != 0) return;
-#pragma unroll
-  for (int s = 0; s < NS; ++s)
-#pragma unroll
-    for (int t = 0; t < RT; ++t)
-#pragma unroll
-      for (int e = 0; e < 4; ++e) {
-        if constexpr (NWV == 4) {
-          acc[s][t][e] += (part[0][s][t][e][lane] + part[1][s][t][e][lane]) + part[2][s][t][e][lane];
-        } else {
-          float sum = 0.f;
-#pragma unroll
-          for (int w = 0; w < NWV - 1; ++w) sum += part[w][s][t][e][lane];
-          acc[s][t][e] += sum;
-        }
-      }
-
-  if constexpr (P == 2) {
-#pragma unroll
-    for (int s = 0; s < NS; ++s)
-#pragma unroll
-      for (int e = 0; e < 4; ++e) acc[s][0][e] += __shfl(acc[s][0][e], (lane + 40) & 63, 64);
-  } else if constexpr (P == 4) {
-#pragma unroll
-    for (int s = 0; s < NS; ++s)
-#pragma unroll
-      for (int e = 0; e < 4; ++e) {
-        const float v = acc[s][0][e];
-        acc[s][0][e] = ((v + __shfl(v, (lane + 20) & 63, 64)) + __shfl(v, (lane + 40) & 63, 64)) + __shfl(v, (lane + 60) & 63, 64);
-      }
-  }
-  const bool own = P == 1 || (fr < RS && fq < RS / 4);
-
-#pragma unroll
-  for (int t = 0; t < RT; ++t) {
-    const int r = own ? t * 16 + fr : R;
-    if constexpr (EPI == SK_ARGMAX) {
-      unsigned long long best = 0ull;
-#pragma unroll
-      for (int sl = 0; sl < NS; ++sl)
-#pragma unroll
-        for (int e = 0; e < 4; ++e) {
-          const int n = n0 + sl * 16 + 4 * fq + e;
-          if (n < N) {
-            const unsigned long long key = ((unsigned long long)ord_f32(rbf(acc[sl][t][e])) << 32) | (0xFFFFFFFFu - (unsigned)n);
-            best = key > best ? key : best;
-          }
-        }
-      unsigned long long o = __shfl_xor(best, 16, 64); best = o > best ? o : best;
-      o = __shfl_xor(best, 32, 64); best = o > best ? o : best;
-      if (fq == 0 && r < R) atomicMax(packed + r, best);
-    } else if constexpr (EPI == SK_ROPE_KV) {
-      if (r < R) {
-        const int hs = blockIdx.x / (64 / RS), d = (int)(blockIdx.x % (64 / RS)) * RS + 4 * fq;
-        const int slot = hs % (rk.g + 2), gi = hs / (rk.g + 2);
-        const int p = rk.pos[r];
-        u16x4 olo, ohi;
-        if (slot <= rk.g) {
-          const u16x4 co = *(const u16x4*)(rk.cos + (size_t)p * 64 + d), si = *(const u16x4*)(rk.sin + (size_t)p * 64 + d);
-#pragma unroll
-          for (int e = 0; e < 4; ++e) {
-            const float x1 = rbf(acc[0][t][e]), x2 = rbf(acc[1][t][e]), cc = bf2f(co[e]), ss = bf2f(si[e]);
-            olo[e] = f2bf(rbf(x1 * cc) + rbf(-x2 * ss));
-            ohi[e] = f2bf(rbf(x2 * cc) + rbf(x1 * ss));
-          }
-        } else {
-#pragma unroll
-          for (int e = 0; e < 4; ++e) { olo[e] = f2bf(acc[0][t][e]); ohi[e] = f2bf(acc[1][t][e]); }
-        }
-        bf16_t* dst = slot < rk.g ? out + (size_t)r * ldo + (size_t)hs * 128 + d
-                                  : (slot == rk.g ? rk.kc : rk.vc) + (((size_t)rk.seq[r] * rk.n_kv + gi) * rk.cap + p) * 128 + d;
-        *(u16x4*)dst = olo;
-        *(u16x4*)(dst + 64) = ohi;
-      }
-    } else if constexpr (EPI == SK_SWIGLU) {
-      if (r < R) {
-        const int n = (int)(blockIdx.x / P) * 16 + (int)(blockIdx.x % P) * RS + 4 * fq;
-        u16x4 o;
-#pragma unroll
-        for (int e = 0; e < 4; ++e) {
-          const float g = rbf(acc[0][t][e]), u = rbf(acc[1][t][e]);
-          o[e] = f2bf(rbf(silu_f(g)) * u);
-        }
-        *(u16x4*)(out + (size_t)r * ldo + n) = o;
-      }
-    } else {
-      const int n = n0 + 4 * fq;
-      if (r < R && n < N) {
-        float v[4];
-#pragma unroll
-        for (int e = 0; e < 4; ++e) v[e] = acc[0][t][e] + (bias ? bf2f(bias[n + e]) : 0.f);
-#pragma unroll
-        for (int e = 0; e < 4; ++e) v[e] = rbf(v[e]);
-        if constexpr (EPI == SK_GELU) {
-#pragma unroll
-          for (int e = 0; e < 4; ++e) v[e] = rbf(gelu_fast(v[e]));
-        }
-        if constexpr (EPI == SK_RELU) {
-#pragma unroll
-          for (int e = 0; e < 4; ++e) v[e] = fmaxf(v[e], 0.f);
-        }
-        if constexpr (EPI == SK_LS_RESID) {
-#pragma unroll
-          for (int e = 0; e < 4; ++e) v[e] = rbf(v[e] * bf2f(ls[n + e]));
-        }
-        if constexpr (EPI == SK_RESID || EPI == SK_LS_RESID) {
-          const u16x4 rr = *(const u16x4*)(resid + (size_t)r * ldr + n);
-#pragma unroll
-          for (int e = 0; e < 4; ++e) v[e] = rbf(bf2f(rr[e]) + v[e]);
-        }
-        u16x4 o;
-#pragma unroll
-        for (int e = 0; e < 4; ++e) o[e] = f2bf(v[e]);
-        *(u16x4*)(out + (size_t)r * ldo + n) = o;
-      }
-    }
-  }
+  __shared__ float part[(NWV - 1) * skinny_ns(EPI, RT) * RT * 4 * 64];
+  skinny_body<RT, EPI, NWV, NT, NC, P>((int)blockIdx.x, (int)threadIdx.x, part, xs, x, ldx, R, W, ldw, N, K, bias, resid, ldr, out, ldo, packed, ls, rk, na);
 }
 
 __global__ void unpack_argmax_kernel(const unsigned long long* __restrict__ packed, int64_t* __restrict__ idx,
diff --git a/aigv-assessor_amd/csrc/kernels.h b/aigv-assessor_amd/csrc/kernels.h
--- a/aigv-assessor_amd/csrc/kernels.h
+++ b/aigv-assessor_amd/csrc/kernels.h
@@ -15,6 +15,8 @@
   EPI_PARTIAL = 6
 };
 
+constexpr int AIGV_TINY_JOBS = 4;
+
 struct GemmArgs {
   const bf16_t* A; int lda;
   const bf16_t* W; int ldw;
@@ -31,6 +33,8 @@
   const float* col_scale;
   const int32_t* row_tab; int tab_halves;
   int fuse_tail_halves, fuse_body_wg;
+  int tiny_jobs;
+  int tiny_row0[AIGV_TINY_JOBS], tiny_stride[AIGV_TINY_JOBS], tiny_rows[AIGV_TINY_JOBS];
   int order_sel, variant_sel;
   int order;
 };
@@ -49,6 +53,7 @@
 hipError_t aigv_launch_gemm256_fused(const GemmArgs& a, int epi, hipStream_t s);
 hipError_t aigv_launch_gemm_finalize(const GemmArgs& a, int epi, int k_slices, const float* ws, hipStream_t s);
 hipError_t aigv_launch_gemm256(const GemmArgs& a, int epi, hipStream_t s);
+bool aigv_gemm256_tiny_supported(const GemmArgs& a, int epi);
 bool aigv_gemmco_supported(const GemmArgs& a);
 hipError_t aigv_launch_gemmco(const GemmArgs& a, int epi, hipStream_t s);
 
diff --git a/aigv-assessor_amd/csrc/skinny.h b/aigv-assessor_amd/csrc/skinny.h
--- /dev/null
+++ b/aigv-assessor_amd/csrc/skinny.h
@@ -0,0 +1,273 @@
+#pragma once
+#include <type_traits>
+
+#include "common.h"
+
+namespace {
+
+#ifndef SKINNY_DEPTH2
+#define SKINNY_DEPTH2 8
+#endif
+enum { SK_STORE = 0, SK_RESID = 1, SK_SWIGLU = 2, SK_GELU = 3, SK_ARGMAX = 4, SK_RELU = 5, SK_LS_RESID = 6, SK_ROPE_KV = 7 };
+
+struct RopeKvArgs {
+  const int32_t* pos; const int32_t* seq;
+  const bf16_t* cos; const bf16_t* sin;
+  bf16_t* kc; bf16_t* vc;
+  int g, n_kv, cap;
+};
+
+struct NormArgs { const bf16_t* w; float eps; };
+
+__device__ __forceinline__ unsigned int ord_f32(float f) {
+  const unsigned int u = __float_as_uint(f);
+  return (u & 0x80000000u) ? ~u : (u | 0x80000000u);
+}
+
+template <bool NT>
+__device__ __forceinline__ bf16x8 wload(const bf16_t* p) {
+  if constexpr (NT) return __builtin_nontemporal_load((const bf16x8*)p);
+  else return *(const bf16x8*)p;
+}
+
+constexpr int skinny_ns(int epi, int rt) { return (epi == SK_SWIGLU || epi == SK_ROPE_KV) ? 2 : (epi == SK_ARGMAX && rt >= 2) ? 4 : 1; }
+
+template <int RT, int EPI, int NWV = 4, bool NT = false, int NC = 0, int P = 1>
+__device__ __forceinline__ void skinny_body(const int blk, const int tid, float* part_, bf16_t* xs,
+                                            const bf16_t* __restrict__ x, int ldx, int R,
+                                            const bf16_t* __restrict__ W, int ldw, int N, int K,
+                                            const bf16_t* __restrict__ bias, const bf16_t* __restrict__ resid,
+                                            int ldr, bf16_t* __restrict__ out, int ldo,
+                                            unsigned long long* __restrict__ packed,
+                                            const bf16_t* __restrict__ ls, const RopeKvArgs& rk, const NormArgs& na) {
+  constexpr bool NORM = NC > 0;
+  static_assert(!NORM || (RT == 1 && NWV == 4), "the fused norm is the decode form: one row tile, 256 threads (rmsnorm_kernel's reduction)");
+  constexpr int NS = skinny_ns(EPI, RT);
+  static_assert(P == 1 || ((P == 2 || P == 4) && RT == 1 && EPI != SK_ARGMAX), "sub-slab forms: one row tile, 8 or 4 rows per slab");
+  constexpr int RS = 16 / P;
+  float (*part)[NS][RT][4][64] = reinterpret_cast<float (*)[NS][RT][4][64]>(part_);
+  const int lane = tid & 63, wave = tid >> 6;
+  const int fr = lane & 15, fq = lane >> 4;
+  const int sr = fr % RS, sp = fr / RS;
+  const int n0 = EPI == SK_ROPE_KV ? (int)(blk / (64 / RS)) * 128 + (int)(blk % (64 / RS)) * RS
+                 : EPI == SK_SWIGLU ? (int)(blk / P) * 32 + (int)(blk % P) * RS
+                                    : blk * RS * NS;
+  constexpr int SLAB_STEP = EPI == SK_ROPE_KV ? 64 : 16;
+  const int kper = K / (NWV * P), kbeg = (wave * P + sp) * kper;
+
+  const bf16_t* wrow[NS];
+#pragma unroll
+  for (int s = 0; s < NS; ++s) wrow[s] = W + (size_t)min(n0 + s * SLAB_STEP + sr, N - 1) * ldw + kbeg + fq * 8;
+  const bf16_t* xrow[RT];
+#pragma unroll
+  for (int t = 0; t < RT; ++t) xrow[t] = x + (size_t)min(t * 16 + sr, R - 1) * ldx + kbeg + fq * 8;
+
+  f32x4 acc[NS][RT];
+#pragma unroll
+  for (int s = 0; s < NS; ++s)
+#pragma unroll
+    for (int t = 0; t < RT; ++t) acc[s][t] = f32x4{0.f, 0.f, 0.f, 0.f};
+
+  constexpr int DEPTH = RT == 1 ? (NS == 1 ? 16 : SKINNY_DEPTH2) : (RT == 2 && NS == 1) ? 8 : 4;
+  int k = 0;
+  const int xs_off = min(sr, R - 1) * K + kbeg + fq * 8;
+  if constexpr (NORM) {
+    u16x8 xr[4][NC], gw[NC];
+#pragma unroll
+    for (int r = 0; r < 4; ++r)
+#pragma unroll
+      for (int c = 0; c < NC; ++c) xr[r][c] = *(const u16x8*)(x + (size_t)min(r, R - 1) * ldx + ((tid + c * 256) << 3));
+#pragma unroll
+    for (int c = 0; c < NC; ++c) gw[c] = *(const u16x8*)(na.w + ((tid + c * 256) << 3));
+    bf16x8 wf[DEPTH][NS];
+#pragma unroll
+    for (int u = 0; u < DEPTH; ++u)
+#pragma unroll
+      for (int s = 0; s < NS; ++s) wf[u][s] = wload<NT>(wrow[s] + 32 * u);
+    {
+      __shared__ float red[4];
+#pragma unroll
+      for (int r = 0; r < 4; ++r) {
+        if (r == 0 || r < R) {
+          float sq = 0.f;
+#pragma unroll
+          for (int c = 0; c < NC; ++c)
+#pragma unroll
+            for (int e = 0; e < 8; ++e) { const float v = bf2f(xr[r][c][e]); sq += v * v; }
+          const float rstd = rsqrtf(block_sum_256(sq, red) / (float)K + na.eps);
+#pragma unroll
+          for (int c = 0; c < NC; ++c) {
+            u16x8 o;
+#pragma unroll
+            for (int e = 0; e < 8; ++e) o[e] = f2bf(bf2f(gw[c][e]) * rbf(bf2f(xr[r][c][e]) * rstd));
+            *(u16x8*)(xs + (size_t)r * K + ((tid + c * 256) << 3)) = o;
+          }
+        }
+      }
+      __syncthreads();
+    }
+#pragma unroll
+    for (int u = 0; u < DEPTH; ++u) {
+      const bf16x8 xf = *(const bf16x8*)(xs + xs_off + 32 * u);
+#pragma unroll
+      for (int s = 0; s < NS; ++s) acc[s][0] = __builtin_amdgcn_mfma_f32_16x16x32_bf16(wf[u][s], xf, acc[s][0], 0, 0, 0);
+    }
+    k = 32 * DEPTH;
+  }
+  auto run = [&](auto dtag) {
+    constexpr int DD = decltype(dtag)::value;
+    for (; k + 32 * DD <= kper; k += 32 * DD) {
+      bf16x8 wf[DD][NS], xf[DD][RT];
+#pragma unroll
+      for (int u = 0; u < DD; ++u) {
+#pragma unroll
+        for (int s = 0; s < NS; ++s) wf[u][s] = wload<NT>(wrow[s] + k + 32 * u);
+#pragma unroll
+        for (int t = 0; t < RT; ++t) {
+          if constexpr (NORM) xf[u][t] = *(const bf16x8*)(xs + xs_off + k + 32 * u);
+          else xf[u][t] = *(const bf16x8*)(xrow[t] + k + 32 * u);
+        }
+      }
+#pragma unroll
+      for (int u = 0; u < DD; ++u)
+#pragma unroll
+        for (int s = 0; s < NS; ++s)
+#pragma unroll
+          for (int t = 0; t < RT; ++t)
+            acc[s][t] = __builtin_amdgcn_mfma_f32_16x16x32_bf16(wf[u][s], xf[u][t], acc[s][t], 0, 0, 0);
+    }
+  };
+  run(std::integral_constant<int, DEPTH>{});
+  if constexpr (DEPTH > 8) run(std::integral_constant<int, 8>{});
+  if constexpr (DEPTH > 4) run(std::integral_constant<int, 4>{});
+  run(std::integral_constant<int, 1>{});
+
+  if (wave > 0) {
+#pragma unroll
+    for (int s = 0; s < NS; ++s)
+#pragma unroll
+      for (int t = 0; t < RT; ++t)
+#pragma unroll
+        for (int e = 0; e < 4; ++e) part[wave - 1][s][t][e][lane] = acc[s][t][e];
+  }
+  __syncthreads();
+  if (wave != 0) return;
+#pragma unroll
+  for (int s = 0; s < NS; ++s)
+#pragma unroll
+    for (int t = 0; t < RT; ++t)
+#pragma unroll
+      for (int e = 0; e < 4; ++e) {
+        if constexpr (NWV == 4) {
+          acc[s][t][e] += (part[0][s][t][e][lane] + part[1][s][t][e][lane]) + part[2][s][t][e][lane];
+        } else {
+          float sum = 0.f;
+#pragma unroll
+          for (int w = 0; w < NWV - 1; ++w) sum += part[w][s][t][e][lane];
+          acc[s][t][e] += sum;
+        }
+      }
+
+  if constexpr (P == 2) {
+#pragma unroll
+    for (int s = 0; s < NS; ++s)
+#pragma unroll
+      for (int e = 0; e < 4; ++e) acc[s][0][e] += __shfl(acc[s][0][e], (lane + 40) & 63, 64);
+  } else if constexpr (P == 4) {
+#pragma unroll
+    for (int s = 0; s < NS; ++s)
+#pragma unroll
+      for (int e = 0; e < 4; ++e) {
+        const float v = acc[s][0][e];
+        acc[s][0][e] = ((v + __shfl(v, (lane + 20) & 63, 64)) + __shfl(v, (lane + 40) & 63, 64)) + __shfl(v, (lane + 60) & 63, 64);
+      }
+  }
+  const bool own = P == 1 || (fr < RS && fq < RS / 4);
+
+#pragma unroll
+  for (int t = 0; t < RT; ++t) {
+    const int r = own ? t * 16 + fr : R;
+    if constexpr (EPI == SK_ARGMAX) {
+      unsigned long long best = 0ull;
+#pragma unroll
+      for (int sl = 0; sl < NS; ++sl)
+#pragma unroll
+        for (int e = 0; e < 4; ++e) {
+          const int n = n0 + sl * 16 + 4 * fq + e;
+          if (n < N) {
+            const unsigned long long key = ((unsigned long long)ord_f32(rbf(acc[sl][t][e])) << 32) | (0xFFFFFFFFu - (unsigned)n);
+            best = key > best ? key : best;
+          }
+        }
+      unsigned long long o = __shfl_xor(best, 16, 64); best = o > best ? o : best;
+      o = __shfl_xor(best, 32, 64); best = o > best ? o : best;
+      if (fq == 0 && r < R) atomicMax(packed + r, best);
+    } else if constexpr (EPI == SK_ROPE_KV) {
+      if (r < R) {
+        const int hs = blk / (64 / RS), d = (int)(blk % (64 / RS)) * RS + 4 * fq;
+        const int slot = hs % (rk.g + 2), gi = hs / (rk.g + 2);
+        const int p = rk.pos[r];
+        u16x4 olo, ohi;
+        if (slot <= rk.g) {
+          const u16x4 co = *(const u16x4*)(rk.cos + (size_t)p * 64 + d), si = *(const u16x4*)(rk.sin + (size_t)p * 64 + d);
+#pragma unroll
+          for (int e = 0; e < 4; ++e) {
+            const float x1 = rbf(acc[0][t][e]), x2 = rbf(acc[1][t][e]), cc = bf2f(co[e]), ss = bf2f(si[e]);
+            olo[e] = f2bf(rbf(x1 * cc) + rbf(-x2 * ss));
+            ohi[e] = f2bf(rbf(x2 * cc) + rbf(x1 * ss));
+          }
+        } else {
+#pragma unroll
+          for (int e = 0; e < 4; ++e) { olo[e] = f2bf(acc[0][t][e]); ohi[e] = f2bf(acc[1][t][e]); }
+        }
+        bf16_t* dst = slot < rk.g ? out + (size_t)r * ldo + (size_t)hs * 128 + d
+                                  : (slot == rk.g ? rk.kc : rk.vc) + (((size_t)rk.seq[r] * rk.n_kv + gi) * rk.cap + p) * 128 + d;
+        *(u16x4*)dst = olo;
+        *(u16x4*)(dst + 64) = ohi;
+      }
+    } else if constexpr (EPI == SK_SWIGLU) {
+      if (r < R) {
+        const int n = (int)(blk / P) * 16 + (int)(blk % P) * RS + 4 * fq;
+        u16x4 o;
+#pragma unroll
+        for (int e = 0; e < 4; ++e) {
+          const float g = rbf(acc[0][t][e]), u = rbf(acc[1][t][e]);
+          o[e] = f2bf(rbf(silu_f(g)) * u);
+        }
+        *(u16x4*)(out + (size_t)r * ldo + n) = o;
+      }
+    } else {
+      const int n = n0 + 4 * fq;
+      if (r < R && n < N) {
+        float v[4];
+#pragma unroll
+        for (int e = 0; e < 4; ++e) v[e] = acc[0][t][e] + (bias ? bf2f(bias[n + e]) : 0.f);
+#pragma unroll
+        for (int e = 0; e < 4; ++e) v[e] = rbf(v[e]);
+        if constexpr (EPI == SK_GELU) {
+#pragma unroll
+          for (int e = 0; e < 4; ++e) v[e] = rbf(gelu_fast(v[e]));
+        }
+        if constexpr (EPI == SK_RELU) {
+#pragma unroll
+          for (int e = 0; e < 4; ++e) v[e] = fmaxf(v[e], 0.f);
+        }
+        if constexpr (EPI == SK_LS_RESID) {
+#pragma unroll
+          for (int e = 0; e < 4; ++e) v[e] = rbf(v[e] * bf2f(ls[n + e]));
+        }
+        if constexpr (EPI == SK_RESID || EPI == SK_LS_RESID) {
+          const u16x4 rr = *(const u16x4*)(resid + (size_t)r * ldr + n);
+#pragma unroll
+          for (int e = 0; e < 4; ++e) v[e] = rbf(bf2f(rr[e]) + v[e]);
+        }
+        u16x4 o;
+#pragma unroll
+        for (int e = 0; e < 4; ++e) o[e] = f2bf(v[e]);
+        *(u16x4*)(out + (size_t)r * ldo + n) = o;
+      }
+    }
+  }
+}
+
+}
diff --git a/aigv-assessor_amd/modeling.py b/aigv-assessor_amd/modeling.py
--- a/aigv-assessor_amd/modeling.py
+++ b/aigv-assessor_amd/modeling.py
@@ -1281,7 +1281,7 @@
         native.check(lib.aigv_set_gemm_mode(ctx, int(mode)), ctx)
 
     TUNE_KNOBS = {"gemm_mode": 0, "gemm256_order": 1, "gemm256_variant": 2, "attn_waves": 3, "skinny_p": 4, "body_tile": 5, "co_kmax": 6,
-                  "tail_slices": 7, "attn_lead_key": 8, "decode_fused": 9, "decode_fp8": 10, "skinny_p8": 11, "fuse_tails": 12, "lone_body": 13}
+                  "tail_slices": 7, "attn_lead_key": 8, "decode_fused": 9, "decode_fp8": 10, "skinny_p8": 11, "fuse_tails": 12, "lone_body": 13, "fuse_tiny": 14}
 
     def tune(self, knob: str, value: int = -1):
         self._drop_graphs()
diff --git a/include/aigv_amd.h b/include/aigv_amd.h
--- a/include/aigv_amd.h
+++ b/include/aigv_amd.h
@@ -137,7 +137,8 @@
   AIGV_TUNE_DECODE_FP8 = 10,
   AIGV_TUNE_SKINNY_P8 = 11,
   AIGV_TUNE_FUSE_TAILS = 12,
-  AIGV_TUNE_LONE_BODY = 13
+  AIGV_TUNE_LONE_BODY = 13,
+  AIGV_TUNE_FUSE_TINY = 14
 };
 int aigv_ctx_tune(aigv_ctx* ctx, int knob, int value);
 int aigv_tune_gemm(int mode, double rate256);
```

After: 34.27, median of 6. Within noise of the previous version (+0.3%).
